# songhayeong/aes-fhe

Hardware: AMD Instinct MI355X
Metric: AES-128 blocks/sec (homomorphic full round) at N=2^16, L=30; 1/2/4/8 MI355X (higher is better)
Workload: dtype u64

## Files before the change

### aes-fhe_amd/csrc/bconv_cols.h

```cpp
#pragma once
#include "bconv_mfma.h"
#include "ntt256f.h"

namespace aesfhe {

__device__ __forceinline__ void cols256_stages_store(double (&x)[16], double q, double qi, bool big, const double* tg,
                                                     const double* cw, const double* twq, double* s, u64* out, int b,
                                                     int cl, int c) {
#pragma unroll
    for (int st = 0; st < 4; st++) {
        const int m = 1 << st, hh = 8 >> st;
        if (big && st == 2) {
#pragma unroll
            for (int a = 0; a < 16; a++) x[a] = fred(x[a], q, qi);
        }
#pragma unroll
        for (int a = 0; a < 16; a++) {
            if (a & hh) continue;
            const int ti = m + (a >> (4 - st));
            ct_fw(x[a], x[a + hh], cw[ti], tg[ti], q);
        }
    }
#pragma unroll
    for (int a = 0; a < 16; a++) s[(a * 16 + b) * kPadF + cl] = x[a];
    __syncthreads();
    const int ap = b;
#pragma unroll
    for (int bb = 0; bb < 16; bb++) x[bb] = s[(ap * 16 + bb) * kPadF + cl];
#pragma unroll
    for (int st = 4; st < 8; st++) {
        const int m = 1 << st, hh = 128 >> st;
        if (big && (st & 1) == 0) {
#pragma unroll
            for (int bb = 0; bb < 16; bb++) x[bb] = fred(x[bb], q, qi);
        }
#pragma unroll
        for (int bb = 0; bb < 16; bb++) {
            if (bb & hh) continue;
            ct_f(x[bb], x[bb + hh], twq[m + ap * (m >> 4) + (bb >> (8 - st))], q);
        }
    }
#pragma unroll
    for (int bb = 0; bb < 16; bb++) st_d(&out[(ap * 16 + bb) * 256 + c], x[bb]);
}

template <int NSTEP, bool YIN, bool VC = false, int PF = 1, int TT = 4, int LT = 2, int MODE = 0>
__global__ __launch_bounds__(256, TT == 4 ? 2 : 3) void k_bconv_cols(BconvArgs a, Tabs T, int ntile) {
    static_assert(TT == 4 || TT == 2, "4 or 2 targets per workgroup");
    static_assert(LT == 1 || LT == 2, "1 or 2 LDS tiles");
    __shared__ double s[LT][256 * kPadF];
    __shared__ double twq[TT][256];
    const int tid = threadIdx.x, lane = tid & 63, w = tid >> 6, c = lane & 31, h = lane >> 5;
    const int cl = tid & 15, b = tid >> 4;
    const int id = blockIdx.x, x8 = id & 7, j = id >> 3;
    const int tile = j % ntile, u = (j / ntile) * 8 + x8;
    const int bx = u & 15, z = u >> 4, zb = z / a.nc, zc = z - zb * a.nc;
    const int logN = T.logN;
    const u64* src = a.src + (long)zb * a.sbs + (long)zc * a.scs;
    u64* dst = a.dst + (long)zb * a.dbs + (long)zc * a.dcs;
    auto limb_of = [&](int tau) { return tau < a.skip0 ? tau : tau + a.skipn; };
    auto pid_of = [&](int tl) { return tl <= a.tl_l ? tl : a.Lp1 + tl - a.tl_l - 1; };
    const int tau0 = TT * tile;
    const int nlive = min(TT, a.nt - tau0);
#pragma unroll
    for (int m = 0; m < TT; m++)
        if (m < nlive) twq[m][tid] = T.psif[((long)pid_of(limb_of(tau0 + m)) << logN) + tid];
    bc_v4i af[NSTEP];
    {
        const int row = lane & 31, ta = row >> 3, pb = (row & 3) + 4 * ((row >> 2) & 1);
        const int tau = tau0 + ta;
        const bc_v4i* ap =
            (const bc_v4i*)(a.tab + ((long)(ta < TT && tau < a.nt ? pid_of(limb_of(tau)) : 0) * 8 + pb) * kBconvKT + 16 * h);
#pragma unroll
        for (int st = 0; st < NSTEP; st++) af[st] = ap[2 * st];
    }
    const u64* sp[NSTEP][2];
    double sq[NSTEP][2], sf[NSTEP][2];
#pragma unroll
    for (int st = 0; st < NSTEP; st++)
#pragma unroll
        for (int uu = 0; uu < 2; uu++) {
            const int sl = 4 * st + 2 * h + uu;
            const int i = sl < a.ns ? sl : 0;
            sp[st][uu] = src + ((long)i << logN) + bx * 16 + (c & 15);
            if (!YIN) {
                const int pid = i < a.s_nq ? a.s_q0 + i : a.s_p0 + i - a.s_nq;
                sq[st][uu] = (double)a.qall[pid];
                sf[st][uu] = a.sinvf[i];
            }
        }
    double xv[TT][16];
    double eq[TT], eqi[TT], ew32[TT], ef32[TT], ecr[TT];
#pragma unroll
    for (int m = 0; m < TT; m++) {
        const int pid = tau0 + m < a.nt ? pid_of(limb_of(tau0 + m)) : 0;
        const double* pc = a.pc + 4 * pid;
        eq[m] = pc[0], eqi[m] = pc[1], ew32[m] = pc[2], ef32[m] = pc[3], ecr[m] = a.corr[pid];
    }
    double ev[VC ? 4 * NSTEP : 1];
#pragma unroll
    for (int sl = 0; sl < (VC ? 4 * NSTEP : 0); sl++) ev[sl] = a.einv[sl];
    u64 raw[PF + 1][NSTEP][2][2];
    auto load = [&](u64 (&r)[NSTEP][2][2], int ar) {
#pragma unroll
        for (int st = 0; st < NSTEP; st++)
#pragma unroll
            for (int uu = 0; uu < 2; uu++)
#pragma unroll
                for (int g = 0; g < 2; g++) r[st][uu][g] = sp[st][uu][(16 * ar + 4 * w + 2 * g + (c >> 4)) * 256];
    };
#pragma unroll
    for (int p = 0; p < PF; p++) load(raw[p], p);
#pragma unroll
    for (int ar = 0; ar < 16; ar++) {
        if (ar + PF < 16) load(raw[(ar + PF) % (PF + 1)], ar + PF);
        bc_v4i bf[2][NSTEP];
        double ys[2][NSTEP][2];
#pragma unroll
        for (int st = 0; st < NSTEP; st++)
#pragma unroll
            for (int uu = 0; uu < 2; uu++)
#pragma unroll
                for (int g = 0; g < 2; g++) {
                    u64 yb = PF ? raw[ar % (PF + 1)][st][uu][g] : sp[st][uu][(16 * ar + 4 * w + 2 * g + (c >> 4)) * 256];
                    if (!YIN) {
                        const double q = sq[st][uu], f = sf[st][uu];
                        double y = fmul_rem(u2d(yb), tw_w(f, q), f, q);
                        y = y < 0.0 ? y + q : y;
                        yb = (u64)__double_as_longlong(y + 4503599627370496.0) & 0xFFFFFFFFFFFFFULL;
                    }
                    if (VC) ys[g][st][uu] = u2d(yb);
                    bf[g][st][2 * uu] = (int)(unsigned)yb ^ (int)0x80808080;
                    bf[g][st][2 * uu + 1] = (int)(unsigned)(yb >> 32) ^ (int)0x80808080;
                }
        if constexpr (VC) {
            double yl[NSTEP][2][2];
#pragma unroll
            for (int st = 0; st < NSTEP; st++)
#pragma unroll
                for (int uu = 0; uu < 2; uu++) swap_halves(ys[0][st][uu], ys[1][st][uu], yl[st][uu][0], yl[st][uu][1]);
            double sum = 0.0;
#pragma unroll
            for (int st = 0; st < NSTEP; st++)
#pragma unroll
                for (int hh = 0; hh < 2; hh++)
#pragma unroll
                    for (int uu = 0; uu < 2; uu++) {
                        const int sl = 4 * st + 2 * hh + uu;
                        sum = sum + yl[st][uu][hh] * ev[sl];
                    }
            const int vown = (int)__builtin_rint(sum);
            const auto pr = __builtin_amdgcn_permlane32_swap((unsigned)vown, (unsigned)vown, false, false);
            const int voth = (int)(h ? pr[0] : pr[1]);
#pragma unroll
            for (int st = 0; st < NSTEP; st++)
#pragma unroll
                for (int uu = 0; uu < 2; uu++)
                    if (4 * st + 2 * h + uu == a.ns) {
#pragma unroll
                        for (int g = 0; g < 2; g++) {
                            bf[g][st][2 * uu] = ((g == h ? vown : voth) & 0xff) ^ (int)0x80808080;
                            bf[g][st][2 * uu + 1] = (int)0x80808080;
                        }
                    }
        }
        if constexpr (MODE == 2) {
#pragma unroll
            for (int m = 0; m < TT; m++) xv[m][ar] = (double)(bf[0][0][0] & 0xffffff) + (double)(bf[1][NSTEP - 1][3] & 0xff);
            continue;
        }
        bc_v16i acc[2];
#pragma unroll
        for (int g = 0; g < 2; g++) {
            acc[g] = bc_v16i{};
#pragma unroll
            for (int st = 0; st < NSTEP; st++) acc[g] = __builtin_amdgcn_mfma_i32_32x32x32_i8(af[st], bf[g][st], acc[g], 0, 0, 0);
        }
#pragma unroll
        for (int m = 0; m < TT; m++) {
            if (m >= nlive) break;
            double part[2];
#pragma unroll
            for (int g = 0; g < 2; g++) {
                const int p01 = acc[g][4 * m] + acc[g][4 * m + 1] * 256, p23 = acc[g][4 * m + 2] + acc[g][4 * m + 3] * 256;
                part[g] = __builtin_fma((double)p23, 65536.0, (double)p01);
            }
            double lo, hi;
            swap_halves(part[0], part[1], lo, hi);
            xv[m][ar] = fred(lo + fmul_rem(hi, ew32[m], ef32[m], eq[m]) + ecr[m], eq[m], eqi[m]);
        }
    }
    __syncthreads();
    if constexpr (MODE == 1) {
#pragma unroll
        for (int m = 0; m < TT; m++) {
            if (m >= nlive) break;
            u64* o = dst + ((long)limb_of(tau0 + m) << logN);
#pragma unroll
            for (int ar = 0; ar < 16; ar++) st_d(&o[(ar * 16 + b) * 256 + bx * 16 + cl], xv[m][ar]);
        }
        return;
    }
#pragma unroll
    for (int m = 0; m < TT; m++) {
        if (m >= nlive) break;
        if (LT == 1 && m > 0) __syncthreads();
        const int tl = limb_of(tau0 + m), pid = pid_of(tl);
        const double q = (double)T.q[pid], qi = T.qinv[pid];
        cols256_stages_store(xv[m], q, qi, q >= kBigPrime, T.psif + ((long)pid << logN), T.cw + (long)pid * kColW,
                             twq[m], s[m % LT], dst + ((long)tl << logN), b, cl, bx * 16 + cl);
    }
}

}
```

### aes-fhe_amd/csrc/engine.hip

```cpp
#include <hip/hip_runtime.h>

#include <algorithm>
#include <atomic>
#include <cstdarg>
#include <cstdlib>
#include <cstdio>
#include <cstring>
#include <map>
#include <unordered_map>
#include <memory>
#include <mutex>
#include <string>
#include <vector>

#include "../../include/aesfhe.h"
#include "kernels_ops.h"
#include "ntt256f.h"
#include "ks_fused.h"
#include "bconv_mfma.h"
#include "bconv_cols.h"
#include "basis_tables.h"
#include "bsgs_plan.h"
#include "operands.h"
#include "arena.h"
// ... 241 lines not shown
    }
    ~ProfScope() {
        if (!on) return;
        hipEventRecord(b, s);
        e->recs.push_back({fam, a, b, bytes, label, disp});
    }
};

static void prof_flush(aesfhe_engine* e) {
    if (e->recs.empty()) return;
    hipStreamSynchronize(e->stream);
    for (auto& r : e->recs) {
        float ms = 0;
        hipEventElapsedTime(&ms, r.a, r.b);
        e->prof_ms[r.fam] += ms;
        e->prof_bytes[r.fam] += r.bytes;
        e->prof_n[r.fam] += 1;
        if (r.label) {
            KernStat& k = e->prof_k[r.label];
            k.n++;
            k.d += r.disp;
            k.ms += ms;
            k.bytes += r.bytes;
        }
        e->spare.push_back(r.a);
        e->spare.push_back(r.b);
    }
    e->recs.clear();
}

template <typename T>
static T* upload_small(aesfhe_engine* e, const T* src, size_t count) {
    size_t bytes = (count * sizeof(T) + 255) & ~(size_t)255;
    if (bytes > e->ring_size) throw_err(AESFHE_EARG, "argument upload too large");
    if (e->ring_off + bytes > e->ring_size) {
        HIPC(hipStreamSynchronize(e->stream));
        e->ring_off = 0;
    }
    memcpy(e->ring_h + e->ring_off, src, count * sizeof(T));
    T* dst = (T*)(e->ring_d + e->ring_off);
    HIPC(hipMemcpyAsync(dst, e->ring_h + e->ring_off, count * sizeof(T), hipMemcpyHostToDevice, e->stream));
    e->ring_off += bytes;
    return dst;
}

struct DevOperands {
    const u64* const* ptr = nullptr;
    const long *bs = nullptr, *ps = nullptr;
    const int* np = nullptr;
};
enum { OP_PTR = 1, OP_BS = 2, OP_PS = 4, OP_NP = 8 };
static std::vector<DevOperands> upload(aesfhe_engine* e, std::initializer_list<const OperandTable*> tabs, int fields) {
    std::vector<DevOperands> d(tabs.size());
    auto array = [&](int bit, auto OperandTable::*src, auto DevOperands::*dst) {
        if (!(fields & bit)) return;
        size_t i = 0;
        for (const OperandTable* t : tabs) {
            if (!(t->*src).empty()) d[i].*dst = upload_small(e, (t->*src).data(), (t->*src).size());
            i++;
        }
    };
    array(OP_PTR, &OperandTable::ptr, &DevOperands::ptr);
    array(OP_BS, &OperandTable::bs, &DevOperands::bs);
    array(OP_PS, &OperandTable::ps, &DevOperands::ps);
    array(OP_NP, &OperandTable::np, &DevOperands::np);
    return d;
}

static void* pool_get(aesfhe_engine* e, size_t bytes, bool tmp = false) {
    static const bool poison = getenv("AESFHE_POOL_POISON") && atoi(getenv("AESFHE_POOL_POISON"));
    (void)tmp;
    void* p = e->pool.get(bytes);
    e->peak_total = std::max(e->peak_total, e->pool.live + e->tpool.live);
    if (poison && p) HIPC(hipMemsetAsync(p, 0xA5, bytes, e->stream));
    return p;
}
static u64* dalloc(aesfhe_engine* e, size_t words) { return (u64*)pool_get(e, words * 8, true); }
static void dfree(aesfhe_engine* e, u64* p, size_t words) { e->pool.put(p, words * 8); }

struct Tmp {
    aesfhe_engine* e = nullptr;
    u64* p = nullptr;
    size_t w = 0;
    Tmp() = default;
    Tmp(aesfhe_engine* e_, size_t words) : e(e_), p(dalloc(e_, words)), w(words) {}
    Tmp(Tmp&& o) noexcept : e(o.e), p(o.p), w(o.w) { o.p = nullptr; }
    Tmp& operator=(Tmp&& o) noexcept {
        std::swap(e, o.e), std::swap(p, o.p), std::swap(w, o.w);
        o.reset();
        return *this;
    }
    ~Tmp() { reset(); }
    void reset() {
        if (p) dfree(e, p, w);
        p = nullptr;
    }
    explicit operator bool() const { return p != nullptr; }
};

struct CtFree {
    void operator()(aesfhe_ct* c) const { aesfhe_ct_free(c); }
};
using CtPtr = std::unique_ptr<aesfhe_ct, CtFree>;

static void release_all(std::vector<CtPtr>& v, aesfhe_ct** outs) {
    for (size_t i = 0; i < v.size(); i++) outs[i] = v[i].release();
}

static CtPtr ct_new(aesfhe_engine* e, int B, int np, int level) {
    auto* c = new aesfhe_ct{e, B, np, level, 0, nullptr, 0};
    e->refs++;
    CtPtr h(c);
    c->bytes = (size_t)B * np * (level + 1) * e->N * 8;
    c->d = (u64*)pool_get(e, c->bytes);
    return h;
}

static std::vector<CtPtr> ct_split_batch(aesfhe_engine* e, CtPtr r, int m) {
    const int B = r->B / m;
    const size_t part = (size_t)B * r->np * (r->level + 1) * e->N * 8;
    std::vector<CtPtr> out(m);
    for (int t = 0; t < m; t++) {
        out[t].reset(new aesfhe_ct{e, B, r->np, r->level, 0, nullptr, 0});
        e->refs++;
    }
    e->pool.split(r->d, m, part);
    for (int t = 0; t < m; t++) {
        out[t]->bytes = part;
        out[t]->d = (u64*)((char*)r->d + (size_t)t * part);
    }
    r->d = nullptr;
    aesfhe_ct_free(r.release());
    return out;
}

static CtPtr ct_zero_new(aesfhe_engine* e, int B, int np, int level) {
    CtPtr c = ct_new(e, B, np, level);
    HIPC(hipMemsetAsync(c->d, 0, c->bytes, e->stream));
    c->is_zero = 1;
    return c;
}

using View = Operand;

static View view_of(const aesfhe_ct* c) {
    View v;
    v.d = c->d;
    v.B = c->B;
    v.np = c->np;
    v.level = c->level;
    v.ps = (long)(c->level + 1) * c->eng->N;
    v.bs = (long)c->np * v.ps;
    v.zero = c->is_zero;
    return v;
}

static Opnd opnd(const View& v, int outB) {
    Opnd o;
    o.ptr = v.zero ? nullptr : v.d;
    o.bs = bcast_stride(v.B, v.bs, outB);
    o.ps = v.ps;
    o.np = v.np;
    o.bmask = (v.B > 1 && v.B < outB) ? v.B - 1 : -1;
    return o;
}

static Out out_of(aesfhe_ct* c) {
    Out o;
    o.ptr = c->d;
    o.ps = (long)(c->level + 1) * c->eng->N;
    o.bs = (long)c->np * o.ps;
    return o;
}

static View view_of(const CtPtr& c) { return view_of(c.get()); }
static Out out_of(const CtPtr& c) { return out_of(c.get()); }

static dim3 ew_grid(aesfhe_engine* e, int y, int z) { return dim3(e->N / 256, y, z); }

template <int R1>
static void ntt_fwd_t(aesfhe_engine* e, Span src, Span dst, int total) {
    constexpr int CW = (kTile / R1) < kC2 ? (kTile / R1) : kC2;
    constexpr int RW = (kTile / kC2) < R1 ? (kTile / kC2) : R1;
    Tabs T = e->tabs();
    const double by = 8.0 * e->N * (double)total;
    {
        ProfScope ps(e, FAM_NTT, by, "ntt_generic");
        hipLaunchKernelGGL(k_ntt_fwd_cols<R1>, dim3(kC2 / CW, total), dim3(256), 0, e->stream, src, dst, T);
    }
    {
        ProfScope ps(e, FAM_NTT, by, "ntt_generic");
        hipLaunchKernelGGL(k_ntt_fwd_rows<R1>, dim3(R1 / RW, total), dim3(256), 0, e->stream, dst, T);
    }
}
template <int R1>
static void ntt_inv_t(aesfhe_engine* e, Span src, Span dst, int total) {
    constexpr int CW = (kTile / R1) < kC2 ? (kTile / R1) : kC2;
    constexpr int RW = (kTile / kC2) < R1 ? (kTile / kC2) : R1;
    Tabs T = e->tabs();
    const double by = 8.0 * e->N * (double)total;
    {
        ProfScope ps(e, FAM_NTT, by, "ntt_generic");
        hipLaunchKernelGGL(k_ntt_inv_rows<R1>, dim3(R1 / RW, total), dim3(256), 0, e->stream, src, dst, T);
    }
    {
        ProfScope ps(e, FAM_NTT, by, "ntt_generic");
        hipLaunchKernelGGL(k_ntt_inv_cols<R1>, dim3(kC2 / CW, total), dim3(256), 0, e->stream, dst, T);
    }
}

template <int R>
static void ntt256(aesfhe_engine* e, Span src, Span dst, int total, bool inverse, const double* lf = nullptr) {
    Tabs T = e->tabs();
    const double by = 8.0 * e->N * (double)total;
    {
        ProfScope ps(e, FAM_NTT, by, inverse ? "ntt_inv_rows" : "ntt_fwd_cols");
        if (!inverse) hipLaunchKernelGGL(k_nttf_fwd_cols<R>, dim3(16, total), dim3(256), 0, e->stream, src, dst, T);
        else hipLaunchKernelGGL((k_nttf_inv_rows<R, false>), dim3(R / 16, total), dim3(256), 0, e->stream, src, dst, T, Span{}, (const u64*)nullptr);
    }
    ProfScope ps(e, FAM_NTT, by, inverse ? "ntt_inv_cols" : "ntt_fwd_rows");
    if (!inverse) hipLaunchKernelGGL((k_nttf_fwd_rows_t<false, R>), dim3(R / 16, total), dim3(256), 0, e->stream, dst, T, RowFin{});
    else if (lf) hipLaunchKernelGGL((k_nttf_inv_cols<R, true>), dim3(16, total), dim3(256), 0, e->stream, dst, T, lf);
    else hipLaunchKernelGGL((k_nttf_inv_cols<R, false>), dim3(16, total), dim3(256), 0, e->stream, dst, T, (const double*)nullptr);
}

static bool fused_ntt(const aesfhe_engine* e) { return e->logN == 16 || e->logN == 17; }

static void intt_prod(aesfhe_engine* e, Span a, Span b, Span dst, int total, const u64* fac, const double* lf = nullptr) {
    if (total <= 0) return;
    Tabs T = e->tabs();
    const double by = 8.0 * e->N * (double)total;
    {
        ProfScope ps(e, FAM_NTT, 2.0 * by, "ntt_inv_rows_prod");
        if (e->logN == 16) {
            if (fac) hipLaunchKernelGGL((k_nttf_inv_rows<256, true, true>), dim3(16, total), dim3(256), 0, e->stream, a, dst, T, b, fac);
            else hipLaunchKernelGGL((k_nttf_inv_rows<256, true, false>), dim3(16, total), dim3(256), 0, e->stream, a, dst, T, b, fac);
        } else {
            if (fac) hipLaunchKernelGGL((k_nttf_inv_rows<512, true, true>), dim3(32, total), dim3(256), 0, e->stream, a, dst, T, b, fac);
            else hipLaunchKernelGGL((k_nttf_inv_rows<512, true, false>), dim3(32, total), dim3(256), 0, e->stream, a, dst, T, b, fac);
        }
    }
    ProfScope ps(e, FAM_NTT, by, "ntt_inv_cols");
    if (e->logN == 16) {
        if (lf) hipLaunchKernelGGL((k_nttf_inv_cols<256, true>), dim3(16, total), dim3(256), 0, e->stream, dst, T, lf);
        else hipLaunchKernelGGL((k_nttf_inv_cols<256, false>), dim3(16, total), dim3(256), 0, e->stream, dst, T, lf);
    } else {
        if (lf) throw_err(AESFHE_EUNSUPPORTED, "per-limb INTT factors at N = 2^17");
        hipLaunchKernelGGL((k_nttf_inv_cols<512, false>), dim3(16, total), dim3(256), 0, e->stream, dst, T, lf);
    }
    HIPC(hipGetLastError());
}

static void ntt_fwd_cols(aesfhe_engine* e, Span src, Span dst, int total) {
    if (e->logN == 16) hipLaunchKernelGGL(k_nttf_fwd_cols<256>, dim3(16, total), dim3(256), 0, e->stream, src, dst, e->tabs());
    else hipLaunchKernelGGL(k_nttf_fwd_cols<512>, dim3(16, total), dim3(256), 0, e->stream, src, dst, e->tabs());
}
static void ntt_fwd_cols(aesfhe_engine* e, Span sp, int total) { ntt_fwd_cols(e, sp, sp, total); }

static void ntt(aesfhe_engine* e, Span src, Span dst, int total, bool inverse) {
    if (total <= 0) return;
    if (e->logN == 16 || e->logN == 17) {
        if (e->logN == 16) ntt256<256>(e, src, dst, total, inverse);
        else ntt256<512>(e, src, dst, total, inverse);
        HIPC(hipGetLastError());
        return;
    }
    switch (e->logN) {
#define CASE(LG, R)                                                        \
    case LG:                                                               \
        if (inverse) ntt_inv_t<R>(e, src, dst, total);                     \
        else ntt_fwd_t<R>(e, src, dst, total);                             \
        break;
        CASE(10, 4)
        CASE(11, 8)
        CASE(12, 16)
        CASE(13, 32)
        CASE(14, 64)
        CASE(15, 128)
        CASE(16, 256)
        CASE(17, 512)
#undef CASE
        default:
            throw_err(AESFHE_EUNSUPPORTED, "log_n %d not supported by the HIP NTT", e->logN);
    }
    HIPC(hipGetLastError());
}

static Span span_s(u64* base, long pstride, int nl, int nq, int qpid0, int spid0) {
    Span s;
    s.base = base;
    s.pstride = pstride;
    s.nl = nl;
    s.nq = nq;
    s.qpid0 = qpid0;
    s.spid0 = spid0;
    return s;
}


static void build_tables(aesfhe_engine* e) {
    const int N = e->N, np = e->np, L = e->L, K = e->K, Lp1 = e->Lp1;
    const auto& Q = e->chain.q;
    std::vector<u64> hq(Q), hpsi((size_t)np * N), hipsi((size_t)np * N), hninv(np);
    std::vector<double> hqinv(np), hpsif((size_t)np * N), hipsif((size_t)np * N), hninvf(np);
    e->h_iroot.resize(np);
    for (int p = 0; p < np; p++) {
        u64 qq = Q[p];
        hqinv[p] = 1.0 / (double)qq;
        u64 psi = min_primitive_root(qq, N), ip = h_invmod(psi, qq);
        std::vector<u64> pw(N), ipw(N);
        pw[0] = ipw[0] = 1;
        for (int k = 1; k < N; k++) {
            pw[k] = h_mulmod(pw[k - 1], psi, qq);
            ipw[k] = h_mulmod(ipw[k - 1], ip, qq);
        }
        for (int k = 0; k < N; k++) {
            unsigned r = bit_reverse((unsigned)k, e->logN);
            hpsi[(size_t)p * N + k] = pw[r];
            hipsi[(size_t)p * N + k] = ipw[r];
            hpsif[(size_t)p * N + k] = (double)pw[r] / (double)qq;
            hipsif[(size_t)p * N + k] = (double)ipw[r] / (double)qq;
        }
        e->h_iroot[p] = pw[N / 2];
        hninv[p] = h_invmod((u64)N, qq);
        hninvf[p] = (double)hninv[p] / (double)qq;
    }
    DevBlocks& dev = e->dev;
    Tabs& t = e->tab;
    t.q = e->q = dev.up(hq);
    t.qinv = e->qinv = dev.up(hqinv);
    t.psi = dev.up(hpsi);
    t.psif = dev.up(hpsif);
    t.ipsi = dev.up(hipsi);
    t.ipsif = dev.up(hipsif);
    t.ninv = dev.up(hninv);
    t.ninvf = dev.up(hninvf);
    if (fused_ntt(e)) {
        const int R = N / 256;
        std::vector<double> hr((size_t)np * R * 8), hir((size_t)np * R * 8);
        for (int p = 0; p < np; p++)
            for (int row = 0; row < R; row++)
                for (int sh = 0; sh < 8; sh++) {
                    hr[((size_t)p * R + row) * 8 + sh] = hpsif[(size_t)p * N + (row << sh)];
                    hir[((size_t)p * R + row) * 8 + sh] = hipsif[(size_t)p * N + (row << sh)];
                }
        t.rtwf = dev.up(hr);
        t.irtwf = dev.up(hir);
    }
    {
        std::vector<Tw> htw((size_t)np * N), hitw((size_t)np * N);
        for (size_t i = 0; i < htw.size(); i++) {
            htw[i] = Tw{hpsi[i], hpsif[i]};
            hitw[i] = Tw{hipsi[i], hipsif[i]};
        }
        t.tw = dev.up(htw);
        t.itw = dev.up(hitw);
    }
    {
        std::vector<double> hcw((size_t)np * kColW), hicw((size_t)np * kColW);
        for (int p = 0; p < np; p++)
            for (int k = 0; k < kColW; k++) {
                hcw[(size_t)p * kColW + k] = (double)hpsi[(size_t)p * N + (k < N ? k : 0)];
                hicw[(size_t)p * kColW + k] = (double)hipsi[(size_t)p * N + (k < N ? k : 0)];
            }
        t.cw = dev.up(hcw);
        t.icw = dev.up(hicw);
    }
    t.logN = e->logN;
    t.Lp1 = Lp1;

    static_assert(sizeof(WQ) == sizeof(TwD), "ModDown's hatf rows are the kernels' TwD");
    ModUpTables mu;
    ModDownTables md;
    if (!build_modup_tables(Q, Lp1, e->A, hninv, mu) || !build_moddown_tables(Q, Lp1, e->K, hninv, md))
        throw_err(AESFHE_EUNSUPPORTED, "base-conversion constant beyond 7 bytes");
    e->mu_hatinvf = dev.up(mu.hatinvf);
    e->mu_nhatf = dev.up(mu.nhatf);
    e->bc_mu_tab = dev.up(mu.tab);
    e->bc_mu_corr = dev.up(mu.corr);
    e->bc_pc = dev.up(mu.pc);
    e->md = MdTabs{dev.up(md.invf), dev.up(md.ninvf), dev.up(md.einv), dev.up(md.tab), dev.up(md.corr),
                   dev.up(md.dinv), dev.up(md.dinvf), (TwD*)dev.up(md.hatf), dev.up(md.dmodf)};
    e->pmod = dev.up(md.pmod);
    e->pmodf = e->md.dmodf;
    const RescaleTables rs = build_rescale_tables(Q, Lp1);
    e->rs_inv = dev.up(rs.inv);
    e->rs_invf = dev.up(rs.invf);
    e->rs_mod = dev.up(rs.mod);
}

extern "C" int aesfhe_engine_create(const aesfhe_params* pp, aesfhe_engine** out) {
    API_BEGIN
    if (!pp || !out) throw_err(AESFHE_EARG, "null argument");
    if (pp->log_n < 10 || pp->log_n > 17) throw_err(AESFHE_EARG, "log_n must be in [10, 17]");
    if (pp->max_level < 1 || pp->special_primes < 1 || pp->special_primes > 16 ||
        pp->max_level + 1 + pp->special_primes > kMaxPrimes)
        throw_err(AESFHE_EARG, "bad level / special prime count");
    if (pp->scale_bits < 20 || pp->scale_bits > 50 || pp->base_bits > 50 || pp->special_bits > 50)
        throw_err(AESFHE_EARG, "bit sizes must keep every prime below 2^50");
    std::unique_ptr<aesfhe_engine> e(new aesfhe_engine());
    e->logN = pp->log_n;
    e->N = 1 << pp->log_n;
    e->L = pp->max_level;
    e->K = pp->special_primes;
    e->Lp1 = e->L + 1;
    e->np = e->L + 1 + e->K;
    e->A = pp->digit_primes > 0 ? pp->digit_primes : e->K;
    if (e->A > 16) throw_err(AESFHE_EARG, "key-switch digit width %d outside 1..16", e->A);
    e->dnum = (e->L + 1 + e->A - 1) / e->A;
    e->device = pp->device;
    e->seed = pp->seed;
    e->ck = chacha_key(pp->seed, pp->seed_ext);
    if (pp->primes) {
        e->chain.q.assign(pp->primes, pp->primes + e->np);
        e->chain.scale = scales_from_primes(e->chain.q, e->L, pp->scale_bits);
    } else {
        e->chain = make_chain(e->logN, e->L, e->K, pp->base_bits, pp->special_bits, pp->scale_bits);
    }
    for (u64 x : e->chain.q)
        if (x >> 50) throw_err(AESFHE_EARG, "prime %llu exceeds 2^50", (unsigned long long)x);
    if (e->A > e->K && !digits_below_p(e->chain.q, e->Lp1, e->K, e->A))
        throw_err(AESFHE_EARG, "a key-switch digit of %d primes exceeds P (%d special primes)", e->A, e->K);
    HIPC(hipSetDevice(e->device));
    HIPC(hipStreamCreateWithFlags(&e->stream, hipStreamNonBlocking));
    build_tables(e.get());
    e->pool.chunk_bytes = std::max((size_t)1 << 28, ((size_t)16384 * 8) << e->logN);
    if (e->logN == 16) {
        e->pool.chunk_bytes = (size_t)8192 * 8 << e->logN;
        e->pool.first_fit = true;
        e->pool.grow_cap = 1.2;
    }
    if (const char* cm = getenv("AESFHE_ARENA_CHUNK_MB")) {
        const long mb = atol(cm);
        if (mb > 0) e->pool.chunk_bytes = (size_t)mb << 20;
    }
    e->tpool.chunk_bytes = e->pool.chunk_bytes;
    e->tpool.tag = 't';
    if (const char* tp = getenv("AESFHE_ARENA_TRACE")) {
        static std::atomic<int> engines{0};
        const std::string path = std::string(tp) + "." + std::to_string(engines++);
        e->pool.trace = e->tpool.trace = fopen(path.c_str(), "w");
    }
    HIPC(hipMalloc(&e->ring_d, e->ring_size));
    HIPC(hipHostMalloc((void**)&e->ring_h, e->ring_size, hipHostMallocDefault));
    *out = e.release();
    API_END
}

extern "C" int aesfhe_chain(const aesfhe_params* pp, uint64_t* primes, double* scales) {
    API_BEGIN
    Chain c = make_chain(pp->log_n, pp->max_level, pp->special_primes, pp->base_bits, pp->special_bits, pp->scale_bits);
    std::copy(c.q.begin(), c.q.end(), primes);
    std::copy(c.scale.begin(), c.scale.end(), scales);
    API_END
}

static void engine_unref(aesfhe_engine* e) {
    if (--e->refs == 0) delete e;
}
extern "C" void aesfhe_engine_destroy(aesfhe_engine* e) {
    if (e) engine_unref(e);
}

extern "C" int aesfhe_engine_dims(const aesfhe_engine* e, int32_t d[4]) {
    d[0] = e->logN;
    d[1] = e->L;
    d[2] = e->K;
    d[3] = e->dnum;
    return 0;
}
extern "C" int aesfhe_engine_primes(const aesfhe_engine* e, uint64_t* o) {
    std::copy(e->chain.q.begin(), e->chain.q.end(), o);
    return 0;
}
extern "C" int aesfhe_engine_scales(const aesfhe_engine* e, double* o) {
    std::copy(e->chain.scale.begin(), e->chain.scale.end(), o);
    return 0;
}
extern "C" double aesfhe_engine_mul_scale(const aesfhe_engine* e, int32_t l) {
    if (l < 1 || l > e->L) return 0.0;
    return e->chain.scale[l - 1] * (double)e->chain.q[l] / e->chain.scale[l];
}
extern "C" int aesfhe_engine_sync(aesfhe_engine* e) {
    API_BEGIN
    HIPC(hipStreamSynchronize(e->stream));
    API_END
}
extern "C" int aesfhe_engine_profile(aesfhe_engine* e, int32_t en) {
    API_BEGIN
    prof_flush(e);
    e->prof = en == -1 ? 7 : (en & 7);
    if (e->prof) {
        for (int i = 0; i < 4; i++) e->prof_ms[i] = e->prof_bytes[i] = 0, e->prof_n[i] = 0;
        e->prof_k.clear();
        while (e->spare.size() < 65536) {
            hipEvent_t x;
            HIPC(hipEventCreate(&x));
            e->spare.push_back(x);
        }
    }
    API_END
}
extern "C" int aesfhe_engine_profile_read(aesfhe_engine* e, const char* fam, int64_t* n,
                                          double* ms, double* bytes) {
    API_BEGIN
    prof_flush(e);
    int f = !strcmp(fam, "ntt") ? FAM_NTT : !strcmp(fam, "keyswitch") ? FAM_KS : !strcmp(fam, "elementwise") ? FAM_EW : 3;
    if (f == 3) {
        *n = e->prof_n[0] + e->prof_n[1] + e->prof_n[2];
        *ms = e->prof_ms[0] + e->prof_ms[1] + e->prof_ms[2];
        if (bytes) *bytes = e->prof_bytes[0] + e->prof_bytes[1] + e->prof_bytes[2];
    } else {
        *n = e->prof_n[f];
        *ms = e->prof_ms[f];
        if (bytes) *bytes = e->prof_bytes[f];
    }
    API_END
}
extern "C" int aesfhe_engine_profile_kernels(aesfhe_engine* e, char* buf, int64_t cap, int64_t* need) {
    API_BEGIN
    prof_flush(e);
    std::string js = "{";
    char tmp[256];
    for (auto& kv : e->prof_k) {
        snprintf(tmp, sizeof tmp, "%s\"%s\": [%lld, %.6f, %.1f, %lld]", js.size() > 1 ? ", " : "", kv.first.c_str(),
                 (long long)kv.second.n, kv.second.ms, kv.second.bytes, (long long)kv.second.d);
        js += tmp;
    }
    js += "}";
    if (need) *need = (int64_t)js.size() + 1;
    if (buf && cap > 0) {
        const size_t m = std::min((size_t)cap - 1, js.size());
        memcpy(buf, js.data(), m);
        buf[m] = 0;
    }
    API_END
}
extern "C" int64_t aesfhe_engine_device_bytes(const aesfhe_engine* e) { return (int64_t)(e->pool.held + e->tpool.held); }
extern "C" int aesfhe_engine_pool_trim(aesfhe_engine* e) {
    API_BEGIN
    HIPC(hipSetDevice(e->device));
    HIPC(hipStreamSynchronize(e->stream));
    e->pool.trim();
    e->tpool.trim();
    API_END
}
extern "C" int aesfhe_engine_pool_stats(const aesfhe_engine* e, int64_t* out) {
    if (!e || !out) return set_err(AESFHE_EARG, "null argument");
    out[0] = (int64_t)(e->pool.held + e->tpool.held);
    out[1] = (int64_t)(e->pool.live + e->tpool.live);
    out[2] = e->pool.mallocs + e->tpool.mallocs;
    out[3] = e->pool.trims + e->tpool.trims;
    out[4] = e->pool.reuse_larger + e->tpool.reuse_larger;
    out[5] = (int64_t)e->peak_total;
    out[6] = (int64_t)(e->pool.fragmentation() + e->tpool.fragmentation());
    return AESFHE_OK;
}

extern "C" int aesfhe_encode(int32_t logN, const double* re, const double* im, int64_t n_slots,
                             double scale, int64_t* co) {
    API_BEGIN
    if (logN < 2 || logN > 17) throw_err(AESFHE_EARG, "log_n out of range");
    Codec c(logN);
    if (n_slots < 0 || n_slots > c.n) throw_err(AESFHE_EARG, "too many slots: %lld > %d", (long long)n_slots, c.n);
    std::vector<double> vr(c.n, 0.0), vi(c.n, 0.0);
    for (int64_t i = 0; i < n_slots; i++) {
        vr[i] = re ? re[i] : 0.0;
        vi[i] = im ? im[i] : 0.0;
    }
    c.special_inv(vr.data(), vi.data());
    for (int i = 0; i < c.n; i++) {
        double a = vr[i] * scale, b = vi[i] * scale;
        if (!(std::fabs(a) < 9.0e18) || !(std::fabs(b) < 9.0e18))
            throw_err(AESFHE_EARG, "encoded coefficient overflows int64 (scale too large?)");
        co[i] = llround(a);
        co[i + c.n] = llround(b);
    }
    API_END
}

extern "C" int aesfhe_decode(int32_t logN, const int64_t* co, double scale, double* re, double* im) {
    API_BEGIN
    if (logN < 2 || logN > 17) throw_err(AESFHE_EARG, "log_n out of range");
    Codec c(logN);
    for (int i = 0; i < c.n; i++) {
        re[i] = (double)co[i] / scale;
        im[i] = (double)co[i + c.n] / scale;
    }
    c.special(re, im);
    API_END
}

extern "C" void aesfhe_key_free(aesfhe_key* k) {
    if (!k) return;
    aesfhe_engine* e = k->eng;
    e->pool.put(k->d, k->bytes);
    delete k;
    engine_unref(e);
}
extern "C" int aesfhe_key_info(const aesfhe_key* k, int32_t* kind, uint64_t* g) {
    *kind = k->kind;
    *g = k->galois;
    return 0;
}
extern "C" uint64_t aesfhe_galois_elt(int32_t logN, int64_t rot, int32_t conj) {
    u64 M = 2ULL << logN, n = 1ULL << (logN - 1);
    if (conj) return M - 1;
    int64_t r = rot % (int64_t)n;
    if (r < 0) r += (int64_t)n;
    u64 ex = (n - (u64)r) % n;
    return h_powmod(5, ex, M);
}

static aesfhe_key* key_new(aesfhe_engine* e, int kind, size_t words) {
    auto* k = new aesfhe_key;
    k->eng = e;
    e->refs++;
    k->kind = kind;
    k->galois = 0;
    k->keyseed = 0;
    k->bytes = words * 8;
    k->d = (u64*)pool_get(e, k->bytes);
    return k;
}

static void sample_small_ntt(aesfhe_engine* e, u64* dst, int nprimes, u64 key, int kind) {
    Span s = span_s(dst, 0, nprimes, std::min(nprimes, e->Lp1), 0, e->Lp1);
    s.pstride = (long)nprimes * e->N;
    hipLaunchKernelGGL(k_sample_small, dim3((e->N / 8 + 255) / 256), dim3(256), 0, e->stream, s, e->ck, key, kind, e->q, e->logN, e->Lp1, nprimes);
    ntt(e, s, s, nprimes, false);
}

extern "C" int aesfhe_key_secret(aesfhe_engine* e, uint64_t seed, aesfhe_key** out) {
    API_BEGIN
    aesfhe_key* k = key_new(e, 0, (size_t)e->np * e->N);
    k->keyseed = derive(e->seed, seed);
    sample_small_ntt(e, k->d, e->np, derive(k->keyseed, 1), 0);
    *out = k;
    API_END
}

extern "C" int aesfhe_key_public(aesfhe_engine* e, const aesfhe_key* sk, aesfhe_key** out) {
    API_BEGIN
    if (!sk || sk->kind != 0) throw_err(AESFHE_EARG, "public key needs a secret key");
    const int N = e->N, nq = e->Lp1;
    aesfhe_key* k = key_new(e, 1, (size_t)2 * nq * N);
    k->keyseed = sk->keyseed;
    u64* b = k->d;
    u64* a = k->d + (size_t)nq * N;
    Span sa = span_s(a, 0, nq, nq, 0, e->Lp1);
    hipLaunchKernelGGL(k_sample_uniform, dim3((N / 8 + 255) / 256, nq), dim3(256), 0, e->stream, sa, e->ck, derive(sk->keyseed, 2), e->q, e->logN, e->Lp1);
    Tmp et(e, (size_t)nq * N);
    sample_small_ntt(e, et.p, nq, derive(sk->keyseed, 3), 1);
    hipLaunchKernelGGL(k_key_combine, dim3(N / 256, nq), dim3(256), 0, e->stream, a, sk->d, et.p, (const u64*)nullptr, (const u64*)nullptr, 0, 0, b, e->q, e->qinv, e->logN);
    HIPC(hipGetLastError());
    *out = k;
    API_END
}

static aesfhe_key* make_ksk_t(aesfhe_engine* e, const u64* starget, u64 keyseed, const u64* sprime, int kind,
                              u64 g, u64 salt) {
    const int N = e->N, np = e->np;
    aesfhe_key* k = key_new(e, kind, (size_t)e->dnum * 2 * np * N);
    k->galois = g;
    k->keyseed = keyseed;
    k->ndig = e->dnum;
    u64 base = derive(derive(keyseed, 4 + (u64)kind), g);
    if (salt) base = derive(base, salt);
    Tmp et(e, (size_t)np * N);
// ... 2252 lines not shown
```

### aes-fhe_amd/csrc/kernels.h

```cpp
#pragma once
#include <hip/hip_runtime.h>

#include <cstdint>

#define AESFHE_HD __host__ __device__
#include "ckks_host.h"

namespace aesfhe {

constexpr int kMaxPrimes = 96;
constexpr double kBigPrime = 4398046511104.0;

__device__ __forceinline__ u64 add_m(u64 a, u64 b, u64 q) {
    u64 s = a + b;
    return s >= q ? s - q : s;
}
__device__ __forceinline__ u64 sub_m(u64 a, u64 b, u64 q) { return a >= b ? a - b : a + q - b; }

__device__ __forceinline__ u64 fix_m(u64 r, u64 q) {
    int64_t s = (int64_t)r;
    s = s < 0 ? s + (int64_t)q : s;
    s = s >= (int64_t)q ? s - (int64_t)q : s;
    return (u64)s;
}

__device__ __forceinline__ double u2d(u64 a) {
    return __longlong_as_double((long long)(a | 0x4330000000000000ULL)) - 4503599627370496.0;
}
__device__ __forceinline__ u64 rint_u(double x_times, double scale) {
    return (u64)__double_as_longlong(__builtin_fma(x_times, scale, 4503599627370496.0)) & 0xFFFFFFFFFFFFFULL;
}

__device__ __forceinline__ u64 mul_m(u64 a, u64 b, u64 q, double qinv) {
    const u64 qh = rint_u(u2d(a) * u2d(b), qinv);
    return fix_m(a * b - qh * q, q);
}
__device__ __forceinline__ u64 mul_w(u64 a, u64 w, double wq, u64 q) {
    const u64 qh = rint_u(u2d(a), wq);
    int64_t r = (int64_t)(a * w - qh * q);
    r += (r >> 63) & (int64_t)q;
    return (u64)r;
}

constexpr double kMagic52 = 6755399441055744.0;
__device__ __forceinline__ double fmul_rem(double a, double w, double wq, double q) {
    const double p = a * w;
    const double pl = __builtin_fma(a, w, -p);
    const double qh = __builtin_rint(a * wq);
    const double u = __builtin_fma(-qh, q, p);
    return u + pl;
}
__device__ __forceinline__ double fmul_rem_r(double a, double w, double wq, double q) {
    return fmul_rem(a, w, wq, q);
}
__device__ __forceinline__ double fred(double x, double q, double qinv) {
    const double qh = __builtin_rint(x * qinv);
    return __builtin_fma(-qh, q, x);
}
__device__ __forceinline__ u64 fcanon(double x, double q, double qinv) {
    double r = fred(x, q, qinv);
    r = r < 0.0 ? r + q : r;
    return (u64)__double_as_longlong(r + 4503599627370496.0) & 0xFFFFFFFFFFFFFULL;
}
__device__ __forceinline__ double tw_w(double wq, double q) {
    return __builtin_rint(wq * q);
}
struct Opnd2 {
    const u64* ptr;
    long bs, ps;
    int np;
};
struct alignas(16) TwD {
    double w;
    double wq;
};

struct Span {
    u64* base;
    long pstride;
    int nl;
    int nq;
    int qpid0;
    int spid0;
    int pmask = -1;
};

__device__ __forceinline__ u64* span_ptr(const Span& s, int y, int logN, int Lp1, int& pid) {
    (void)Lp1;
    int p = y / s.nl, l = y - p * s.nl;
    pid = l < s.nq ? s.qpid0 + l : s.spid0 + (l - s.nq);
    return s.base + (long)(p & s.pmask) * s.pstride + ((long)l << logN);
}

constexpr int kColW = 64;

struct Tabs {
    const u64* q;
    const double* qinv;
    const u64* psi;
    const double* psif;
    const u64* ipsi;
    const double* ipsif;
    const double* rtwf;
    const double* irtwf;
    const u64* ninv;
    const double* ninvf;
    const struct Tw* tw;
    const struct Tw* itw;
    const double* cw;
    const double* icw;
    int logN;
    int Lp1;
};

struct alignas(16) Tw {
    u64 w;
    double wq;
};

constexpr int kTile = 4096;
constexpr int kC2 = 256;

template <int R1>
__global__ __launch_bounds__(256) void k_ntt_fwd_cols(Span src, Span dst, Tabs T) {
    constexpr int CW = (kTile / R1) < kC2 ? (kTile / R1) : kC2;
    __shared__ u64 s[R1 * CW];
    int pid;
    const u64* in = span_ptr(src, blockIdx.y, T.logN, T.Lp1, pid);
    u64* out = span_ptr(dst, blockIdx.y, T.logN, T.Lp1, pid);
    const int c0 = blockIdx.x * CW;
    const u64 q = T.q[pid];
    const u64* W = T.psi + ((long)pid << T.logN);
    const double* Wf = T.psif + ((long)pid << T.logN);
    for (int e = threadIdx.x; e < R1 * CW; e += 256) {
        int r = e / CW, c = e - r * CW;
        s[e] = in[r * kC2 + c0 + c];
    }
    __syncthreads();
    for (int m = 1, t = R1 / 2; m < R1; m <<= 1, t >>= 1) {
        for (int bf = threadIdx.x; bf < (R1 / 2) * CW; bf += 256) {
            int c = bf % CW, g = bf / CW;
            int i = g / t, r1 = i * 2 * t + (g - i * t), r2 = r1 + t;
            u64 w = W[m + i];
            double wf = Wf[m + i];
            u64 U = s[r1 * CW + c];
            u64 V = mul_w(s[r2 * CW + c], w, wf, q);
            s[r1 * CW + c] = add_m(U, V, q);
            s[r2 * CW + c] = sub_m(U, V, q);
        }
        __syncthreads();
    }
    for (int e = threadIdx.x; e < R1 * CW; e += 256) {
        int r = e / CW, c = e - r * CW;
        out[r * kC2 + c0 + c] = s[e];
    }
}

template <int R1>
__global__ __launch_bounds__(256) void k_ntt_fwd_rows(Span dst, Tabs T) {
    constexpr int RW = (kTile / kC2) < R1 ? (kTile / kC2) : R1;
    __shared__ u64 s[RW * kC2];
    int pid;
    u64* io = span_ptr(dst, blockIdx.y, T.logN, T.Lp1, pid);
    const int row0 = blockIdx.x * RW;
    const u64 q = T.q[pid];
    const u64* W = T.psi + ((long)pid << T.logN);
    const double* Wf = T.psif + ((long)pid << T.logN);
    u64* base = io + (long)row0 * kC2;
    for (int e = threadIdx.x; e < RW * kC2; e += 256) s[e] = base[e];
    __syncthreads();
    for (int ml = 1, t = kC2 / 2; ml < kC2; ml <<= 1, t >>= 1) {
        for (int bf = threadIdx.x; bf < RW * (kC2 / 2); bf += 256) {
            int rl = bf / (kC2 / 2), g = bf - rl * (kC2 / 2);
            int i = g / t, c1 = i * 2 * t + (g - i * t), c2 = c1 + t;
            int widx = R1 * ml + (row0 + rl) * ml + i;
            u64 w = W[widx];
            double wf = Wf[widx];
            u64* rowp = s + rl * kC2;
            u64 U = rowp[c1];
            u64 V = mul_w(rowp[c2], w, wf, q);
            rowp[c1] = add_m(U, V, q);
            rowp[c2] = sub_m(U, V, q);
        }
        __syncthreads();
    }
    for (int e = threadIdx.x; e < RW * kC2; e += 256) base[e] = s[e];
}

template <int R1>
__global__ __launch_bounds__(256) void k_ntt_inv_rows(Span src, Span dst, Tabs T) {
    constexpr int RW = (kTile / kC2) < R1 ? (kTile / kC2) : R1;
    __shared__ u64 s[RW * kC2];
    int pid;
    const u64* in = span_ptr(src, blockIdx.y, T.logN, T.Lp1, pid);
    u64* out = span_ptr(dst, blockIdx.y, T.logN, T.Lp1, pid);
    const int row0 = blockIdx.x * RW;
    const u64 q = T.q[pid];
    const u64* W = T.ipsi + ((long)pid << T.logN);
    const double* Wf = T.ipsif + ((long)pid << T.logN);
    const int N = 1 << T.logN;
    for (int e = threadIdx.x; e < RW * kC2; e += 256) s[e] = in[(long)row0 * kC2 + e];
    __syncthreads();
    for (int t = 1; t < kC2; t <<= 1) {
        int hg = N / (2 * t);
        for (int bf = threadIdx.x; bf < RW * (kC2 / 2); bf += 256) {
            int rl = bf / (kC2 / 2), g = bf - rl * (kC2 / 2);
            int i = g / t, c1 = i * 2 * t + (g - i * t), c2 = c1 + t;
            int widx = hg + (row0 + rl) * (kC2 / (2 * t)) + i;
            u64* rowp = s + rl * kC2;
            u64 U = rowp[c1], V = rowp[c2];
            rowp[c1] = add_m(U, V, q);
            rowp[c2] = mul_w(sub_m(U, V, q), W[widx], Wf[widx], q);
        }
        __syncthreads();
    }
    for (int e = threadIdx.x; e < RW * kC2; e += 256) out[(long)row0 * kC2 + e] = s[e];
}

template <int R1>
__global__ __launch_bounds__(256) void k_ntt_inv_cols(Span dst, Tabs T) {
    constexpr int CW = (kTile / R1) < kC2 ? (kTile / R1) : kC2;
    __shared__ u64 s[R1 * CW];
    int pid;
    u64* io = span_ptr(dst, blockIdx.y, T.logN, T.Lp1, pid);
    const int c0 = blockIdx.x * CW;
    const u64 q = T.q[pid];
    const u64* W = T.ipsi + ((long)pid << T.logN);
    const double* Wf = T.ipsif + ((long)pid << T.logN);
    for (int e = threadIdx.x; e < R1 * CW; e += 256) {
        int r = e / CW, c = e - r * CW;
        s[e] = io[r * kC2 + c0 + c];
    }
    __syncthreads();
    for (int tr = 1; tr < R1; tr <<= 1) {
        int hg = R1 / (2 * tr);
        for (int bf = threadIdx.x; bf < (R1 / 2) * CW; bf += 256) {
            int c = bf % CW, g = bf / CW;
            int i = g / tr, r1 = i * 2 * tr + (g - i * tr), r2 = r1 + tr;
            u64 U = s[r1 * CW + c], V = s[r2 * CW + c];
            s[r1 * CW + c] = add_m(U, V, q);
            s[r2 * CW + c] = mul_w(sub_m(U, V, q), W[hg + i], Wf[hg + i], q);
        }
        __syncthreads();
    }
    const u64 ni = T.ninv[pid];
    const double nif = T.ninvf[pid];
    for (int e = threadIdx.x; e < R1 * CW; e += 256) {
        int r = e / CW, c = e - r * CW;
        io[r * kC2 + c0 + c] = mul_w(s[e], ni, nif, q);
    }
}

}
```

### aes-fhe_amd/csrc/kernels_ops.h

```cpp
#pragma once
#include "kernels.h"

namespace aesfhe {

__device__ __forceinline__ u64 red_m(u64 x, u64 q, double qinv) {
    u64 qh = (u64)((double)x * qinv);
    return fix_m(x - qh * q, q);
}

struct Opnd {
    const u64* ptr;
    long bs;
    long ps;
    int np;
    int bmask = -1;
};

__device__ const u64 kZeroWord = 0;
__device__ __forceinline__ u64 opnd_get(const Opnd& o, int b, int p, int l, int k, int logN) {
    const bool has = o.ptr && p < o.np;
    return *(has ? o.ptr + (long)(b & o.bmask) * o.bs + (long)p * o.ps + ((long)l << logN) + k : &kZeroWord);
}

struct Out {
    u64* ptr;
    long bs;
    long ps;
};

__global__ void k_addsub(Opnd a, Opnd b, Out o, int np, const u64* __restrict__ qs, int sub,
                         int logN) {
    const int k = blockIdx.x * blockDim.x + threadIdx.x;
    const int l = blockIdx.y, bb = blockIdx.z / np, p = blockIdx.z - bb * np;
    const u64 q = qs[l];
    u64 va = opnd_get(a, bb, p, l, k, logN), vb = opnd_get(b, bb, p, l, k, logN);
    o.ptr[(long)bb * o.bs + (long)p * o.ps + ((long)l << logN) + k] = sub ? sub_m(va, vb, q) : add_m(va, vb, q);
}

__global__ void k_gather_batch(const u64* __restrict__ src, u64* __restrict__ dst,
                               const int* __restrict__ idx, long per) {
    const int b = blockIdx.y;
    const ulonglong2* s = (const ulonglong2*)(src + (long)idx[b] * per);
    ulonglong2* o = (ulonglong2*)(dst + (long)b * per);
    const long nv = per >> 1;
    for (long i = (long)blockIdx.x * blockDim.x + threadIdx.x; i < nv; i += (long)gridDim.x * blockDim.x)
        o[i] = s[i];
}

__global__ void k_mul_const(Opnd in, Out o, int np, const u64* __restrict__ f,
                            const double* __restrict__ ff, const u64* __restrict__ qs, int acc,
                            int logN) {
    const int k = blockIdx.x * blockDim.x + threadIdx.x;
    const int l = blockIdx.y, bb = blockIdx.z / np, p = blockIdx.z - bb * np;
    const u64 q = qs[l];
    const int h = k >> (logN - 1);
    u64 v = mul_w(opnd_get(in, bb, p, l, k, logN), f[2 * l + h], ff[2 * l + h], q);
    u64* dst = o.ptr + (long)bb * o.bs + (long)p * o.ps + ((long)l << logN) + k;
    *dst = acc ? add_m(*dst, v, q) : v;
}

__global__ void k_mul_pt(Opnd in, const u64* __restrict__ pt, Out o, int np,
                         const u64* __restrict__ qs, const double* __restrict__ qinv, int logN) {
    const int k = blockIdx.x * blockDim.x + threadIdx.x;
    const int l = blockIdx.y, bb = blockIdx.z / np, p = blockIdx.z - bb * np;
    u64 v = mul_m(opnd_get(in, bb, p, l, k, logN), pt[((long)l << logN) + k], qs[l], qinv[l]);
    o.ptr[(long)bb * o.bs + (long)p * o.ps + ((long)l << logN) + k] = v;
}

__global__ void k_add_pt(Opnd in, const u64* __restrict__ pt, Out o, int np,
                         const u64* __restrict__ qs, int logN) {
    const int k = blockIdx.x * blockDim.x + threadIdx.x;
    const int l = blockIdx.y, bb = blockIdx.z / np, p = blockIdx.z - bb * np;
    u64 v = opnd_get(in, bb, p, l, k, logN);
    if (p == 0) v = add_m(v, pt[((long)l << logN) + k], qs[l]);
    o.ptr[(long)bb * o.bs + (long)p * o.ps + ((long)l << logN) + k] = v;
}

__global__ void k_add_const(Opnd in, Out o, int np, const u64* __restrict__ f,
                            const u64* __restrict__ qs, int logN) {
    const int k = blockIdx.x * blockDim.x + threadIdx.x;
    const int l = blockIdx.y, bb = blockIdx.z / np, p = blockIdx.z - bb * np;
    u64 v = opnd_get(in, bb, p, l, k, logN);
    if (p == 0) v = add_m(v, f[2 * l + (k >> (logN - 1))], qs[l]);
    o.ptr[(long)bb * o.bs + (long)p * o.ps + ((long)l << logN) + k] = v;
}

__global__ void k_tensor(Opnd a, Opnd b, Out o, const u64* __restrict__ qs,
                         const double* __restrict__ qinv, int acc, int logN) {
    const int k = blockIdx.x * blockDim.x + threadIdx.x;
    const int l = blockIdx.y, bb = blockIdx.z;
    const u64 q = qs[l];
    const double qi = qinv[l];
    u64 a0 = opnd_get(a, bb, 0, l, k, logN), a1 = opnd_get(a, bb, 1, l, k, logN);
    u64 b0 = opnd_get(b, bb, 0, l, k, logN), b1 = opnd_get(b, bb, 1, l, k, logN);
    u64 d0 = mul_m(a0, b0, q, qi);
    u64 d1 = add_m(mul_m(a0, b1, q, qi), mul_m(a1, b0, q, qi), q);
    u64 d2 = mul_m(a1, b1, q, qi);
    u64* base = o.ptr + (long)bb * o.bs + ((long)l << logN) + k;
    if (acc) {
        base[0] = add_m(base[0], d0, q);
        base[o.ps] = add_m(base[o.ps], d1, q);
        base[2 * o.ps] = add_m(base[2 * o.ps], d2, q);
    } else {
        __builtin_nontemporal_store(d0, &base[0]);
        __builtin_nontemporal_store(d1, &base[o.ps]);
        __builtin_nontemporal_store(d2, &base[2 * o.ps]);
    }
}

__global__ void k_tensor_fma(Opnd a, Opnd b, Opnd c, Out o, const u64* __restrict__ fac,
                             const u64* __restrict__ qs, const double* __restrict__ qinv, int logN) {
    const int k = blockIdx.x * blockDim.x + threadIdx.x;
    const int l = blockIdx.y, bb = blockIdx.z;
    const u64 q = qs[l];
    const double qi = qinv[l];
    const u64 am = fac[3 * l], cm = fac[3 * l + 1], km = fac[3 * l + 2];
    const u64 a0 = opnd_get(a, bb, 0, l, k, logN), a1 = opnd_get(a, bb, 1, l, k, logN);
    const u64 b0 = opnd_get(b, bb, 0, l, k, logN), b1 = opnd_get(b, bb, 1, l, k, logN);
    u64 d0 = mul_m(mul_m(a0, b0, q, qi), am, q, qi);
    u64 d1 = mul_m(add_m(mul_m(a0, b1, q, qi), mul_m(a1, b0, q, qi), q), am, q, qi);
    const u64 d2 = mul_m(mul_m(a1, b1, q, qi), am, q, qi);
    d0 = add_m(d0, mul_m(opnd_get(c, bb, 0, l, k, logN), cm, q, qi), q);
    d1 = add_m(d1, mul_m(opnd_get(c, bb, 1, l, k, logN), cm, q, qi), q);
    d0 = add_m(d0, km, q);
    u64* base = o.ptr + (long)bb * o.bs + ((long)l << logN) + k;
    base[0] = d0;
    base[o.ps] = d1;
    base[2 * o.ps] = d2;
}

__global__ void k_lincomb(const u64* const* __restrict__ ptrs, const long* __restrict__ bstr,
                          const int* __restrict__ npi, int n, const long* __restrict__ pss,
                          const u64* __restrict__ f,
                          const double* __restrict__ ff, Out o, int np, int nl,
                          const u64* __restrict__ qs, const double* __restrict__ qinv, int logN) {
    const int k = blockIdx.x * blockDim.x + threadIdx.x;
    const int l = blockIdx.y, bb = blockIdx.z / np, p = blockIdx.z - bb * np;
    const u64 q = qs[l];
    const int h = k >> (logN - 1);
    const long off = ((long)l << logN) + k;
    u64 acc = 0;
    for (int i0 = 0; i0 < n; i0 += 8) {
        u64 v[8];
#pragma unroll
        for (int c = 0; c < 8; c++) {
            const int i = i0 + c;
            v[c] = (i < n && p < npi[i]) ? ptrs[i][(long)bb * bstr[i] + (long)p * pss[i] + off] : 0;
        }
#pragma unroll
        for (int c = 0; c < 8; c++) {
            const int i = i0 + c;
            if (i < n) {
                const int fi = (i * nl + l) * 2 + h;
                acc += mul_w(v[c], f[fi], ff[fi], q);
            }
        }
    }
    o.ptr[(long)bb * o.bs + (long)p * o.ps + ((long)l << logN) + k] = red_m(acc, q, qinv[l]);
}

constexpr int kManyMax = 16;
__global__ void k_lincomb_many(const u64* const* __restrict__ ptrs, const long* __restrict__ bstr,
                               const int* __restrict__ npi, int n, const long* __restrict__ pss,
                               const u64* __restrict__ F, const double* __restrict__ FF, int m,
                               u64* __restrict__ out, long orow, long obs, int np, int nl,
                               const u64* __restrict__ qs, const double* __restrict__ qinv,
                               int logN) {
    const int k = blockIdx.x * blockDim.x + threadIdx.x;
    const int l = blockIdx.y, bb = blockIdx.z / np, p = blockIdx.z - bb * np;
    const u64 q = qs[l];
    const int h = k >> (logN - 1);
    const long off = ((long)l << logN) + k;
    u64 v[kManyMax];
#pragma unroll
    for (int j = 0; j < kManyMax; j++)
        v[j] = (j < n && p < npi[j]) ? ptrs[j][(long)bb * bstr[j] + (long)p * pss[j] + off] : 0;
    u64* o = out + (long)bb * obs + ((long)p * nl << logN) + off;
    for (int i = 0; i < m; i++) {
        u64 acc = 0;
#pragma unroll
        for (int j = 0; j < kManyMax; j++) {
            if (j < n) {
                const int fi = ((i * n + j) * nl + l) * 2 + h;
                acc += mul_w(v[j], F[fi], FF[fi], q);
            }
        }
        o[(long)i * orow] = red_m(acc, q, qinv[l]);
    }
}

__global__ void k_dot(const u64* const* __restrict__ ap, const long* __restrict__ abs_,
                      const u64* const* __restrict__ bp, const long* __restrict__ bbs, int n,
                      long ps, Out o, const u64* __restrict__ qs, const double* __restrict__ qinv,
                      int logN) {
    const int k = blockIdx.x * blockDim.x + threadIdx.x;
    const int l = blockIdx.y, bb = blockIdx.z;
    const u64 q = qs[l];
    const double qi = qinv[l];
    const long off = ((long)l << logN) + k;
    u64 d0 = 0, d1 = 0, d2 = 0;
    for (int i = 0; i < n; i++) {
        const u64* a = ap[i] + (long)bb * abs_[i] + off;
        const u64* b = bp[i] + (long)bb * bbs[i] + off;
        const u64 a0 = a[0], a1 = a[ps], b0 = b[0], b1 = b[ps];
        d0 += mul_m(a0, b0, q, qi);
        d1 += mul_m(a0, b1, q, qi) + mul_m(a1, b0, q, qi);
        d2 += mul_m(a1, b1, q, qi);
        if ((i & 15) == 15) {
            d0 = red_m(d0, q, qi);
            d1 = red_m(d1, q, qi);
            d2 = red_m(d2, q, qi);
        }
    }
    u64* base = o.ptr + (long)bb * o.bs + off;
    base[0] = red_m(d0, q, qi);
    base[o.ps] = red_m(d1, q, qi);
    base[2 * o.ps] = red_m(d2, q, qi);
}

__global__ void k_dot_fma(const u64* const* __restrict__ ap, const long* __restrict__ abs_,
                          const u64* const* __restrict__ bp, const long* __restrict__ bbs, int n,
                          long ps, const u64* const* __restrict__ cp, const long* __restrict__ cbs,
                          const long* __restrict__ cps, int nc, const u64* __restrict__ cf,
                          const u64* __restrict__ km, int nl, Out o, const u64* __restrict__ qs,
                          const double* __restrict__ qinv, int logN) {
    const int k = blockIdx.x * blockDim.x + threadIdx.x;
    const int l = blockIdx.y, bb = blockIdx.z;
    const u64 q = qs[l];
    const double qi = qinv[l];
    const long off = ((long)l << logN) + k;
    u64 d0 = 0, d1 = 0, d2 = 0;
    for (int i = 0; i < n; i++) {
        const u64* a = ap[i] + (long)bb * abs_[i] + off;
        const u64* b = bp[i] + (long)bb * bbs[i] + off;
        const u64 a0 = a[0], a1 = a[ps], b0 = b[0], b1 = b[ps];
        d0 += mul_m(a0, b0, q, qi);
        d1 += mul_m(a0, b1, q, qi) + mul_m(a1, b0, q, qi);
        d2 += mul_m(a1, b1, q, qi);
        if ((i & 15) == 15) {
            d0 = red_m(d0, q, qi);
            d1 = red_m(d1, q, qi);
            d2 = red_m(d2, q, qi);
        }
    }
    d0 = red_m(d0, q, qi);
    d1 = red_m(d1, q, qi);
    for (int j = 0; j < nc; j++) {
        const u64* c = cp[j] + (long)bb * cbs[j] + off;
        const u64 f = cf[(long)j * nl + l];
        d0 = add_m(d0, mul_m(c[0], f, q, qi), q);
        d1 = add_m(d1, mul_m(c[cps[j]], f, q, qi), q);
    }
    u64* base = o.ptr + (long)bb * o.bs + off;
    base[0] = add_m(d0, km[l], q);
    base[o.ps] = d1;
    base[2 * o.ps] = red_m(d2, q, qi);
}

template <bool SC = false>
__global__ void k_rescale_spread(const u64* __restrict__ x, u64* __restrict__ t, u64 ql,
                                 const u64* __restrict__ qs, const double* __restrict__ qinv,
                                 const u64* __restrict__ qlmod, int l, int logN, u64 sc, double scf) {
    const int k = blockIdx.x * blockDim.x + threadIdx.x;
    const int i = blockIdx.y, P = blockIdx.z;
    const u64 q = qs[i];
    u64 v = x[((long)P << logN) + k];
    if (SC) v = mul_w(v, sc, scf, ql);
    u64 r = red_m(v, q, qinv[i]);
    if (v > (ql >> 1)) r = sub_m(r, qlmod[i], q);
    t[(((long)P * l + i) << logN) + k] = r;
}

template <bool SC = false>
__global__ void k_rescale_finish(Opnd c, const u64* __restrict__ t, Out o, int np, int l,
                                 const u64* __restrict__ qs, const u64* __restrict__ inv,
                                 const double* __restrict__ invf, int logN, const u64* __restrict__ f,
                                 const double* __restrict__ ff) {
    const int k = blockIdx.x * blockDim.x + threadIdx.x;
    const int i = blockIdx.y, P = blockIdx.z, bb = P / np, p = P - bb * np;
    const u64 q = qs[i];
    u64 cv = opnd_get(c, bb, p, i, k, logN);
    if (SC) cv = mul_w(cv, f[2 * i], ff[2 * i], q);
    u64 tv = t[(((long)P * l + i) << logN) + k];
    o.ptr[(long)bb * o.bs + (long)p * o.ps + ((long)i << logN) + k] = mul_w(sub_m(cv, tv, q), inv[i], invf[i], q);
}

__global__ void k_rescale_finish_g(const u64* __restrict__ c, long cps, const u64* __restrict__ t,
                                   u64* const* __restrict__ outs, long ops, int np, int Bg, int l,
                                   const u64* __restrict__ qs, const u64* __restrict__ inv,
                                   const double* __restrict__ invf, int logN) {
    const int k = blockIdx.x * blockDim.x + threadIdx.x;
    const int i = blockIdx.y, P = blockIdx.z;
    const int g = P / (Bg * np), rem = P - g * Bg * np;
    const u64 q = qs[i];
    u64 cv = c[(long)P * cps + ((long)i << logN) + k];
    u64 tv = t[(((long)P * l + i) << logN) + k];
    outs[g][(long)rem * ops + ((long)i << logN) + k] = mul_w(sub_m(cv, tv, q), inv[i], invf[i], q);
}

template <int BM>
__global__ void k_ks_inner_all(const u64* __restrict__ d, long dbs, const u64* __restrict__ ext,
                               long exs, long exj, const u64* __restrict__ key, long kdig,
                               long kcomp, u64* __restrict__ acc, long abs_, long acs, int B,
                               int beta, int K, int l, const u64* __restrict__ qall,
                               const double* __restrict__ qinvall, int Lp1, Opnd addend,
                               const double* __restrict__ pmodf, int logN, int accum) {
    const int k = blockIdx.x * blockDim.x + threadIdx.x;
    const int t = blockIdx.y;
    const int pid = t <= l ? t : Lp1 + (t - l - 1);
    const double q = (double)qall[pid];
    const double qi = qinvall[pid];
    const int own = t <= l ? t / K : -1;
    double kb[BM], ka[BM], kbq[BM], kaq[BM];
#pragma unroll
    for (int j = 0; j < BM; j++) {
        kb[j] = ka[j] = kbq[j] = kaq[j] = 0.0;
        if (j < beta) {
            const long ko = (long)j * kdig + ((long)pid << logN) + k;
            kb[j] = u2d(key[ko]);
            ka[j] = u2d(key[ko + kcomp]);
            kbq[j] = kb[j] * qi;
            kaq[j] = ka[j] * qi;
        }
    }
#pragma unroll 4
    for (int bb = 0; bb < B; bb++) {
        double s0 = 0.0, s1 = 0.0;
#pragma unroll
        for (int j = 0; j < BM; j++) {
            if (j < beta) {
                const double e = u2d((j == own) ? d[(long)bb * dbs + ((long)t << logN) + k]
                                                : ext[(long)j * exj + (long)bb * exs + ((long)t << logN) + k]);
                s0 += fmul_rem(e, kb[j], kbq[j], q);
                s1 += fmul_rem(e, ka[j], kaq[j], q);
                if ((j & 3) == 3) {
                    s0 = fred(s0, q, qi);
                    s1 = fred(s1, q, qi);
                }
            }
        }
        if (pmodf && t <= l) {
            const double f = pmodf[t], w = tw_w(f, q);
            s0 = fred(s0, q, qi) + fmul_rem(u2d(opnd_get(addend, bb, 0, t, k, logN)), w, f, q);
            s1 = fred(s1, q, qi) + fmul_rem(u2d(opnd_get(addend, bb, 1, t, k, logN)), w, f, q);
        }
        u64* a0 = acc + (long)bb * abs_ + ((long)t << logN) + k;
        if (accum) {
            s0 += u2d(a0[0]);
            s1 += u2d(a0[acs]);
        }
        a0[0] = fcanon(s0, q, qi);
        a0[acs] = fcanon(s1, q, qi);
    }
}

template <int BM, int KC>
__global__ void k_ks_inner_multi(const u64* __restrict__ d, long dbs, const u64* __restrict__ ext,
                                 long exs, long exj, const u64* const* __restrict__ keys, int nk, long kdig,
                                 long kcomp, u64* const* __restrict__ accs, long abs_, long acs, int B,
                                 int beta, int K, int l, const u64* __restrict__ qall,
                                 const double* __restrict__ qinvall, int Lp1, Opnd addend,
                                 const double* __restrict__ pmodf, int logN) {
    const int k = blockIdx.x * blockDim.x + threadIdx.x;
    const int t = blockIdx.y;
    const int pid = t <= l ? t : Lp1 + (t - l - 1);
    const double q = (double)qall[pid];
    const double qi = qinvall[pid];
    const int own = t <= l ? t / K : -1;
    const bool pm = pmodf && t <= l;
    const double f = pm ? pmodf[t] : 0.0, fw = pm ? tw_w(f, q) : 0.0;
    for (int i0 = 0; i0 < nk; i0 += KC) {
        double kb[KC][BM], ka[KC][BM];
#pragma unroll
        for (int ii = 0; ii < KC; ii++) {
#pragma unroll
            for (int j = 0; j < BM; j++) {
                const bool ok = i0 + ii < nk && j < beta;
                const u64* kp = keys[ok ? i0 + ii : 0] + (long)j * kdig + ((long)pid << logN) + k;
                kb[ii][j] = u2d(*(ok ? kp : &kZeroWord));
                ka[ii][j] = u2d(*(ok ? kp + kcomp : &kZeroWord));
            }
        }
#pragma unroll 1
        for (int bb = 0; bb < B; bb++) {
            double e[BM];
#pragma unroll
            for (int j = 0; j < BM; j++)
                e[j] = u2d(*(j >= beta ? &kZeroWord
                             : (j == own) ? d + (long)bb * dbs + ((long)t << logN) + k
                                          : ext + (long)j * exj + (long)bb * exs + ((long)t << logN) + k));
            double ad0 = 0.0, ad1 = 0.0;
            if (pm) {
                ad0 = fmul_rem(u2d(opnd_get(addend, bb, 0, t, k, logN)), fw, f, q);
                ad1 = fmul_rem(u2d(opnd_get(addend, bb, 1, t, k, logN)), fw, f, q);
            }
#pragma unroll
            for (int ii = 0; ii < KC; ii++) {
                if (i0 + ii >= nk) break;
                double s0 = 0.0, s1 = 0.0;
#pragma unroll
                for (int j = 0; j < BM; j++) {
                    if (j < beta) {
                        s0 += fmul_rem(e[j], kb[ii][j], kb[ii][j] * qi, q);
                        s1 += fmul_rem(e[j], ka[ii][j], ka[ii][j] * qi, q);
                        if ((j & 3) == 3) {
                            s0 = fred(s0, q, qi);
                            s1 = fred(s1, q, qi);
                        }
                    }
                }
                if (pm) {
                    s0 = fred(s0, q, qi) + ad0;
                    s1 = fred(s1, q, qi) + ad1;
                }
                u64* a0 = accs[i0 + ii] + (long)bb * abs_ + ((long)t << logN) + k;
                a0[0] = fcanon(s0, q, qi);
                a0[acs] = fcanon(s1, q, qi);
            }
        }
    }
}

template <int NE>
__global__ void k_moddown(const u64* __restrict__ acc, long abs_, long acs, int l, int r,
                          u64* __restrict__ conv, long cbs, long ccs,
                          const double* __restrict__ invf, const TwD* __restrict__ hat,
                          const double* __restrict__ einv, const double* __restrict__ dmodf,
                          int Lp1, const u64* __restrict__ qall, const double* __restrict__ qinvall,
                          int logN, int hs) {
    const int k = blockIdx.x * 512 + threadIdx.x;
    const int bb = blockIdx.z >> 1, c = blockIdx.z & 1;
    const u64* src = acc + (long)bb * abs_ + (long)c * acs;
    const int t0 = l - r + 1;
    double y[NE], z[NE];
#pragma unroll
    for (int j = 0; j < NE; j++) {
        const int pid = j < r ? t0 + j : Lp1 + (j - r);
        const double pp = (double)qall[pid];
        const double f = invf[j], w = tw_w(f, pp);
        const u64* sp = src + ((long)(t0 + j) << logN) + k;
        const double v = fmul_rem(u2d(sp[0]), w, f, pp), v2 = fmul_rem(u2d(sp[256]), w, f, pp);
        y[j] = v < 0.0 ? v + pp : v;
        z[j] = v2 < 0.0 ? v2 + pp : v2;
    }
    double v = 0.0, v2 = 0.0;
    {
        double u = 0.0, u2 = 0.0;
#pragma unroll
        for (int j = 0; j < NE; j++) {
            u = u + y[j] * einv[j];
            u2 = u2 + z[j] * einv[j];
        }
        v = __builtin_rint(u);
        v2 = __builtin_rint(u2);
    }
    const int ig = (l - r + 1 + gridDim.y - 1) / gridDim.y, i0 = blockIdx.y * ig;
    for (int i = i0; i < i0 + ig && i <= l - r; i++) {
        const double q = (double)qall[i], qi = qinvall[i];
        const double fd = dmodf[i], wd = tw_w(fd, q);
        TwD f[NE];
#pragma unroll
        for (int j = 0; j < NE; j++) f[j] = hat[i * hs + j];
        double sum = fmul_rem(-v, wd, fd, q), sum2 = fmul_rem(-v2, wd, fd, q);
        const bool fold = q >= kBigPrime;
#pragma unroll
        for (int j = 0; j < NE; j++) {
            sum += fmul_rem_r(y[j], f[j].w, f[j].wq, q);
            sum2 += fmul_rem_r(z[j], f[j].w, f[j].wq, q);
            if (fold && (j & 3) == 3) {
                sum = fred(sum, q, qi);
                sum2 = fred(sum2, q, qi);
            }
        }
        u64* o = conv + (long)bb * cbs + (long)c * ccs + ((long)i << logN) + k;
        __builtin_nontemporal_store(fcanon(sum, q, qi), &o[0]);
        __builtin_nontemporal_store(fcanon(sum2, q, qi), &o[256]);
    }
}

#define AESFHE_DISPATCH16(n, F, ...)                                                     \
    switch (n) {                                                                         \
        case 1: F<1>(__VA_ARGS__); break;   case 2: F<2>(__VA_ARGS__); break;             \
        case 3: F<3>(__VA_ARGS__); break;   case 4: F<4>(__VA_ARGS__); break;             \
        case 5: F<5>(__VA_ARGS__); break;   case 6: F<6>(__VA_ARGS__); break;             \
        case 7: F<7>(__VA_ARGS__); break;   case 8: F<8>(__VA_ARGS__); break;             \
        case 9: F<9>(__VA_ARGS__); break;   case 10: F<10>(__VA_ARGS__); break;           \
        case 11: F<11>(__VA_ARGS__); break; case 12: F<12>(__VA_ARGS__); break;           \
        case 13: F<13>(__VA_ARGS__); break; case 14: F<14>(__VA_ARGS__); break;           \
        case 15: F<15>(__VA_ARGS__); break; case 16: F<16>(__VA_ARGS__); break;           \
        default: break;                                                                  \
    }

__global__ void k_moddown_finish(const u64* __restrict__ acc, long abs_, long acs,
                                 const u64* __restrict__ conv, long cbs, long ccs, Opnd addend,
                                 Out o, const u64* __restrict__ qs, const u64* __restrict__ pinv,
                                 const double* __restrict__ pinvf, int logN) {
    const int k = blockIdx.x * blockDim.x + threadIdx.x;
    const int i = blockIdx.y, bb = blockIdx.z >> 1, c = blockIdx.z & 1;
    const u64 q = qs[i];
    u64 a = acc[(long)bb * abs_ + (long)c * acs + ((long)i << logN) + k];
    u64 v = conv[(long)bb * cbs + (long)c * ccs + ((long)i << logN) + k];
    u64 r = mul_w(sub_m(a, v, q), pinv[i], pinvf[i], q);
    r = add_m(r, opnd_get(addend, bb, c, i, k, logN), q);
    o.ptr[(long)bb * o.bs + (long)c * o.ps + ((long)i << logN) + k] = r;
}

__global__ void k_galois(Span src, Span dst, u64 g, int logN, int Lp1) {
    const int k = blockIdx.x * blockDim.x + threadIdx.x;
    int pid;
    const u64* in = span_ptr(src, blockIdx.y, logN, Lp1, pid);
    u64* out = span_ptr(dst, blockIdx.y, logN, Lp1, pid);
    const u64 M = 2ULL << logN;
    const unsigned rk = __brev((unsigned)k) >> (32 - logN);
    const u64 e = 2 * (u64)rk + 1;
    const u64 t = (g * e) & (M - 1);
    const unsigned idx = __brev((unsigned)((t - 1) >> 1)) >> (32 - logN);
    out[k] = in[idx];
}

__global__ void k_sample_uniform(Span dst, ChaKey K, u64 key, const u64* __restrict__ qall, int logN,
                                 int Lp1) {
    const int k0 = (blockIdx.x * blockDim.x + threadIdx.x) * 8;
    if (k0 >= (1 << logN)) return;
    int pid;
    u64* out = span_ptr(dst, blockIdx.y, logN, Lp1, pid);
    uint32_t o[16];
    chacha20_block(K, key, (((u64)pid << logN) + k0) >> 3, o);
    const u64 q = qall[pid];
#pragma unroll
    for (int e = 0; e < 8; e += 2) {
        ulonglong2 v;
        v.x = __umul64hi((u64)o[2 * e] | ((u64)o[2 * e + 1] << 32), q);
        v.y = __umul64hi((u64)o[2 * e + 2] | ((u64)o[2 * e + 3] << 32), q);
        *(ulonglong2*)&out[k0 + e] = v;
    }
}

__global__ void k_sample_small(Span dst, ChaKey K, u64 key, int kind, const u64* __restrict__ qall,
                               int logN, int Lp1, int nlim) {
    const int k0 = (blockIdx.x * blockDim.x + threadIdx.x) * 8;
    if (k0 >= (1 << logN)) return;
    uint32_t o[16];
    chacha20_block(K, key, (u64)k0 >> 3, o);
    i64 v[8];
#pragma unroll
    for (int e = 0; e < 8; e++) {
        const u64 r = (u64)o[2 * e] | ((u64)o[2 * e + 1] << 32);
        v[e] = kind == 0 ? ternary(r) : cbd21(r);
    }
    for (int y = 0; y < nlim; y++) {
        int pid;
        u64* out = span_ptr(dst, y, logN, Lp1, pid);
        const u64 q = qall[pid];
#pragma unroll
        for (int e = 0; e < 8; e += 2) {
            ulonglong2 w;
            w.x = v[e] >= 0 ? (u64)v[e] : q - (u64)(-v[e]);
            w.y = v[e + 1] >= 0 ? (u64)v[e + 1] : q - (u64)(-v[e + 1]);
            *(ulonglong2*)&out[k0 + e] = w;
        }
    }
}

__global__ void k_coeffs_res(const i64* __restrict__ co, u64* __restrict__ out, int nl,
                             const u64* __restrict__ qs, int logN) {
    const int k = blockIdx.x * blockDim.x + threadIdx.x;
    const int l = blockIdx.y, bb = blockIdx.z;
    const i64 v = co[((long)bb << logN) + k];
    const u64 q = qs[l];
    u64 r;
    if (v >= 0) r = (u64)v % q;
    else r = q - 1 - ((u64)(-(v + 1)) % q);
    out[(((long)bb * nl + l) << logN) + k] = r;
}

__global__ void k_key_combine(const u64* __restrict__ a, const u64* __restrict__ s,
                              const u64* __restrict__ e, const u64* __restrict__ sp,
                              const u64* __restrict__ pmod, int lo, int hi, u64* __restrict__ out,
                              const u64* __restrict__ qall, const double* __restrict__ qinvall,
                              int logN) {
    const int k = blockIdx.x * blockDim.x + threadIdx.x;
    const int pid = blockIdx.y;
    const long off = ((long)pid << logN) + k;
    const u64 q = qall[pid];
    const double qi = qinvall[pid];
    u64 v = add_m(sub_m(0, mul_m(a[off], s[off], q, qi), q), e[off], q);
    if (sp && pid >= lo && pid < hi) v = add_m(v, mul_m(pmod[pid], sp[off], q, qi), q);
    out[off] = v;
}

__global__ void k_enc_pk(const u64* __restrict__ vem, const u64* __restrict__ pk0,
                         const u64* __restrict__ pk1, u64* __restrict__ ct, int nl,
                         const u64* __restrict__ qs, const double* __restrict__ qinv, int logN) {
    const int k = blockIdx.x * blockDim.x + threadIdx.x;
    const int l = blockIdx.y, bb = blockIdx.z;
    const u64 q = qs[l];
    const double qi = qinv[l];
    const long lo = ((long)l << logN) + k;
    const long step = (long)nl << logN;
    const u64* base = vem + (long)bb * 4 * step + lo;
    u64 v = base[0], e0 = base[step], e1 = base[2 * step], m = base[3 * step];
    u64* c = ct + (long)bb * 2 * step + lo;
    c[0] = add_m(add_m(mul_m(v, pk0[lo], q, qi), e0, q), m, q);
    c[step] = add_m(mul_m(v, pk1[lo], q, qi), e1, q);
}

__global__ void k_enc_sk(const u64* __restrict__ vem, const u64* __restrict__ s,
                         u64* __restrict__ ct, int nl, const u64* __restrict__ qs,
                         const double* __restrict__ qinv, ChaKey K, const u64* __restrict__ keys, int logN) {
    const int k0 = (blockIdx.x * blockDim.x + threadIdx.x) * 8;
    if (k0 >= (1 << logN)) return;
    const int l = blockIdx.y, bb = blockIdx.z;
    const u64 q = qs[l];
    const double qi = qinv[l];
    const long step = (long)nl << logN;
    uint32_t o[16];
    chacha20_block(K, keys[bb], (((u64)l << logN) + k0) >> 3, o);
#pragma unroll
    for (int e = 0; e < 8; e++) {
        const long lo = ((long)l << logN) + k0 + e;
        const u64* base = vem + (long)bb * 4 * step + lo;
        const u64 e0 = base[step], m = base[3 * step];
        const u64 a = __umul64hi((u64)o[2 * e] | ((u64)o[2 * e + 1] << 32), q);
        u64* c = ct + (long)bb * 2 * step + lo;
        c[step] = a;
        c[0] = add_m(add_m(sub_m(0, mul_m(a, s[lo], q, qi), q), e0, q), m, q);
    }
}

__global__ void k_dec_limb0(const u64* __restrict__ ct, long bs, long ps, int np,
                            const u64* __restrict__ s, u64* __restrict__ t, u64 q, double qinv,
                            int logN) {
    const int k = blockIdx.x * blockDim.x + threadIdx.x;
    const int bb = blockIdx.z;
    const u64* c = ct + (long)bb * bs + k;
    u64 sv = s[k];
    u64 v = c[0];
    if (np >= 2) v = add_m(v, mul_m(c[ps], sv, q, qinv), q);
    if (np == 3) v = add_m(v, mul_m(c[2 * ps], mul_m(sv, sv, q, qinv), q, qinv), q);
    t[((long)bb << logN) + k] = v;
}

__global__ void k_square(const u64* __restrict__ s, u64* __restrict__ o,
                         const u64* __restrict__ qall, const double* __restrict__ qinvall,
                         int logN) {
    const int k = blockIdx.x * blockDim.x + threadIdx.x;
    const long off = ((long)blockIdx.y << logN) + k;
    o[off] = mul_m(s[off], s[off], qall[blockIdx.y], qinvall[blockIdx.y]);
}

constexpr int kPoly2Max = 16, kPoly2Out = 4, kPoly2OutMax = 8;
__global__ void __launch_bounds__(256) k_poly2(const u64* const* __restrict__ xp, const long* __restrict__ xbs,
                        const long* __restrict__ xps, int nx, const u64* const* __restrict__ yp,
                        const long* __restrict__ ybs, const long* __restrict__ yps, int ny,
                        const TwD* __restrict__ F, int mtot, int t0, int mc,
                        u64* __restrict__ out, long oos, long obs, const u64* __restrict__ qs,
                        const double* __restrict__ qinv, int logN) {
    const int k = blockIdx.x * blockDim.x + threadIdx.x;
    const int l = blockIdx.y, bb = blockIdx.z, nl = gridDim.y;
    const int h = (int)((blockIdx.x * blockDim.x) >> (logN - 1));
    const double q = (double)qs[l];
    const double qi = qinv[l];
    const long off = ((long)l << logN) + k;
    double y0[kPoly2Max - 1], y1[kPoly2Max - 1];
#pragma unroll
    for (int j = 0; j < kPoly2Max - 1; j++) {
        y0[j] = y1[j] = 0.0;
        if (j < ny - 1) {
            const u64* p = yp[j] + (long)bb * ybs[j] + off;
            y0[j] = u2d(p[0]);
            y1[j] = u2d(p[yps[j]]);
        }
    }
    double d0[kPoly2Out], d1[kPoly2Out], d2[kPoly2Out];
#pragma unroll
    for (int t = 0; t < kPoly2Out; t++) d0[t] = d1[t] = d2[t] = 0.0;
    const TwD* Fl = F + ((size_t)(l * 2 + h) * mtot + t0) * nx * ny;
#pragma unroll 1
    for (int i = 0; i < nx; i++) {
        double xa = 0.0, xb = 0.0;
        if (i > 0) {
            const u64* p = xp[i - 1] + (long)bb * xbs[i - 1] + off;
            xa = u2d(p[0]);
            xb = u2d(p[xps[i - 1]]);
        }
#pragma unroll
        for (int t = 0; t < kPoly2Out; t++) {
            if (t < mc) {
                const TwD* Fi = Fl + ((size_t)t * nx + i) * ny;
                double a0 = Fi[0].w, a1 = 0.0;
#pragma unroll
                for (int j = 1; j < kPoly2Max; j++) {
                    if (j < ny) {
                        const TwD f = Fi[j];
                        a0 += fmul_rem_r(y0[j - 1], f.w, f.wq, q);
                        a1 += fmul_rem_r(y1[j - 1], f.w, f.wq, q);
                        if ((j & 3) == 0) {
                            a0 = fred(a0, q, qi);
                            a1 = fred(a1, q, qi);
                        }
                    }
                }
                a0 = fred(a0, q, qi);
                a1 = fred(a1, q, qi);
                if (i == 0) {
                    d0[t] += a0;
                    d1[t] += a1;
// ... 48 lines not shown
        double y0[kPoly2Max - 1], y1[kPoly2Max - 1];
#pragma unroll
        for (int j = 0; j < kPoly2Max - 1; j++) {
            y0[j] = y1[j] = 0.0;
            if (j < nyv - 1) {
                const u64* p = yp[j] + (long)bb * ybs[j] + off;
                const TwD r = Rc[ycls[j + 1]];
                y0[j] = fred(fmul_rem_r(u2d(p[0]), r.w, r.wq, q), q, qi);
                y1[j] = fred(fmul_rem_r(u2d(p[yps[j]]), r.w, r.wq, q), q, qi);
            }
        }
        const double c0 = C0[(size_t)l * cxn + c];
#pragma unroll 1
    for (int i = xstart[c]; i < xstart[c + 1]; i++) {
        double xa = 0.0, xb = 0.0;
        if (i > 0) {
            const u64* p = xp[i - 1] + (long)bb * xbs[i - 1] + off;
            xa = u2d(p[0]);
            xb = u2d(p[xps[i - 1]]);
        }
#pragma unroll
        for (int t = 0; t < MO; t++) {
            if (t < mc) {
                const double* w = Wt + ((size_t)(t0 + t) * nx + i) * ny;
                double a0, a1;
                if constexpr (!big) {
                    a0 = w[0] * c0;
                    a1 = 0.0;
#pragma unroll
                    for (int j = 1; j < kPoly2Max; j++) {
                        if (j < nyv) {
                            a0 = __builtin_fma(w[j], y0[j - 1], a0);
                            a1 = __builtin_fma(w[j], y1[j - 1], a1);
                        }
                    }
                } else {
                    const double w0 = w[0];
                    a0 = fmul_rem(c0, w0, w0 * qi, q);
                    a1 = 0.0;
#pragma unroll
                    for (int j = 1; j < kPoly2Max; j++) {
                        if (j < nyv) {
                            const double wj = w[j], wjq = wj * qi;
                            a0 = fred(a0 + fmul_rem(y0[j - 1], wj, wjq, q), q, qi);
                            a1 = fred(a1 + fmul_rem(y1[j - 1], wj, wjq, q), q, qi);
                        }
                    }
                }
                if (i == 0) {
                    d0[t] += a0;
                    d1[t] += a1;
                } else {
                    const double a0q = a0 * qi, a1q = a1 * qi;
                    d0[t] += fmul_rem(xa, a0, a0q, q);
                    d1[t] += fmul_rem(xa, a1, a1q, q) + fmul_rem(xb, a0, a0q, q);
                    d2[t] += fmul_rem(xb, a1, a1q, q);
                }
                if constexpr (big) {
                    d0[t] = fred(d0[t], q, qi);
                    d1[t] = fred(d1[t], q, qi);
                    d2[t] = fred(d2[t], q, qi);
                }
            }
        }
    }
    }
    const int ob = (bb & ~3) | ((bb - orot) & 3);
    u64* o = out + (long)ob * obs + off;
    const long pstr = (long)nl << logN;
#pragma unroll
    for (int t = 0; t < MO; t++) {
        if (t < mc) {
            u64* ot = o + (long)(t0 + t) * oos;
            ot[0] = fcanon(d0[t], q, qi);
            ot[pstr] = fcanon(d1[t], q, qi);
            ot[2 * pstr] = fcanon(d2[t], q, qi);
        }
    }
}

template <int NY, bool BIG>
__device__ __forceinline__ void inner_sums(const double* __restrict__ w, double c0, const double (&y0)[NY - 1],
                                           const double (&y1)[NY - 1], double q, double qi, double& a0, double& a1) {
    if constexpr (!BIG) {
        a0 = w[0] * c0;
        a1 = 0.0;
#pragma unroll
        for (int j = 1; j < NY; j++) {
            a0 = __builtin_fma(w[j], y0[j - 1], a0);
            a1 = __builtin_fma(w[j], y1[j - 1], a1);
        }
    } else {
        const double w0 = w[0];
        a0 = fmul_rem(c0, w0, w0 * qi, q);
        a1 = 0.0;
#pragma unroll
        for (int j = 1; j < NY; j++) {
            const double wj = w[j], wjq = wj * qi;
            a0 = fred(a0 + fmul_rem(y0[j - 1], wj, wjq, q), q, qi);
            a1 = fred(a1 + fmul_rem(y1[j - 1], wj, wjq, q), q, qi);
        }
    }
}

template <int MO, bool LAZY, bool BIG = false>
__global__ void __launch_bounds__(256, 3) k_poly2_int_s(const u64* const* __restrict__ xp, const long* __restrict__ xbs,
                        const long* __restrict__ xps, int nx, const u64* const* __restrict__ yp,
                        const long* __restrict__ ybs, const long* __restrict__ yps,
                        const int* __restrict__ xstart, const int* __restrict__ ycls, int cxn,
                        int cyn, const double* __restrict__ Wt, const TwD* __restrict__ Rt,
                        const double* __restrict__ C0, int t0, u64* __restrict__ out, long oos, long obs,
                        const u64* __restrict__ qs, const double* __restrict__ qinv, int l0, int nl,
                        int logN, int orot) {
    constexpr int NY = kPoly2Max;
    static_assert(!(BIG && LAZY), "the folding path needs reduced y'");
    const int bx = blockIdx.x, half = (bx >> 3) & 1;
    const int k = (((bx >> 4) << 3) | (bx & 7)) * blockDim.x + threadIdx.x;
    const int l = l0 + blockIdx.y, bb = blockIdx.z;
    t0 += half * MO;
    const double q = (double)qs[l];
    const double qi = qinv[l];
    const long off = ((long)l << logN) + k;
    const TwD* Rl = Rt + (size_t)l * cxn * cyn;
    double y0[NY - 1], y1[NY - 1];
    auto load_y = [&](int c) {
        const TwD* Rc = Rl + c * cyn;
#pragma unroll
        for (int j = 0; j < NY - 1; j++) {
            const u64* p = yp[j] + (long)bb * ybs[j] + off;
            const TwD r = Rc[ycls[j + 1]];
            const double v0 = fmul_rem_r(u2d(p[0]), r.w, r.wq, q), v1 = fmul_rem_r(u2d(p[yps[j]]), r.w, r.wq, q);
            y0[j] = LAZY ? v0 : fred(v0, q, qi);
            y1[j] = LAZY ? v1 : fred(v1, q, qi);
        }
    };
    double d0[MO], d1[MO], d2[MO];
    load_y(0);
    {
        const double c0 = C0[(size_t)l * cxn];
#pragma unroll
        for (int t = 0; t < MO; t++) {
            const double* w = Wt + (size_t)(t0 + t) * nx * NY;
            double a0, a1;
            inner_sums<NY, BIG>(w, c0, y0, y1, q, qi, a0, a1);
            d0[t] = a0;
            d1[t] = a1;
            d2[t] = 0.0;
        }
    }
#pragma unroll 1
    for (int c = 1; c < cxn; c++) {
        load_y(c);
        const double c0 = C0[(size_t)l * cxn + c];
#pragma unroll 1
        for (int i = xstart[c]; i < xstart[c + 1]; i++) {
            const u64* p = xp[i - 1] + (long)bb * xbs[i - 1] + off;
            const double xa = u2d(p[0]), xb = u2d(p[xps[i - 1]]);
#pragma unroll
            for (int t = 0; t < MO; t++) {
                const double* w = Wt + ((size_t)(t0 + t) * nx + i) * NY;
                double a0, a1;
                inner_sums<NY, BIG>(w, c0, y0, y1, q, qi, a0, a1);
                const double a0q = a0 * qi, a1q = a1 * qi;
                d0[t] += fmul_rem(xa, a0, a0q, q);
                d1[t] += fmul_rem(xa, a1, a1q, q) + fmul_rem(xb, a0, a0q, q);
                d2[t] += fmul_rem(xb, a1, a1q, q);
                if constexpr (BIG) {
                    d0[t] = fred(d0[t], q, qi);
                    d1[t] = fred(d1[t], q, qi);
                    d2[t] = fred(d2[t], q, qi);
                }
            }
        }
    }
    const int ob = (bb & ~3) | ((bb - orot) & 3);
    u64* o = out + (long)ob * obs + off;
    const long pstr = (long)nl << logN;
#pragma unroll
    for (int t = 0; t < MO; t++) {
        u64* ot = o + (long)(t0 + t) * oos;
        ot[0] = fcanon(d0[t], q, qi);
        ot[pstr] = fcanon(d1[t], q, qi);
        ot[2 * pstr] = fcanon(d2[t], q, qi);
    }
}

template <int MO>
__global__ void __launch_bounds__(256, 3) k_poly2_int_split(const u64* const* __restrict__ xp, const long* __restrict__ xbs,
                        const long* __restrict__ xps, int nx, const u64* const* __restrict__ yp,
                        const long* __restrict__ ybs, const long* __restrict__ yps,
                        const int* __restrict__ xstart, const int* __restrict__ ycls, int cxn,
                        int cyn, const double* __restrict__ Wt, const TwD* __restrict__ Rt,
                        const double* __restrict__ C0, int t0, u64* __restrict__ out, long oos, long obs,
                        const u64* __restrict__ qs, const double* __restrict__ qinv, int l0, int nl,
                        int logN, int orot) {
    constexpr int NY = kPoly2Max;
    constexpr double S = 16777216.0, Si = 1.0 / 16777216.0;
    const int bx = blockIdx.x, half = (bx >> 3) & 1;
    const int k = (((bx >> 4) << 3) | (bx & 7)) * blockDim.x + threadIdx.x;
    const int l = l0 + blockIdx.y, bb = blockIdx.z;
    t0 += half * MO;
    const double q = (double)qs[l], qi = qinv[l], sq = S * qi;
    const long off = ((long)l << logN) + k;
    const TwD* Rl = Rt + (size_t)l * cxn * cyn;
    double d0[MO], d1[MO], d2[MO];
#pragma unroll
    for (int t = 0; t < MO; t++) d0[t] = d1[t] = d2[t] = 0.0;
#pragma unroll 1
    for (int p = 0; p < 2; p++) {
        double yh[NY - 1], yl[NY - 1];
#pragma unroll 1
        for (int c = 0; c < cxn; c++) {
            const TwD* Rc = Rl + c * cyn;
#pragma unroll
            for (int j = 0; j < NY - 1; j++) {
                const u64* yq = yp[j] + (long)bb * ybs[j] + off + (p ? yps[j] : 0);
                const TwD r = Rc[ycls[j + 1]];
                const double v = fred(fmul_rem_r(u2d(*yq), r.w, r.wq, q), q, qi);
                yh[j] = __builtin_rint(v * Si);
                yl[j] = __builtin_fma(-yh[j], S, v);
            }
            const double c0 = p ? 0.0 : C0[(size_t)l * cxn + c];
            const double c0h = __builtin_rint(c0 * Si), c0l = __builtin_fma(-c0h, S, c0);
#pragma unroll 1
            for (int i = xstart[c]; i < xstart[c + 1]; i++) {
                double xa = 1.0, xb = 0.0;
                if (i > 0) {
                    const u64* xq = xp[i - 1] + (long)bb * xbs[i - 1] + off;
                    xa = u2d(xq[0]);
                    xb = u2d(xq[xps[i - 1]]);
                }
#pragma unroll
                for (int t = 0; t < MO; t++) {
                    const double* w = Wt + ((size_t)(t0 + t) * nx + i) * NY;
                    double ah = w[0] * c0h, al = w[0] * c0l;
#pragma unroll
                    for (int j = 1; j < NY; j++) {
                        ah = __builtin_fma(w[j], yh[j - 1], ah);
                        al = __builtin_fma(w[j], yl[j - 1], al);
                    }
                    const double a = fmul_rem(ah, S, sq, q) + al, aq = a * qi;
                    if (i == 0) {
                        if (p == 0) d0[t] += a;
                        else d1[t] += a;
                    } else if (p == 0) {
                        d0[t] += fmul_rem(xa, a, aq, q);
                        d1[t] += fmul_rem(xb, a, aq, q);
                    } else {
                        d1[t] += fmul_rem(xa, a, aq, q);
                        d2[t] += fmul_rem(xb, a, aq, q);
                    }
                    d0[t] = fred(d0[t], q, qi);
                    d1[t] = fred(d1[t], q, qi);
                    d2[t] = fred(d2[t], q, qi);
                }
            }
        }
    }
    const int ob = (bb & ~3) | ((bb - orot) & 3);
    u64* o = out + (long)ob * obs + off;
    const long pstr = (long)nl << logN;
#pragma unroll
    for (int t = 0; t < MO; t++) {
        u64* ot = o + (long)(t0 + t) * oos;
        ot[0] = fcanon(d0[t], q, qi);
        ot[pstr] = fcanon(d1[t], q, qi);
        ot[2 * pstr] = fcanon(d2[t], q, qi);
    }
}

__global__ void k_lift0(const u64* __restrict__ x, u64* __restrict__ out, int nl, u64 q0,
                        const u64* __restrict__ qs, int logN) {
    const int k = blockIdx.x * blockDim.x + threadIdx.x;
    const int i = blockIdx.y, p = blockIdx.z;
    const u64 v = x[((long)p << logN) + k], q = qs[i];
    u64 r;
    if (v > (q0 >> 1)) {
        const u64 m = (q0 - v) % q;
        r = m ? q - m : 0;
    } else {
        r = v % q;
    }
    out[(((long)p * nl + i) << logN) + k] = r;
}

__global__ void k_dot_pt(const u64* const* __restrict__ cp, const long* __restrict__ cbs, long cps,
                         const u64* const* __restrict__ pp, int n, Out o, int np,
                         const u64* __restrict__ qs, const double* __restrict__ qinv, int logN) {
    const int k = blockIdx.x * blockDim.x + threadIdx.x;
    const int l = blockIdx.y, bb = blockIdx.z / np, p = blockIdx.z - bb * np;
    const double q = (double)qs[l], qi = qinv[l];
    const long off = ((long)l << logN) + k;
    double acc = 0.0;
    int i = 0;
    for (; i + 8 <= n; i += 8) {
        double cv[8], wv[8];
#pragma unroll
        for (int u = 0; u < 8; u++) {
            cv[u] = u2d(cp[i + u][(long)bb * cbs[i + u] + (long)p * cps + off]);
            wv[u] = u2d(pp[i + u][off]);
        }
#pragma unroll
        for (int u = 0; u < 8; u++) {
            acc += fmul_rem(cv[u], wv[u], wv[u] * qi, q);
            if ((u & 3) == 3) acc = fred(acc, q, qi);
        }
    }
    for (; i < n; i++) {
        const double c = u2d(cp[i][(long)bb * cbs[i] + (long)p * cps + off]);
        const double w = u2d(pp[i][off]);
        acc += fmul_rem(c, w, w * qi, q);
        if ((i & 3) == 3) acc = fred(acc, q, qi);
    }
    o.ptr[(long)bb * o.bs + (long)p * o.ps + off] = fcanon(acc, q, qi);
}

__device__ __forceinline__ int ext_pid(int t, int l, int Lp1) { return t <= l ? t : Lp1 + (t - l - 1); }

__global__ void k_scale_p_ext(Opnd in, u64* __restrict__ out, int l, int ne, const u64* __restrict__ qall,
                              const double* __restrict__ qinvall, const double* __restrict__ pmodf, int Lp1, int logN) {
    const int k = blockIdx.x * blockDim.x + threadIdx.x;
    const int t = blockIdx.y, bb = blockIdx.z >> 1, c = blockIdx.z & 1;
    u64 v = 0;
    if (t <= l) {
        const double q = (double)qall[t], qi = qinvall[t], f = pmodf[t];
        v = fcanon(fmul_rem(u2d(opnd_get(in, bb, c, t, k, logN)), tw_w(f, q), f, q), q, qi);
    }
    out[((((long)bb * 2 + c) * ne + t) << logN) + k] = v;
}

template <int GM, int BCT>
__global__ void k_dot_pt_ext_multi(const u64* const* __restrict__ ep, const u64* __restrict__ gal,
                                   const u64* const* __restrict__ pt, int nb,
                                   int ng, u64* const* __restrict__ outs, int l, int ne,
                                   const u64* __restrict__ qall, const double* __restrict__ qinvall, int Lp1,
                                   int logN, int nbc) {
    const int kbits = logN - 8, ngrp = nbc / BCT;
    const int x8 = blockIdx.x & 7, w = blockIdx.x >> 3;
    const int pair = (w / ngrp) * 8 + x8, bc0 = (w % ngrp) * BCT;
    if (pair >= (ne << kbits)) return;
    const int t = pair >> kbits, k = ((pair & ((1 << kbits) - 1)) << 8) + threadIdx.x;
    const int pid = ext_pid(t, l, Lp1);
    const double q = (double)qall[pid], qi = qinvall[pid];
    const long po = ((long)t << logN) + k;
    long base[BCT];
#pragma unroll
    for (int u = 0; u < BCT; u++) base[u] = ((long)(bc0 + u) * ne + t) << logN;
    const u64 M = 2ULL << logN;
    const u64 ek = 2 * (u64)(__brev((unsigned)k) >> (32 - logN)) + 1;
    double acc[BCT][GM];
#pragma unroll
    for (int u = 0; u < BCT; u++)
#pragma unroll
        for (int j = 0; j < GM; j++) acc[u][j] = 0.0;
    for (int i = 0; i < nb; i++) {
        const u64 g = gal[i];
        long src = k;
        if (g > 1) src = __brev((unsigned)((((g * ek) & (M - 1)) - 1) >> 1)) >> (32 - logN);
        double e[BCT];
#pragma unroll
        for (int u = 0; u < BCT; u++) e[u] = u2d(ep[i][base[u] + src]);
        const u64* pj[GM];
        double wv[GM];
#pragma unroll
        for (int j = 0; j < GM; j++) pj[j] = j < ng ? pt[j * nb + i] : nullptr;
#pragma unroll
        for (int j = 0; j < GM; j++) wv[j] = pj[j] ? u2d(pj[j][po]) : 0.0;
#pragma unroll
        for (int j = 0; j < GM; j++) {
            if (pj[j]) {
                const double wq = wv[j] * qi;
#pragma unroll
                for (int u = 0; u < BCT; u++) acc[u][j] += fmul_rem(e[u], wv[j], wq, q);
            }
        }
        if ((i & 3) == 3) {
#pragma unroll
            for (int u = 0; u < BCT; u++)
#pragma unroll
                for (int j = 0; j < GM; j++) acc[u][j] = fred(acc[u][j], q, qi);
        }
    }
#pragma unroll
    for (int j = 0; j < GM; j++)
        if (j < ng) {
#pragma unroll
            for (int u = 0; u < BCT; u++) outs[j][base[u] + k] = fcanon(acc[u][j], q, qi);
        }
}

template <int GM, int BM, int BB, int PB = 1, int OCC = 1>
__global__ __launch_bounds__(256, OCC) void k_bsgs_terms(const u64* __restrict__ c0p, long c0bs, const u64* __restrict__ c1p, long c1bs,
                             const u64* __restrict__ ext, long exs, long exj,
                             const u64* const* __restrict__ keys, const u64* __restrict__ gal, long kdig, long kcomp,
                             const u64* const* __restrict__ pt, int nb, int ng, u64* const* __restrict__ outs,
                             int l, int ne, int beta, int A, const u64* __restrict__ qall,
                             const double* __restrict__ qinvall, const double* __restrict__ pmodf, int Lp1, int logN,
                             int B, const unsigned short* __restrict__ kord) {
    const int nblk = 1 << (logN - 8), nbb = (B + BB - 1) / BB;
    const int x8 = blockIdx.x & 7, w = blockIdx.x >> 3;
    const int r = w / nbb, b0 = (w % nbb) * BB;
    int t, m;
    if (nblk >= 8) {
        const int seg = nblk >> 3;
        t = r / seg;
        m = x8 * seg + r - t * seg;
    } else {
        const int pos = r * 8 + x8;
        t = pos / nblk;
        m = pos - t * nblk;
    }
    if (t >= ne) return;
    const int k = ((int)kord[m] << 8) + threadIdx.x;
    const int pid = ext_pid(t, l, Lp1);
    const bool isq = t <= l;
    const int own = isq ? t / A : -1;
    const double q = (double)qall[pid], qi = qinvall[pid];
    const double pf = isq ? pmodf[t] : 0.0, pw = isq ? tw_w(pf, q) : 0.0;
    const long po = ((long)t << logN) + k;
    const u64 M = 2ULL << logN;
    const u64 ek = 2 * (u64)(__brev((unsigned)k) >> (32 - logN)) + 1;
    const u64* c0r[BB];
    const u64* c1r[BB];
    const u64* er[BB];
#pragma unroll
    for (int u = 0; u < BB; u++) {
        const int b = min(b0 + u, B - 1);
        c0r[u] = c0p + (long)b * c0bs + ((long)t << logN);
        c1r[u] = c1p + (long)b * c1bs + ((long)t << logN);
        er[u] = ext + (long)b * exs + ((long)t << logN);
    }
    double acc0[BB][GM], acc1[BB][GM];
#pragma unroll
    for (int u = 0; u < BB; u++)
#pragma unroll
        for (int j = 0; j < GM; j++) acc0[u][j] = acc1[u][j] = 0.0;
    auto pt_word = [&](int j, int i) {
        const u64* pp = j < ng ? pt[j * nb + i] : nullptr;
        return u2d(*(pp ? pp + po : &kZeroWord));
    };
    auto add_terms = [&](const double (&e0)[BB], const double (&e1)[BB], const double (&wv)[GM]) {
#pragma unroll
        for (int u = 0; u < BB; u++) {
            const double f0 = fred(e0[u], q, qi), f1 = fred(e1[u], q, qi);
#pragma unroll
            for (int j = 0; j < GM; j++) {
                const double wq = wv[j] * qi;
                acc0[u][j] += fmul_rem(f0, wv[j], wq, q);
                acc1[u][j] += fmul_rem(f1, wv[j], wq, q);
            }
        }
    };
    int i = 0;
    if (!keys[0]) {
        double wv[GM], e0[BB], e1[BB];
#pragma unroll
        for (int j = 0; j < GM; j++) wv[j] = pt_word(j, 0);
#pragma unroll
        for (int u = 0; u < BB; u++) {
            e0[u] = isq ? fmul_rem(u2d(*(isq ? c0r[u] + k : &kZeroWord)), pw, pf, q) : 0.0;
            e1[u] = isq ? fmul_rem(u2d(*(isq ? c1r[u] + k : &kZeroWord)), pw, pf, q) : 0.0;
        }
        add_terms(e0, e1, wv);
        i = 1;
    }
    int nsum = 1;
#pragma unroll 1
    for (; i < nb; i += PB) {
        double kb[PB][BM], ka[PB][BM], x[PB][BB][BM], c0v[PB][BB], wv[PB][GM];
#pragma unroll
        for (int p = 0; p < PB; p++) {
            const int ii = min(i + p, nb - 1);
            const bool live = i + p < nb;
            const u64 g = gal[ii];
            const long src = __brev((unsigned)((((g * ek) & (M - 1)) - 1) >> 1)) >> (32 - logN);
            const u64* kp = keys[ii];
#pragma unroll
            for (int d = 0; d < BM; d++) {
                const u64* kk = kp + (long)min(d, beta - 1) * kdig + ((long)pid << logN) + src;
                kb[p][d] = u2d(kk[0]);
                ka[p][d] = u2d(kk[kcomp]);
            }
#pragma unroll
            for (int j = 0; j < GM; j++) wv[p][j] = live ? pt_word(j, ii) : 0.0;
#pragma unroll
            for (int u = 0; u < BB; u++) {
#pragma unroll
                for (int d = 0; d < BM; d++)
                    x[p][u][d] = u2d(*(d == own ? c1r[u] + src : er[u] + (long)min(d, beta - 1) * exj + src));
                c0v[p][u] = u2d(*(isq ? c0r[u] + src : &kZeroWord));
            }
        }
#pragma unroll
        for (int p = 0; p < PB; p++) {
            double e0[BB], e1[BB];
#pragma unroll
            for (int u = 0; u < BB; u++) {
                double a0 = isq ? fmul_rem(c0v[p][u], pw, pf, q) : 0.0, a1 = 0.0;
#pragma unroll
                for (int d = 0; d < BM; d++) {
                    if (d < beta) {
                        a0 += fmul_rem(x[p][u][d], kb[p][d], kb[p][d] * qi, q);
                        a1 += fmul_rem(x[p][u][d], ka[p][d], ka[p][d] * qi, q);
                        if ((d & 3) == 3) {
                            a0 = fred(a0, q, qi);
                            a1 = fred(a1, q, qi);
                        }
                    }
                }
                e0[u] = a0;
                e1[u] = a1;
            }
            add_terms(e0, e1, wv[p]);
        }
        nsum += PB;
        if (nsum >= 4) {
            nsum = 0;
#pragma unroll
            for (int u = 0; u < BB; u++)
#pragma unroll
                for (int j = 0; j < GM; j++) {
                    acc0[u][j] = fred(acc0[u][j], q, qi);
                    acc1[u][j] = fred(acc1[u][j], q, qi);
                }
        }
    }
#pragma unroll
    for (int u = 0; u < BB; u++) {
        if (b0 + u >= B) break;
#pragma unroll
        for (int j = 0; j < GM; j++)
            if (j < ng) {
                u64* o = outs[j] + (((long)(2 * (b0 + u)) * ne + t) << logN) + k;
                o[0] = fcanon(acc0[u][j], q, qi);
                o[(long)ne << logN] = fcanon(acc1[u][j], q, qi);
            }
    }
}

}
```

### aes-fhe_amd/csrc/ks_fused.h

```cpp
#pragma once
#include "kernels_ops.h"
#include "ntt256f.h"

namespace aesfhe {

__device__ __forceinline__ int r8p(int e) { return e + (e >> 3); }

__device__ __forceinline__ void wave_lds_sync() {
    __builtin_amdgcn_fence(__ATOMIC_RELEASE, "wavefront");
    __builtin_amdgcn_wave_barrier();
    __builtin_amdgcn_fence(__ATOMIC_ACQUIRE, "wavefront");
}

__device__ __forceinline__ void row_ntt8_stages(double (&x)[8], double* sr, int L, int rt, const double* W, double q,
                                                double qi, bool big);
__device__ __forceinline__ void row_ntt8_fwd(double (&x)[8], const u64* rp, double* sr, int L, int rt,
                                             const double* W, double q, double qi, bool big) {
#pragma unroll
    for (int r = 0; r < 8; r++) x[r] = ld_d(&rp[L + 32 * r]);
    row_ntt8_stages(x, sr, L, rt, W, q, qi, big);
}
__device__ __forceinline__ void row_ntt8_stages(double (&x)[8], double* sr, int L, int rt, const double* W, double q,
                                                double qi, bool big) {
#pragma unroll
    for (int st = 0; st < 3; st++) {
        const int ml = 1 << st, h = 4 >> st;
        if (big && (st & 1) == 0) {
#pragma unroll
            for (int r = 0; r < 8; r++) x[r] = fred(x[r], q, qi);
        }
        const int base = ml * rt;
#pragma unroll
        for (int j = 0; j < ml; j++) {
            const double wq = W[base + j];
#pragma unroll
            for (int k = 0; k < h; k++) ct_f(x[j * 2 * h + k], x[j * 2 * h + k + h], wq, q);
        }
    }
#pragma unroll
    for (int r = 0; r < 8; r++) sr[r8p(L + 32 * r)] = x[r];
    wave_lds_sync();
    const int eb = 32 * (L >> 2) + (L & 3);
#pragma unroll
    for (int r = 0; r < 8; r++) x[r] = sr[r8p(eb + 4 * r)];
#pragma unroll
    for (int st = 3; st < 6; st++) {
        const int ml = 1 << st, h = 4 >> (st - 3), nj = ml >> 3;
        if (big && (st & 1) == 0) {
#pragma unroll
            for (int r = 0; r < 8; r++) x[r] = fred(x[r], q, qi);
        }
        const int base = ml * rt + (L >> 2) * nj;
#pragma unroll
        for (int j = 0; j < nj; j++) {
            const double wq = W[base + j];
#pragma unroll
            for (int k = 0; k < h; k++) ct_f(x[j * 2 * h + k], x[j * 2 * h + k + h], wq, q);
        }
    }
    wave_lds_sync();
#pragma unroll
    for (int r = 0; r < 8; r++) sr[r8p(eb + 4 * r)] = x[r];
    wave_lds_sync();
#pragma unroll
    for (int r = 0; r < 8; r++) x[r] = sr[r8p(8 * L + r)];
    if (big) {
#pragma unroll
        for (int r = 0; r < 8; r++) x[r] = fred(x[r], q, qi);
    }
    {
        const int base = 64 * rt + 2 * L;
        const double w0 = W[base], w1 = W[base + 1];
        ct_f(x[0], x[2], w0, q);
        ct_f(x[1], x[3], w0, q);
        ct_f(x[4], x[6], w1, q);
        ct_f(x[5], x[7], w1, q);
    }
    {
        const int base = 128 * rt + 4 * L;
#pragma unroll
        for (int j = 0; j < 4; j++) ct_f(x[2 * j], x[2 * j + 1], W[base + j], q);
    }
    wave_lds_sync();
#pragma unroll
    for (int r = 0; r < 8; r++) sr[r8p(8 * L + r)] = big ? fred(x[r], q, qi) : x[r];
    wave_lds_sync();
#pragma unroll
    for (int r = 0; r < 8; r++) x[r] = sr[r8p(L + 32 * r)];
    wave_lds_sync();
}

__device__ __forceinline__ void row_intt8(double (&x)[8], double* sr, int L, const double* W, double q, double qi,
                                          bool big) {
    auto gs = [&](double& a, double& b, double wq) {
        if (big) gs_f<true>(a, b, wq, q, qi);
        else gs_f<false>(a, b, wq, q, qi);
    };
#pragma unroll
    for (int r = 0; r < 8; r++) sr[r8p(L + 32 * r)] = x[r];
    wave_lds_sync();
#pragma unroll
    for (int r = 0; r < 8; r++) x[r] = sr[r8p(8 * L + r)];
#pragma unroll
    for (int j = 0; j < 4; j++) gs(x[2 * j], x[2 * j + 1], W[128 + 4 * L + j]);
    {
        const double w0 = W[64 + 2 * L], w1 = W[64 + 2 * L + 1];
        gs(x[0], x[2], w0);
        gs(x[1], x[3], w0);
        gs(x[4], x[6], w1);
        gs(x[5], x[7], w1);
    }
    wave_lds_sync();
#pragma unroll
    for (int r = 0; r < 8; r++) sr[r8p(8 * L + r)] = x[r];
    wave_lds_sync();
    const int eb = 32 * (L >> 2) + (L & 3);
#pragma unroll
    for (int r = 0; r < 8; r++) x[r] = sr[r8p(eb + 4 * r)];
#pragma unroll
    for (int st = 5; st >= 3; st--) {
        const int ml = 1 << st, h = 4 >> (st - 3), nj = ml >> 3;
        const int base = ml + (L >> 2) * nj;
#pragma unroll
        for (int j = 0; j < nj; j++) {
            const double wq = W[base + j];
#pragma unroll
            for (int k = 0; k < h; k++) gs(x[j * 2 * h + k], x[j * 2 * h + k + h], wq);
        }
    }
    wave_lds_sync();
#pragma unroll
    for (int r = 0; r < 8; r++) sr[r8p(eb + 4 * r)] = x[r];
    wave_lds_sync();
#pragma unroll
    for (int r = 0; r < 8; r++) x[r] = sr[r8p(L + 32 * r)];
#pragma unroll
    for (int st = 2; st >= 0; st--) {
        const int ml = 1 << st, h = 4 >> st;
#pragma unroll
        for (int j = 0; j < ml; j++) {
            const double wq = W[ml + j];
#pragma unroll
            for (int k = 0; k < h; k++) gs(x[j * 2 * h + k], x[j * 2 * h + k + h], wq);
        }
    }
    wave_lds_sync();
}

template <bool FMA>
__device__ __forceinline__ void ks_prod_prologue(double (&a0)[8], double (&a1)[8], const u64* kp, long kcomp,
                                                 const u64* xa, long aps, const u64* xb, long bps, const u64* xc,
                                                 long cps, bool has_c, double wv, double f, double fal, double fC,
                                                 double fK, double q, double qi, bool big) {
    double x0[8], x1[8], y0[8], y1[8], kb[8], ka[8];
#pragma unroll
    for (int r = 0; r < 8; r++) {
        x0[r] = u2d(xa[32 * r]);
        x1[r] = u2d(xa[aps + 32 * r]);
        y0[r] = u2d(xb[32 * r]);
        y1[r] = u2d(xb[bps + 32 * r]);
        kb[r] = u2d(kp[32 * r]);
        ka[r] = u2d(kp[32 * r + kcomp]);
    }
#pragma unroll
    for (int r = 0; r < 8; r++) {
        const double y0q = y0[r] * qi, y1q = y1[r] * qi;
        double p0 = fmul_rem(x0[r], y0[r], y0q, q);
        double p1 = fmul_rem(x0[r], y1[r], y1q, q) + fmul_rem(x1[r], y0[r], y0q, q);
        double p2 = fmul_rem(x1[r], y1[r], y1q, q);
        if constexpr (FMA) {
            p0 = fmul_rem(p0, fal, fal * qi, q) + fK;
            p1 = fmul_rem(p1, fal, fal * qi, q);
            p2 = fmul_rem(p2, fal, fal * qi, q);
            if (has_c) {
                p0 += fmul_rem(u2d(xc[32 * r]), fC, fC * qi, q);
                p1 += fmul_rem(u2d(xc[cps + 32 * r]), fC, fC * qi, q);
            }
        }
        a0[r] = fmul_rem(p0, wv, f, q) + fmul_rem(p2, kb[r], kb[r] * qi, q);
        a1[r] = fmul_rem(p1, wv, f, q) + fmul_rem(p2, ka[r], ka[r] * qi, q);
        if (big) {
            a0[r] = fred(a0[r], q, qi);
            a1[r] = fred(a1[r], q, qi);
        }
    }
}

struct KsFin {
    const u64* conv;
    long cbs, cps;
    u64* out;
    long obs, ops;
    const double* dinvf;
    Opnd2 add;
};
template <int G, int R = 256, bool PROD = false, int EPI = 0>
__global__ __launch_bounds__(256, 4) void k_nttf_rows_ks(const u64* __restrict__ d, long dbs,
                                                      const u64* __restrict__ ext, long exs, long exj,
                                                      const u64* __restrict__ key, long kdig, long kcomp,
                                                      u64* __restrict__ acc, long abs_, long acs, int B,
                                                      int beta, int K, int l, int ne, Tabs T, Opnd addend,
                                                      const double* __restrict__ pmodf, int accum, Opnd pb,
                                                      const u64* __restrict__ fac, Opnd pc, int t0, int nt,
                                                      KsFin fin) {
    static_assert(G == 1 && !PROD && EPI == 0, "the accumulating giants' kernel: the other forms are k_nttf_rows_ks_p's");
    __shared__ double s[8 * 288 + 8 * 256];
    const int nbg = (B + G - 1) / G;
    const int id = blockIdx.x, x8 = id & 7, rest = id >> 3;
    const int b0 = (rest % nbg) * G, pair = (rest / nbg) * 8 + x8;
    constexpr int RB = R / 8;
    constexpr int LOGN = R == 256 ? 16 : 17;
    const int tq = pair / RB, rb = pair - tq * RB;
    if (tq >= nt) return;
    const int t = t0 + tq;
    const int pid = t <= l ? t : T.Lp1 + (t - l - 1);
    const int own = t <= l ? t / K : -1;
    const int tid = threadIdx.x, L = tid & 31, rl = tid >> 5;
    const int row = rb * 8 + rl;
    const double q = (double)T.q[pid], qi = T.qinv[pid];
    const bool big = q >= kBigPrime;
    const double* W = T.psif + ((long)pid << LOGN);
    double* sr = s + rl * 288;
    double* tw = s + 8 * 288 + rl * 256;
#pragma unroll
    for (int m = 0; m < 8; m++) {
        const int e = L + 32 * m;
        if (e > 0) {
            const int ml = 1 << (31 - __clz(e));
            tw[e] = W[(long)ml * (R + row) + (e - ml)];
        }
    }
    wave_lds_sync();
    const long roff = ((long)t << LOGN) + (long)row * 256 + L;
    double a0[G][8], a1[G][8];
#pragma unroll
    for (int g = 0; g < G; g++) {
        const int bb = b0 + g;
#pragma unroll
        for (int r = 0; r < 8; r++) a0[g][r] = a1[g][r] = 0.0;
        if (bb >= B) continue;
        if (pmodf && t <= l && addend.ptr) {
            const double f = pmodf[t], w = tw_w(f, q);
            const u64* xa = addend.ptr + (long)bb * addend.bs + roff;
            if (addend.np > 0) {
#pragma unroll
                for (int r = 0; r < 8; r++) a0[g][r] = fmul_rem(u2d(xa[32 * r]), w, f, q);
            }
            if (addend.np > 1) {
#pragma unroll
                for (int r = 0; r < 8; r++) a1[g][r] = fmul_rem(u2d(xa[addend.ps + 32 * r]), w, f, q);
            }
        }
        if (accum) {
            const u64* o0 = acc + (long)bb * abs_ + roff;
#pragma unroll
            for (int r = 0; r < 8; r++) {
                a0[g][r] = fred(a0[g][r] + u2d(o0[32 * r]), q, qi);
                a1[g][r] = fred(a1[g][r] + u2d(o0[acs + 32 * r]), q, qi);
            }
        }
    }
    int nsum = 0;
#pragma unroll 1
    for (int j = 0; j < beta; j++) {
        const u64* kp = key + (long)j * kdig + ((long)pid << LOGN) + (long)row * 256 + L;
        u64 kbw[8], kaw[8];
#pragma unroll
        for (int r = 0; r < 8; r++) {
            kbw[r] = kp[32 * r];
            kaw[r] = kp[32 * r + kcomp];
        }
#pragma unroll
        for (int g = 0; g < G; g++) {
            const int bb = b0 + g;
            if (bb >= B) break;
            double v[8];
            if (j == own) {
                const u64* dp = d + (long)bb * dbs + roff;
#pragma unroll
                for (int r = 0; r < 8; r++) v[r] = u2d(dp[32 * r]);
            } else {
                row_ntt8_fwd(v, ext + (long)j * exj + (long)bb * exs + ((long)t << LOGN) + (long)row * 256, sr, L, 1,
                             tw, q, qi, big);
            }
#pragma unroll
            for (int r = 0; r < 8; r++) {
                const double kb = u2d(kbw[r]), ka = u2d(kaw[r]);
                a0[g][r] += fmul_rem(v[r], kb, kb * qi, q);
                a1[g][r] += fmul_rem(v[r], ka, ka * qi, q);
            }
        }
        if (big && (++nsum & 3) == 0) {
#pragma unroll
            for (int g = 0; g < G; g++)
#pragma unroll
                for (int r = 0; r < 8; r++) {
                    a0[g][r] = fred(a0[g][r], q, qi);
                    a1[g][r] = fred(a1[g][r], q, qi);
                }
        }
    }
#pragma unroll
    for (int g = 0; g < G; g++) {
        const int bb = b0 + g;
        if (bb >= B) break;
        u64* o0 = acc + (long)bb * abs_ + roff;
#pragma unroll
        for (int r = 0; r < 8; r++) {
            __builtin_nontemporal_store(fcanon(a0[g][r], q, qi), &o0[32 * r]);
            __builtin_nontemporal_store(fcanon(a1[g][r], q, qi), &o0[acs + 32 * r]);
        }
    }
}

typedef __attribute__((address_space(3))) void ks_lds_void;
__device__ __forceinline__ void ks_dma_rows(const u64* g, double* lds_wave, int lane) {
#pragma unroll
    for (int k = 0; k < 4; k++)
        __builtin_amdgcn_global_load_lds((const void*)(g + 128 * k + 2 * lane), (ks_lds_void*)(lds_wave + 128 * k), 16, 0, 0);
}
__device__ __forceinline__ void ks_dma_wait() {
    asm volatile("s_waitcnt vmcnt(0)" ::: "memory");
    __builtin_amdgcn_wave_barrier();
}
__device__ __forceinline__ void ks_lds_reads_done() {
    asm volatile("s_waitcnt lgkmcnt(0)" ::: "memory");
    __builtin_amdgcn_wave_barrier();
}

template <int R = 256, bool PROD = false, int EPI = 0>
__global__ __launch_bounds__(256, 3) void k_nttf_rows_ks_p(const u64* __restrict__ d, long dbs,
                                                      const u64* __restrict__ ext, long exs, long exj,
                                                      const u64* __restrict__ key, long kdig, long kcomp,
                                                      u64* __restrict__ acc, long abs_, long acs, int B,
                                                      int beta, int K, int l, int ne, Tabs T, Opnd addend,
                                                      const double* __restrict__ pmodf, int accum, Opnd pb,
                                                      const u64* __restrict__ fac, Opnd pc, int t0, int nt,
                                                      KsFin fin) {
    static_assert(EPI == 1 || EPI == 2, "FIN or INV: the canonical accumulators are k_nttf_rows_ks's");
    constexpr bool FIN = EPI == 1;
    __shared__ double s[8 * 288 + 8 * 256 + 8 * 256];
    const int id = blockIdx.x, x8 = id & 7, rest = id >> 3;
    const int bb = rest % B, pair = (rest / B) * 8 + x8;
    constexpr int RB = R / 8;
    constexpr int LOGN = R == 256 ? 16 : 17;
    const int tq = pair / RB, rb = pair - tq * RB;
    if (tq >= nt) return;
    const int t = t0 + tq;
    const int pid = t <= l ? t : T.Lp1 + (t - l - 1);
    const int own = t <= l ? t / K : -1;
    const int tid = threadIdx.x, L = tid & 31, rl = tid >> 5, lane = tid & 63, w = tid >> 6;
    const int row = rb * 8 + rl;
    const double q = (double)T.q[pid], qi = T.qinv[pid];
    const bool big = q >= kBigPrime;
    const double* W = T.psif + ((long)pid << LOGN);
    double* sr = s + rl * 288;
    double* tw = s + 8 * 288 + rl * 256;
    double* ebw = s + 8 * 288 + 8 * 256 + w * 512;
    const double* er = ebw + (rl & 1) * 256;
    const long woff = ((long)t << LOGN) + (long)(rb * 8 + 2 * w) * 256;
    auto next_digit = [&](int j) {
        for (j++; j < beta && j == own; j++) {
        }
        return j;
    };
    int jn = next_digit(-1);
    if (jn < beta) ks_dma_rows(ext + (long)jn * exj + (long)bb * exs + woff, ebw, lane);
#pragma unroll
    for (int m = 0; m < 8; m++) {
        const int e = L + 32 * m;
        if (e > 0) {
            const int ml = 1 << (31 - __clz(e));
            tw[e] = W[(long)ml * (R + row) + (e - ml)];
        }
    }
    const long roff = ((long)t << LOGN) + (long)row * 256 + L;
    double a0[8], a1[8];
#pragma unroll
    for (int r = 0; r < 8; r++) a0[r] = a1[r] = 0.0;
    if (PROD && t <= l) {
        const double f = pmodf[t], wv = tw_w(f, q);
        const u64* kp = key + (long)own * kdig + ((long)pid << LOGN) + (long)row * 256 + L;
        const u64* xa = addend.ptr + (long)(bb & addend.bmask) * addend.bs + roff;
        const u64* xb = pb.ptr + (long)(bb & pb.bmask) * pb.bs + roff;
        const u64* xc = pc.ptr ? pc.ptr + (long)(bb & pc.bmask) * pc.bs + roff : xb;
        if (fac)
            ks_prod_prologue<true>(a0, a1, kp, kcomp, xa, addend.ps, xb, pb.ps, xc, pc.ps, pc.ptr != nullptr, wv, f,
                                   (double)fac[3 * t], (double)fac[3 * t + 1], (double)fac[3 * t + 2], q, qi, big);
        else
            ks_prod_prologue<false>(a0, a1, kp, kcomp, xa, addend.ps, xb, pb.ps, xc, pc.ps, false, wv, f, 0.0, 0.0, 0.0,
                                    q, qi, big);
    } else if (!PROD) {
        if (pmodf && t <= l && addend.ptr) {
            const double f = pmodf[t], wv = tw_w(f, q);
            const u64* xa = addend.ptr + (long)bb * addend.bs + roff;
            if (addend.np > 0) {
#pragma unroll
                for (int r = 0; r < 8; r++) a0[r] = fmul_rem(u2d(xa[32 * r]), wv, f, q);
            }
            if (addend.np > 1) {
#pragma unroll
                for (int r = 0; r < 8; r++) a1[r] = fmul_rem(u2d(xa[addend.ps + 32 * r]), wv, f, q);
            }
        }
        if (own >= 0 && own < beta) {
            const u64* kp = key + (long)own * kdig + ((long)pid << LOGN) + (long)row * 256 + L;
            const u64* dp = d + (long)bb * dbs + roff;
#pragma unroll
            for (int r = 0; r < 8; r++) {
                const double v = u2d(dp[32 * r]), kb = u2d(kp[32 * r]), ka = u2d(kp[32 * r + kcomp]);
                a0[r] += fmul_rem(v, kb, kb * qi, q);
                a1[r] += fmul_rem(v, ka, ka * qi, q);
            }
        }
    }
    if (accum) {
        const u64* o0 = acc + (long)bb * abs_ + roff;
#pragma unroll
        for (int r = 0; r < 8; r++) {
            a0[r] = fred(a0[r] + u2d(o0[32 * r]), q, qi);
            a1[r] = fred(a1[r] + u2d(o0[acs + 32 * r]), q, qi);
        }
    } else if (big) {
#pragma unroll
        for (int r = 0; r < 8; r++) {
            a0[r] = fred(a0[r], q, qi);
            a1[r] = fred(a1[r], q, qi);
        }
    }
    wave_lds_sync();
    int nsum = 0;
    const long coff = ((long)t << LOGN) + (long)(rb * 8 + 2 * w) * 256;
#pragma unroll 1
    while (jn < beta) {
        const int j = jn;
        ks_dma_wait();
        double v[8];
#pragma unroll
        for (int r = 0; r < 8; r++) v[r] = er[L + 32 * r];
        ks_lds_reads_done();
        jn = next_digit(j);
        if (jn < beta) ks_dma_rows(ext + (long)jn * exj + (long)bb * exs + woff, ebw, lane);
        else if (FIN) ks_dma_rows(fin.conv + (long)bb * fin.cbs + coff, ebw, lane);
        const u64* kp = key + (long)j * kdig + ((long)pid << LOGN) + (long)row * 256 + L;
        u64 kbw[8], kaw[8];
#pragma unroll
        for (int r = 0; r < 8; r++) {
            kbw[r] = kp[32 * r];
            kaw[r] = kp[32 * r + kcomp];
        }
        row_ntt8_stages(v, sr, L, 1, tw, q, qi, big);
#pragma unroll
        for (int r = 0; r < 8; r++) {
            const double kb = u2d(kbw[r]), ka = u2d(kaw[r]);
            a0[r] += fmul_rem(v[r], kb, kb * qi, q);
            a1[r] += fmul_rem(v[r], ka, ka * qi, q);
        }
        if (big && (++nsum & 3) == 0) {
#pragma unroll
            for (int r = 0; r < 8; r++) {
                a0[r] = fred(a0[r], q, qi);
                a1[r] = fred(a1[r], q, qi);
            }
        }
    }
    if constexpr (FIN) {
        const double f = fin.dinvf[t], wv = tw_w(f, q);
        if (beta == 0 || next_digit(-1) >= beta)
            ks_dma_rows(fin.conv + (long)bb * fin.cbs + coff, ebw, lane);
#pragma unroll 1
        for (int c = 0; c < 2; c++) {
            ks_dma_wait();
            double cv[8];
#pragma unroll
            for (int r = 0; r < 8; r++) cv[r] = er[L + 32 * r];
            ks_lds_reads_done();
            if (c == 0) ks_dma_rows(fin.conv + (long)bb * fin.cbs + fin.cps + coff, ebw, lane);
            row_ntt8_stages(cv, sr, L, 1, tw, q, qi, big);
            const u64* ap = fin.add.ptr && c < fin.add.np ? fin.add.ptr + (long)bb * fin.add.bs + (long)c * fin.add.ps + roff
                                                          : nullptr;
            u64* op = fin.out + (long)bb * fin.obs + (long)c * fin.ops + roff;
#pragma unroll
            for (int r = 0; r < 8; r++) {
                double a = c ? a1[r] : a0[r];
                if (big) a = fred(a, q, qi);
                double v = fmul_rem(a - cv[r], wv, f, q);
                if (ap) v += u2d(ap[32 * r]);
                __builtin_nontemporal_store(fcanon(v, q, qi), &op[32 * r]);
            }
        }
        return;
    }
    const double* IW = T.ipsif + ((long)pid << LOGN);
#pragma unroll
    for (int m = 0; m < 8; m++) {
        const int e = L + 32 * m;
        if (e > 0) {
            const int ml = 1 << (31 - __clz(e));
            tw[e] = IW[(long)ml * (R + row) + (e - ml)];
        }
    }
    wave_lds_sync();
    u64* o0 = acc + (long)bb * abs_ + roff;
#pragma unroll
    for (int c = 0; c < 2; c++) {
        double x[8];
#pragma unroll
        for (int r = 0; r < 8; r++) x[r] = fred(c ? a1[r] : a0[r], q, qi);
        row_intt8(x, sr, L, tw, q, qi, big);
#pragma unroll
        for (int r = 0; r < 8; r++) st_d(&o0[(long)c * acs + 32 * r], x[r]);
    }
}

}
```

### aes-fhe_amd/csrc/ntt256f.h

```cpp
#pragma once
#include <type_traits>

#include "kernels.h"

namespace aesfhe {


__device__ __forceinline__ void ct_f(double& x, double& y, double wq, double q) {
    const double v = fmul_rem(y, tw_w(wq, q), wq, q);
    const double t = x;
    x = t + v;
    y = t - v;
}
template <bool FOLD>
__device__ __forceinline__ void gs_f(double& x, double& y, double wq, double q, double qi) {
    const double s = x + y, d = x - y;
    x = FOLD ? fred(s, q, qi) : s;
    y = fmul_rem(d, tw_w(wq, q), wq, q);
}
__device__ __forceinline__ void ct_fw(double& x, double& y, double w, double wq, double q) {
    const double v = fmul_rem(y, w, wq, q);
    const double t = x;
    x = t + v;
    y = t - v;
}
template <bool FOLD>
__device__ __forceinline__ void gs_fw(double& x, double& y, double w, double wq, double q, double qi) {
    const double s = x + y, d = x - y;
    x = FOLD ? fred(s, q, qi) : s;
    y = fmul_rem(d, w, wq, q);
}
__device__ __forceinline__ void tw_row(const double* W, int idx, double rq, double q, double qi,
                                       double& w, double& wq) {
    w = fmul_rem(tw_w(W[idx], q), tw_w(rq, q), rq, q);
    wq = w * qi;
}
__device__ __forceinline__ double ld_d(const u64* p) { return __longlong_as_double((long long)*p); }
__device__ __forceinline__ void st_d(u64* p, double v) { __builtin_nontemporal_store((u64)__double_as_longlong(v), p); }

constexpr int kPadF = 17;

__device__ __forceinline__ void wave_sync_lds() {
    __builtin_amdgcn_fence(__ATOMIC_RELEASE, "wavefront");
    __builtin_amdgcn_wave_barrier();
    __builtin_amdgcn_fence(__ATOMIC_ACQUIRE, "wavefront");
}

struct SpreadSrc {
    const u64* x;
    long xs;
    u64 ql, sc;
    double scf;
};
template <int R, int SPREAD = 0>
__device__ __forceinline__ void nttf_fwd_cols_body(const Span& src, const Span& dst, const Tabs& T, int bx, int by,
                                                   double* s, double* twq, const SpreadSrc& ss = SpreadSrc{}) {
    static_assert(R == 256 || R == 512, "rows of 256: N = 2^16 or 2^17");
    constexpr int H = R / 256;
    int pid;
    const u64* in = SPREAD ? ss.x + (long)(by / dst.nl) * ss.xs : span_ptr(src, by, T.logN, T.Lp1, pid);
    u64* out = span_ptr(dst, by, T.logN, T.Lp1, pid);
    const int tid = threadIdx.x, cl = tid & 15, b = tid >> 4;
    const int c = bx * 16 + cl;
    const double q = (double)T.q[pid], qi = T.qinv[pid];
    const bool big = q >= kBigPrime;
    const double* tg = T.psif + ((long)pid << T.logN);
    const double* cw = T.cw + (long)pid * kColW;
#pragma unroll
    for (int h = 0; h < H; h++) twq[tid + 256 * h] = tg[tid + 256 * h];
    double x[16 * H];
#pragma unroll
    for (int h = 0; h < H; h++)
#pragma unroll
        for (int a = 0; a < 16; a++) {
            const u64 v = in[(h * 256 + a * 16 + b) * 256 + c];
            if constexpr (SPREAD == 0) {
                x[16 * h + a] = u2d(v);
            } else {
                const u64 w = SPREAD == 2 ? mul_w(v, ss.sc, ss.scf, ss.ql) : v;
                double d = u2d(w) - (SPREAD != 3 && w > (ss.ql >> 1) ? (double)ss.ql : 0.0);
                d = fred(d, q, qi);
                x[16 * h + a] = d < 0.0 ? d + q : d;
            }
        }
    __syncthreads();
    if (H == 2) {
        const double w = cw[1], wq = tg[1];
#pragma unroll
        for (int a = 0; a < 16; a++) ct_fw(x[a], x[16 + a], w, wq, q);
    }
#pragma unroll
    for (int h = 0; h < H; h++) {
        double* xh = x + 16 * h;
        const int mul = H == 1 ? 1 : 2 + h;
#pragma unroll
        for (int st = 0; st < 4; st++) {
            const int m = 1 << st, hh = 8 >> st;
            if (big && (H == 1 ? st == 2 : (st & 1) == 0)) {
#pragma unroll
                for (int a = 0; a < 16; a++) xh[a] = fred(xh[a], q, qi);
            }
#pragma unroll
            for (int a = 0; a < 16; a++) {
                if (a & hh) continue;
                const int ti = m * mul + (a >> (4 - st));
                ct_fw(xh[a], xh[a + hh], cw[ti], tg[ti], q);
            }
        }
        if (h > 0) __syncthreads();
#pragma unroll
        for (int a = 0; a < 16; a++) s[(a * 16 + b) * kPadF + cl] = xh[a];
        __syncthreads();
        const int ap = b;
#pragma unroll
        for (int bb = 0; bb < 16; bb++) xh[bb] = s[(ap * 16 + bb) * kPadF + cl];
#pragma unroll
        for (int st = 4; st < 8; st++) {
            const int m = 1 << st, hh = 128 >> st;
            if (big && (st & 1) == 0) {
#pragma unroll
                for (int bb = 0; bb < 16; bb++) xh[bb] = fred(xh[bb], q, qi);
            }
#pragma unroll
            for (int bb = 0; bb < 16; bb++) {
                if (bb & hh) continue;
                ct_f(xh[bb], xh[bb + hh], twq[m * mul + ap * (m >> 4) + (bb >> (8 - st))], q);
            }
        }
#pragma unroll
        for (int bb = 0; bb < 16; bb++) st_d(&out[(h * 256 + ap * 16 + bb) * 256 + c], xh[bb]);
    }
}
template <int R = 256>
__global__ __launch_bounds__(256) void k_nttf_fwd_cols(Span src, Span dst, Tabs T) {
    __shared__ double s[256 * kPadF];
    __shared__ double twq[R];
    nttf_fwd_cols_body<R>(src, dst, T, blockIdx.x, blockIdx.y, s, twq);
}
template <int R, int SPREAD>
__global__ __launch_bounds__(256) void k_nttf_fwd_cols_spread(SpreadSrc ss, Span dst, Tabs T) {
    __shared__ double s[256 * kPadF];
    __shared__ double twq[R];
    nttf_fwd_cols_body<R, SPREAD>(dst, dst, T, blockIdx.x, blockIdx.y, s, twq, ss);
}

struct RowFin {
    const u64* acc;
    long abs_, acs;
    Opnd2 addend;
    u64* out;
    long obs, ops;
    const double* dinvf;
    int nl;
    const double* cf;
};

__device__ __forceinline__ void row_ntt_load(double (&x)[16], const u64* rp, int b) {
#pragma unroll
    for (int a = 0; a < 16; a++) x[a] = ld_d(&rp[a * 16 + b]);
}
template <int RR>
__device__ __forceinline__ void row_ntt_fwd_stages(double (&x)[16], double* sr, int b, int row,
                                                   const double* W, const double* R, double q, double qi,
                                                   bool big) {
#pragma unroll
    for (int st = 0; st < 4; st++) {
        const int ml = 1 << st, h = 8 >> st;
        if (big && (st & 1) == 0) {
#pragma unroll
            for (int a = 0; a < 16; a++) x[a] = fred(x[a], q, qi);
        }
        const double rq = R[st];
#pragma unroll
        for (int j = 0; j < ml; j++) {
            double w, wq;
            tw_row(W, RR * ml + j, rq, q, qi, w, wq);
#pragma unroll
            for (int k = 0; k < h; k++) ct_fw(x[j * 2 * h + k], x[j * 2 * h + k + h], w, wq, q);
        }
    }
#pragma unroll
    for (int a = 0; a < 16; a++) sr[a * kPadF + b] = x[a];
    wave_sync_lds();
    const int ap = b;
#pragma unroll
    for (int bb = 0; bb < 16; bb++) x[bb] = sr[ap * kPadF + bb];
#pragma unroll
    for (int st = 4; st < 8; st++) {
        const int ml = 1 << st, h = 128 >> st, nj = ml >> 4;
        if (big && (st & 1) == 0) {
#pragma unroll
            for (int bb = 0; bb < 16; bb++) x[bb] = fred(x[bb], q, qi);
        }
        const double rq = R[st];
#pragma unroll
        for (int j = 0; j < nj; j++) {
            double w, wq;
            tw_row(W, RR * ml + ap * nj + j, rq, q, qi, w, wq);
#pragma unroll
            for (int k = 0; k < h; k++) ct_fw(x[j * 2 * h + k], x[j * 2 * h + k + h], w, wq, q);
        }
    }
}
template <int RR>
__device__ __forceinline__ void row_ntt_fwd(double (&x)[16], const u64* rp, double* sr, int b, int row,
                                            const double* W, const double* R, double q, double qi,
                                            bool big) {
    row_ntt_load(x, rp, b);
    row_ntt_fwd_stages<RR>(x, sr, b, row, W, R, q, qi, big);
}
__device__ __forceinline__ int row_tile_idx(int e) {
    const int r = e >> 8, cc = e & 255;
    return r * 16 * kPadF + (cc >> 4) * kPadF + (cc & 15);
}

template <bool FIN, int R>
__device__ __forceinline__ void nttf_fwd_rows_body(const Span& dst, const Tabs& T, const RowFin& fin, int bx, int by,
                                                   double* s) {
    int pid;
    u64* io = span_ptr(dst, by, T.logN, T.Lp1, pid);
    const int tid = threadIdx.x, b = tid & 15, rl = tid >> 4;
    const int row = bx * 16 + rl;
    const double q = (double)T.q[pid], qi = T.qinv[pid];
    const bool big = q >= kBigPrime;
    const double* W = T.psif + ((long)pid << T.logN);
    const double* Rf = T.rtwf + (long)pid * R * 8 + row * 8;
    double x[16];
    double* sr = s + rl * 16 * kPadF;
    const int ap = b;
    const int e0 = (tid >> 6) * 1024 + (tid & 63);
    row_ntt_load(x, io + (long)row * 256, b);
    u64 accw[FIN ? 16 : 1];
    if (FIN) {
        const int p = by / fin.nl, i = by - p * fin.nl;
        const u64* apf = fin.acc + (long)(p >> 1) * fin.abs_ + (long)(p & 1) * fin.acs + ((long)i << T.logN) +
                         (long)bx * 16 * 256;
#pragma unroll
        for (int k = 0; k < (FIN ? 16 : 1); k++) accw[k] = apf[e0 + 64 * k];
    }
    row_ntt_fwd_stages<R>(x, sr, b, row, W, Rf, q, qi, big);
#pragma unroll
    for (int bb = 0; bb < 16; bb++) sr[ap * kPadF + bb] = __longlong_as_double((long long)fcanon(x[bb], q, qi));
    wave_sync_lds();
    if (!FIN) {
        u64* base = io + (long)bx * 16 * 256;
#pragma unroll
        for (int k = 0; k < 16; k++) {
            const int e = e0 + 64 * k;
            __builtin_nontemporal_store((u64)__double_as_longlong(s[row_tile_idx(e)]), &base[e]);
        }
    } else {
        const int y = by, p = y / fin.nl, i = y - p * fin.nl, bb = p >> 1, c = p & 1;
        const long off = ((long)i << T.logN) + (long)bx * 16 * 256;
        const u64* dp = fin.addend.ptr && c < fin.addend.np ? fin.addend.ptr + (long)bb * fin.addend.bs + (long)c * fin.addend.ps + off : nullptr;
        u64* op = fin.out + (long)bb * fin.obs + (long)c * fin.ops + off;
        const double f = fin.dinvf[i], w = tw_w(f, q);
        const double cf = fin.cf ? fin.cf[i] : 0.0, cw = fin.cf ? tw_w(cf, q) : 0.0;
#pragma unroll
        for (int k = 0; k < 16; k++) {
            const int e = e0 + 64 * k;
            const double conv = u2d((u64)__double_as_longlong(s[row_tile_idx(e)]));
            double a = u2d(accw[FIN ? k : 0]);
            if (fin.cf) a = fmul_rem(a, cw, cf, q);
            double v = fmul_rem(a - conv, w, f, q);
            if (dp) v += u2d(dp[e]);
            __builtin_nontemporal_store(fcanon(v, q, qi), &op[e]);
        }
    }
}
template <bool FIN, int R = 256>
__global__ __launch_bounds__(256) void k_nttf_fwd_rows_t(Span dst, Tabs T, RowFin fin) {
    __shared__ double s[16 * 16 * kPadF];
    nttf_fwd_rows_body<FIN, R>(dst, T, fin, blockIdx.x, blockIdx.y, s);
}

template <int RR = 256, bool PROD = false, bool FMA = false>
__global__ __launch_bounds__(256, 4) void k_nttf_inv_rows(Span src, Span dst, Tabs T, Span src2,
                                                          const u64* __restrict__ fac) {
    __shared__ double s[16 * 16 * kPadF];
    int pid;
    const u64* in = span_ptr(src, blockIdx.y, T.logN, T.Lp1, pid);
    u64* out = span_ptr(dst, blockIdx.y, T.logN, T.Lp1, pid);
    const int tid = threadIdx.x, b = tid & 15, rl = tid >> 4;
    const int row = blockIdx.x * 16 + rl;
    const double q = (double)T.q[pid], qi = T.qinv[pid];
    const bool big = q >= kBigPrime;
    const double* W = T.ipsif + ((long)pid << T.logN);
    const u64* gb = in + (long)blockIdx.x * 16 * 256;
    {
        const int e0 = (tid >> 6) * 1024 + (tid & 63);
        if (PROD) {
            int pid2;
            const u64* gb2 = span_ptr(src2, blockIdx.y, T.logN, T.Lp1, pid2) + (long)blockIdx.x * 16 * 256;
            const double al = FMA ? (double)fac[3 * pid] : 0.0;
#pragma unroll
            for (int k = 0; k < 16; k++) {
                const int e = e0 + 64 * k;
                const double y = u2d(gb2[e]);
                double v = fmul_rem(u2d(gb[e]), y, y * qi, q);
                if (FMA) v = fmul_rem(v, al, al * qi, q);
                s[row_tile_idx(e)] = u2d(fcanon(v, q, qi));
            }
        } else {
#pragma unroll
            for (int k = 0; k < 16; k++) {
                const int e = e0 + 64 * k;
                s[row_tile_idx(e)] = u2d(gb[e]);
            }
        }
    }
    wave_sync_lds();
    double* sr = s + rl * 16 * kPadF;
    const int ap = b;
    double x[16];
#pragma unroll
    for (int bb = 0; bb < 16; bb++) x[bb] = sr[ap * kPadF + bb];
    const double* R = T.irtwf + (long)pid * RR * 8 + row * 8;
    auto stages_lo = [&](auto fold) {
#pragma unroll
        for (int st = 0; st < 4; st++) {
            const int t = 1 << st, ml = 128 / t, nj = 8 / t;
            const double rq = R[7 - st];
#pragma unroll
            for (int j = 0; j < nj; j++) {
                double w, wq;
                tw_row(W, RR * ml + ap * nj + j, rq, q, qi, w, wq);
#pragma unroll
                for (int k = 0; k < t; k++)
                    gs_fw<decltype(fold)::value>(x[j * 2 * t + k], x[j * 2 * t + k + t], w, wq, q, qi);
            }
        }
    };
    if (big) stages_lo(std::true_type{});
    else stages_lo(std::false_type{});
#pragma unroll
    for (int bb = 0; bb < 16; bb++) sr[ap * kPadF + bb] = x[bb];
    wave_sync_lds();
#pragma unroll
    for (int a = 0; a < 16; a++) x[a] = sr[a * kPadF + b];
    auto stages_hi = [&](auto fold) {
#pragma unroll
        for (int st = 4; st < 8; st++) {
            const int t = 1 << st, ta = t >> 4, ml = 128 / t;
            const double rq = R[7 - st];
#pragma unroll
            for (int j = 0; j < ml; j++) {
                double w, wq;
                tw_row(W, RR * ml + j, rq, q, qi, w, wq);
#pragma unroll
                for (int k = 0; k < ta; k++)
                    gs_fw<decltype(fold)::value>(x[j * 2 * ta + k], x[j * 2 * ta + k + ta], w, wq, q, qi);
            }
        }
    };
    if (big) stages_hi(std::true_type{});
    else stages_hi(std::false_type{});
    u64* op = out + (long)row * 256;
#pragma unroll
    for (int a = 0; a < 16; a++) st_d(&op[a * 16 + b], x[a]);
}

template <int R = 256, bool LF = false>
__global__ __launch_bounds__(256) void k_nttf_inv_cols(Span dst, Tabs T, const double* __restrict__ lf) {
    static_assert(R == 256 || R == 512, "rows of 256: N = 2^16 or 2^17");
    constexpr int H = R / 256;
    __shared__ double s[256 * kPadF];
    __shared__ double twq[R];
    int pid;
    u64* io = span_ptr(dst, blockIdx.y, T.logN, T.Lp1, pid);
    const int tid = threadIdx.x, cl = tid & 15, b = tid >> 4;
    const int c = blockIdx.x * 16 + cl;
    const double q = (double)T.q[pid], qi = T.qinv[pid];
    const bool big = q >= kBigPrime;
    const double* tg = T.ipsif + ((long)pid << T.logN);
    const double* icw = T.icw + (long)pid * kColW;
#pragma unroll
    for (int h = 0; h < H; h++) twq[tid + 256 * h] = tg[tid + 256 * h];
    const int ap = b;
    double x[16 * H];
#pragma unroll
    for (int h = 0; h < H; h++)
#pragma unroll
        for (int bb = 0; bb < 16; bb++) x[16 * h + bb] = fred(ld_d(&io[(h * 256 + ap * 16 + bb) * 256 + c]), q, qi);
    __syncthreads();
#pragma unroll
    for (int h = 0; h < H; h++) {
        double* xh = x + 16 * h;
        const int mul = H == 1 ? 1 : 2 + h;
        auto stages_lo = [&](auto fold) {
#pragma unroll
            for (int st = 0; st < 4; st++) {
                const int tr = 1 << st;
                const int base = (128 / tr) * mul + ap * (8 / tr);
#pragma unroll
                for (int bb = 0; bb < 16; bb++) {
                    if (bb & tr) continue;
                    gs_f<decltype(fold)::value>(xh[bb], xh[bb + tr], twq[base + (bb >> (st + 1))], q, qi);
                }
            }
        };
        if (big) stages_lo(std::true_type{});
        else stages_lo(std::false_type{});
        if (h > 0) __syncthreads();
#pragma unroll
        for (int bb = 0; bb < 16; bb++) s[(ap * 16 + bb) * kPadF + cl] = xh[bb];
        __syncthreads();
#pragma unroll
        for (int a = 0; a < 16; a++) xh[a] = s[(a * 16 + b) * kPadF + cl];
        auto stages_hi = [&](auto fold) {
#pragma unroll
            for (int st = 4; st < 8; st++) {
                const int tr = 1 << st, ta = tr >> 4;
                const int base = (128 / tr) * mul;
#pragma unroll
                for (int a = 0; a < 16; a++) {
                    if (a & ta) continue;
                    const int ti = base + (a >> (st - 3));
                    gs_fw<decltype(fold)::value>(xh[a], xh[a + ta], icw[ti], tg[ti], q, qi);
                }
            }
        };
        if (big) stages_hi(std::true_type{});
        else stages_hi(std::false_type{});
    }
    if (H == 2) {
        const double w = icw[1], wq = tg[1];
#pragma unroll
        for (int a = 0; a < 16; a++) {
            x[a] = fred(x[a], q, qi);
            x[16 + a] = fred(x[16 + a], q, qi);
            gs_fw<false>(x[a], x[16 + a], w, wq, q, qi);
        }
    }
    const double nif = LF ? lf[blockIdx.y % dst.nl] : T.ninvf[pid];
    const double ni = LF ? tw_w(nif, q) : (double)T.ninv[pid];
#pragma unroll
    for (int h = 0; h < H; h++)
#pragma unroll
        for (int a = 0; a < 16; a++) {
            const double r = fred(x[16 * h + a], q, qi);
            __builtin_nontemporal_store(fcanon(fmul_rem(r, ni, nif, q), q, qi), &io[(h * 256 + a * 16 + b) * 256 + c]);
        }
}


}
```

Before: 283,500.

## Store raw twiddles and compute modular-multiply quotient from q inverse

Twiddle tables now hold the raw root values in double instead of precomputed w/q ratios. Butterflies and key/weight multiplies use a new fmul_remq that forms the product a*w first and multiplies it by 1/q to estimate the quotient. This drops the separate cw/icw column twiddle tables and the per-element kbq/kaq precomputation, which cuts table loads, LDS traffic and register pressure. In exchange each multiply has one more dependent operation, and the rounding behaviour of the reduction changes.

```diff
diff --git a/aes-fhe_amd/csrc/bconv_cols.h b/aes-fhe_amd/csrc/bconv_cols.h
--- a/aes-fhe_amd/csrc/bconv_cols.h
+++ b/aes-fhe_amd/csrc/bconv_cols.h
@@ -5,8 +5,7 @@
 namespace aesfhe {
 
 __device__ __forceinline__ void cols256_stages_store(double (&x)[16], double q, double qi, bool big, const double* tg,
-                                                     const double* cw, const double* twq, double* s, u64* out, int b,
-                                                     int cl, int c) {
+                                                     const double* tws, double* s, u64* out, int b, int cl, int c) {
 #pragma unroll
     for (int st = 0; st < 4; st++) {
         const int m = 1 << st, hh = 8 >> st;
@@ -18,7 +17,7 @@
         for (int a = 0; a < 16; a++) {
             if (a & hh) continue;
             const int ti = m + (a >> (4 - st));
-            ct_fw(x[a], x[a + hh], cw[ti], tg[ti], q);
+            ct_f(x[a], x[a + hh], tg[ti], q, qi);
         }
     }
 #pragma unroll
@@ -37,7 +36,7 @@
 #pragma unroll
         for (int bb = 0; bb < 16; bb++) {
             if (bb & hh) continue;
-            ct_f(x[bb], x[bb + hh], twq[m + ap * (m >> 4) + (bb >> (8 - st))], q);
+            ct_f(x[bb], x[bb + hh], tws[m + ap * (m >> 4) + (bb >> (8 - st))], q, qi);
         }
     }
 #pragma unroll
@@ -49,7 +48,7 @@
     static_assert(TT == 4 || TT == 2, "4 or 2 targets per workgroup");
     static_assert(LT == 1 || LT == 2, "1 or 2 LDS tiles");
     __shared__ double s[LT][256 * kPadF];
-    __shared__ double twq[TT][256];
+    __shared__ double tws[TT][256];
     const int tid = threadIdx.x, lane = tid & 63, w = tid >> 6, c = lane & 31, h = lane >> 5;
     const int cl = tid & 15, b = tid >> 4;
     const int id = blockIdx.x, x8 = id & 7, j = id >> 3;
@@ -64,7 +63,7 @@
     const int nlive = min(TT, a.nt - tau0);
 #pragma unroll
     for (int m = 0; m < TT; m++)
-        if (m < nlive) twq[m][tid] = T.psif[((long)pid_of(limb_of(tau0 + m)) << logN) + tid];
+        if (m < nlive) tws[m][tid] = T.psid[((long)pid_of(limb_of(tau0 + m)) << logN) + tid];
     bc_v4i af[NSTEP];
     {
         const int row = lane & 31, ta = row >> 3, pb = (row & 3) + 4 * ((row >> 2) & 1);
@@ -207,8 +206,8 @@
         if (LT == 1 && m > 0) __syncthreads();
         const int tl = limb_of(tau0 + m), pid = pid_of(tl);
         const double q = (double)T.q[pid], qi = T.qinv[pid];
-        cols256_stages_store(xv[m], q, qi, q >= kBigPrime, T.psif + ((long)pid << logN), T.cw + (long)pid * kColW,
-                             twq[m], s[m % LT], dst + ((long)tl << logN), b, cl, bx * 16 + cl);
+        cols256_stages_store(xv[m], q, qi, q >= kBigPrime, T.psid + ((long)pid << logN), tws[m], s[m % LT],
+                             dst + ((long)tl << logN), b, cl, bx * 16 + cl);
     }
 }
 
diff --git a/aes-fhe_amd/csrc/engine.hip b/aes-fhe_amd/csrc/engine.hip
--- a/aes-fhe_amd/csrc/engine.hip
+++ b/aes-fhe_amd/csrc/engine.hip
@@ -567,7 +567,7 @@
     const int N = e->N, np = e->np, L = e->L, K = e->K, Lp1 = e->Lp1;
     const auto& Q = e->chain.q;
     std::vector<u64> hq(Q), hpsi((size_t)np * N), hipsi((size_t)np * N), hninv(np);
-    std::vector<double> hqinv(np), hpsif((size_t)np * N), hipsif((size_t)np * N), hninvf(np);
+    std::vector<double> hqinv(np), hpsid((size_t)np * N), hipsid((size_t)np * N), hninvf(np);
     e->h_iroot.resize(np);
     for (int p = 0; p < np; p++) {
         u64 qq = Q[p];
@@ -583,8 +583,8 @@
             unsigned r = bit_reverse((unsigned)k, e->logN);
             hpsi[(size_t)p * N + k] = pw[r];
             hipsi[(size_t)p * N + k] = ipw[r];
-            hpsif[(size_t)p * N + k] = (double)pw[r] / (double)qq;
-            hipsif[(size_t)p * N + k] = (double)ipw[r] / (double)qq;
+            hpsid[(size_t)p * N + k] = (double)pw[r];
+            hipsid[(size_t)p * N + k] = (double)ipw[r];
         }
         e->h_iroot[p] = pw[N / 2];
         hninv[p] = h_invmod((u64)N, qq);
@@ -595,9 +595,9 @@
     t.q = e->q = dev.up(hq);
     t.qinv = e->qinv = dev.up(hqinv);
     t.psi = dev.up(hpsi);
-    t.psif = dev.up(hpsif);
+    t.psid = dev.up(hpsid);
     t.ipsi = dev.up(hipsi);
-    t.ipsif = dev.up(hipsif);
+    t.ipsid = dev.up(hipsid);
     t.ninv = dev.up(hninv);
     t.ninvf = dev.up(hninvf);
     if (fused_ntt(e)) {
@@ -606,30 +606,21 @@
         for (int p = 0; p < np; p++)
             for (int row = 0; row < R; row++)
                 for (int sh = 0; sh < 8; sh++) {
-                    hr[((size_t)p * R + row) * 8 + sh] = hpsif[(size_t)p * N + (row << sh)];
-                    hir[((size_t)p * R + row) * 8 + sh] = hipsif[(size_t)p * N + (row << sh)];
+                    hr[((size_t)p * R + row) * 8 + sh] = hpsid[(size_t)p * N + (row << sh)];
+                    hir[((size_t)p * R + row) * 8 + sh] = hipsid[(size_t)p * N + (row << sh)];
                 }
-        t.rtwf = dev.up(hr);
-        t.irtwf = dev.up(hir);
+        t.rtwd = dev.up(hr);
+        t.irtwd = dev.up(hir);
     }
     {
         std::vector<Tw> htw((size_t)np * N), hitw((size_t)np * N);
         for (size_t i = 0; i < htw.size(); i++) {
-            htw[i] = Tw{hpsi[i], hpsif[i]};
-            hitw[i] = Tw{hipsi[i], hipsif[i]};
+            const double qq = (double)Q[i / (size_t)N];
+            htw[i] = Tw{hpsi[i], (double)hpsi[i] / qq};
+            hitw[i] = Tw{hipsi[i], (double)hipsi[i] / qq};
         }
         t.tw = dev.up(htw);
         t.itw = dev.up(hitw);
-    }
-    {
-        std::vector<double> hcw((size_t)np * kColW), hicw((size_t)np * kColW);
-        for (int p = 0; p < np; p++)
-            for (int k = 0; k < kColW; k++) {
-                hcw[(size_t)p * kColW + k] = (double)hpsi[(size_t)p * N + (k < N ? k : 0)];
-                hicw[(size_t)p * kColW + k] = (double)hipsi[(size_t)p * N + (k < N ? k : 0)];
-            }
-        t.cw = dev.up(hcw);
-        t.icw = dev.up(hicw);
     }
     t.logN = e->logN;
     t.Lp1 = Lp1;
diff --git a/aes-fhe_amd/csrc/kernels.h b/aes-fhe_amd/csrc/kernels.h
--- a/aes-fhe_amd/csrc/kernels.h
+++ b/aes-fhe_amd/csrc/kernels.h
@@ -52,6 +52,13 @@
 }
 __device__ __forceinline__ double fmul_rem_r(double a, double w, double wq, double q) {
     return fmul_rem(a, w, wq, q);
+}
+__device__ __forceinline__ double fmul_remq(double a, double w, double qi, double q) {
+    const double p = a * w;
+    const double pl = __builtin_fma(a, w, -p);
+    const double qh = __builtin_rint(p * qi);
+    const double u = __builtin_fma(-qh, q, p);
+    return u + pl;
 }
 __device__ __forceinline__ double fred(double x, double q, double qinv) {
     const double qh = __builtin_rint(x * qinv);
@@ -92,23 +99,19 @@
     return s.base + (long)(p & s.pmask) * s.pstride + ((long)l << logN);
 }
 
-constexpr int kColW = 64;
-
 struct Tabs {
     const u64* q;
     const double* qinv;
     const u64* psi;
-    const double* psif;
+    const double* psid;
     const u64* ipsi;
-    const double* ipsif;
-    const double* rtwf;
-    const double* irtwf;
+    const double* ipsid;
+    const double* rtwd;
+    const double* irtwd;
     const u64* ninv;
     const double* ninvf;
     const struct Tw* tw;
     const struct Tw* itw;
-    const double* cw;
-    const double* icw;
     int logN;
     int Lp1;
 };
@@ -130,8 +133,7 @@
     u64* out = span_ptr(dst, blockIdx.y, T.logN, T.Lp1, pid);
     const int c0 = blockIdx.x * CW;
     const u64 q = T.q[pid];
-    const u64* W = T.psi + ((long)pid << T.logN);
-    const double* Wf = T.psif + ((long)pid << T.logN);
+    const Tw* W = T.tw + ((long)pid << T.logN);
     for (int e = threadIdx.x; e < R1 * CW; e += 256) {
         int r = e / CW, c = e - r * CW;
         s[e] = in[r * kC2 + c0 + c];
@@ -141,8 +143,9 @@
         for (int bf = threadIdx.x; bf < (R1 / 2) * CW; bf += 256) {
             int c = bf % CW, g = bf / CW;
             int i = g / t, r1 = i * 2 * t + (g - i * t), r2 = r1 + t;
-            u64 w = W[m + i];
-            double wf = Wf[m + i];
+            const Tw tw = W[m + i];
+            u64 w = tw.w;
+            double wf = tw.wq;
             u64 U = s[r1 * CW + c];
             u64 V = mul_w(s[r2 * CW + c], w, wf, q);
             s[r1 * CW + c] = add_m(U, V, q);
@@ -164,8 +167,7 @@
     u64* io = span_ptr(dst, blockIdx.y, T.logN, T.Lp1, pid);
     const int row0 = blockIdx.x * RW;
     const u64 q = T.q[pid];
-    const u64* W = T.psi + ((long)pid << T.logN);
-    const double* Wf = T.psif + ((long)pid << T.logN);
+    const Tw* W = T.tw + ((long)pid << T.logN);
     u64* base = io + (long)row0 * kC2;
     for (int e = threadIdx.x; e < RW * kC2; e += 256) s[e] = base[e];
     __syncthreads();
@@ -174,8 +176,9 @@
             int rl = bf / (kC2 / 2), g = bf - rl * (kC2 / 2);
             int i = g / t, c1 = i * 2 * t + (g - i * t), c2 = c1 + t;
             int widx = R1 * ml + (row0 + rl) * ml + i;
-            u64 w = W[widx];
-            double wf = Wf[widx];
+            const Tw tw = W[widx];
+            u64 w = tw.w;
+            double wf = tw.wq;
             u64* rowp = s + rl * kC2;
             u64 U = rowp[c1];
             u64 V = mul_w(rowp[c2], w, wf, q);
@@ -196,8 +199,7 @@
     u64* out = span_ptr(dst, blockIdx.y, T.logN, T.Lp1, pid);
     const int row0 = blockIdx.x * RW;
     const u64 q = T.q[pid];
-    const u64* W = T.ipsi + ((long)pid << T.logN);
-    const double* Wf = T.ipsif + ((long)pid << T.logN);
+    const Tw* W = T.itw + ((long)pid << T.logN);
     const int N = 1 << T.logN;
     for (int e = threadIdx.x; e < RW * kC2; e += 256) s[e] = in[(long)row0 * kC2 + e];
     __syncthreads();
@@ -210,7 +212,8 @@
             u64* rowp = s + rl * kC2;
             u64 U = rowp[c1], V = rowp[c2];
             rowp[c1] = add_m(U, V, q);
-            rowp[c2] = mul_w(sub_m(U, V, q), W[widx], Wf[widx], q);
+            const Tw tw = W[widx];
+            rowp[c2] = mul_w(sub_m(U, V, q), tw.w, tw.wq, q);
         }
         __syncthreads();
     }
@@ -225,8 +228,7 @@
     u64* io = span_ptr(dst, blockIdx.y, T.logN, T.Lp1, pid);
     const int c0 = blockIdx.x * CW;
     const u64 q = T.q[pid];
-    const u64* W = T.ipsi + ((long)pid << T.logN);
-    const double* Wf = T.ipsif + ((long)pid << T.logN);
+    const Tw* W = T.itw + ((long)pid << T.logN);
     for (int e = threadIdx.x; e < R1 * CW; e += 256) {
         int r = e / CW, c = e - r * CW;
         s[e] = io[r * kC2 + c0 + c];
@@ -239,7 +241,8 @@
             int i = g / tr, r1 = i * 2 * tr + (g - i * tr), r2 = r1 + tr;
             u64 U = s[r1 * CW + c], V = s[r2 * CW + c];
             s[r1 * CW + c] = add_m(U, V, q);
-            s[r2 * CW + c] = mul_w(sub_m(U, V, q), W[hg + i], Wf[hg + i], q);
+            const Tw tw = W[hg + i];
+            s[r2 * CW + c] = mul_w(sub_m(U, V, q), tw.w, tw.wq, q);
         }
         __syncthreads();
     }
diff --git a/aes-fhe_amd/csrc/kernels_ops.h b/aes-fhe_amd/csrc/kernels_ops.h
--- a/aes-fhe_amd/csrc/kernels_ops.h
+++ b/aes-fhe_amd/csrc/kernels_ops.h
@@ -311,16 +311,14 @@
     const double q = (double)qall[pid];
     const double qi = qinvall[pid];
     const int own = t <= l ? t / K : -1;
-    double kb[BM], ka[BM], kbq[BM], kaq[BM];
+    double kb[BM], ka[BM];
 #pragma unroll
     for (int j = 0; j < BM; j++) {
-        kb[j] = ka[j] = kbq[j] = kaq[j] = 0.0;
+        kb[j] = ka[j] = 0.0;
         if (j < beta) {
             const long ko = (long)j * kdig + ((long)pid << logN) + k;
             kb[j] = u2d(key[ko]);
             ka[j] = u2d(key[ko + kcomp]);
-            kbq[j] = kb[j] * qi;
-            kaq[j] = ka[j] * qi;
         }
     }
 #pragma unroll 4
@@ -331,8 +329,8 @@
             if (j < beta) {
                 const double e = u2d((j == own) ? d[(long)bb * dbs + ((long)t << logN) + k]
                                                 : ext[(long)j * exj + (long)bb * exs + ((long)t << logN) + k]);
-                s0 += fmul_rem(e, kb[j], kbq[j], q);
-                s1 += fmul_rem(e, ka[j], kaq[j], q);
+                s0 += fmul_remq(e, kb[j], qi, q);
+                s1 += fmul_remq(e, ka[j], qi, q);
                 if ((j & 3) == 3) {
                     s0 = fred(s0, q, qi);
                     s1 = fred(s1, q, qi);
@@ -401,8 +399,8 @@
 #pragma unroll
                 for (int j = 0; j < BM; j++) {
                     if (j < beta) {
-                        s0 += fmul_rem(e[j], kb[ii][j], kb[ii][j] * qi, q);
-                        s1 += fmul_rem(e[j], ka[ii][j], ka[ii][j] * qi, q);
+                        s0 += fmul_remq(e[j], kb[ii][j], qi, q);
+                        s1 += fmul_remq(e[j], ka[ii][j], qi, q);
                         if ((j & 3) == 3) {
                             s0 = fred(s0, q, qi);
                             s1 = fred(s1, q, qi);
@@ -1057,14 +1055,14 @@
         }
 #pragma unroll
         for (int u = 0; u < 8; u++) {
-            acc += fmul_rem(cv[u], wv[u], wv[u] * qi, q);
+            acc += fmul_remq(cv[u], wv[u], qi, q);
             if ((u & 3) == 3) acc = fred(acc, q, qi);
         }
     }
     for (; i < n; i++) {
         const double c = u2d(cp[i][(long)bb * cbs[i] + (long)p * cps + off]);
         const double w = u2d(pp[i][off]);
-        acc += fmul_rem(c, w, w * qi, q);
+        acc += fmul_remq(c, w, qi, q);
         if ((i & 3) == 3) acc = fred(acc, q, qi);
     }
     o.ptr[(long)bb * o.bs + (long)p * o.ps + off] = fcanon(acc, q, qi);
@@ -1124,9 +1122,8 @@
 #pragma unroll
         for (int j = 0; j < GM; j++) {
             if (pj[j]) {
-                const double wq = wv[j] * qi;
-#pragma unroll
-                for (int u = 0; u < BCT; u++) acc[u][j] += fmul_rem(e[u], wv[j], wq, q);
+#pragma unroll
+                for (int u = 0; u < BCT; u++) acc[u][j] += fmul_remq(e[u], wv[j], qi, q);
             }
         }
         if ((i & 3) == 3) {
@@ -1200,9 +1197,8 @@
             const double f0 = fred(e0[u], q, qi), f1 = fred(e1[u], q, qi);
 #pragma unroll
             for (int j = 0; j < GM; j++) {
-                const double wq = wv[j] * qi;
-                acc0[u][j] += fmul_rem(f0, wv[j], wq, q);
-                acc1[u][j] += fmul_rem(f1, wv[j], wq, q);
+                acc0[u][j] += fmul_remq(f0, wv[j], qi, q);
+                acc1[u][j] += fmul_remq(f1, wv[j], qi, q);
             }
         }
     };
@@ -1255,8 +1251,8 @@
 #pragma unroll
                 for (int d = 0; d < BM; d++) {
                     if (d < beta) {
-                        a0 += fmul_rem(x[p][u][d], kb[p][d], kb[p][d] * qi, q);
-                        a1 += fmul_rem(x[p][u][d], ka[p][d], ka[p][d] * qi, q);
+                        a0 += fmul_remq(x[p][u][d], kb[p][d], qi, q);
+                        a1 += fmul_remq(x[p][u][d], ka[p][d], qi, q);
                         if ((d & 3) == 3) {
                             a0 = fred(a0, q, qi);
                             a1 = fred(a1, q, qi);
diff --git a/aes-fhe_amd/csrc/ks_fused.h b/aes-fhe_amd/csrc/ks_fused.h
--- a/aes-fhe_amd/csrc/ks_fused.h
+++ b/aes-fhe_amd/csrc/ks_fused.h
@@ -32,9 +32,9 @@
         const int base = ml * rt;
 #pragma unroll
         for (int j = 0; j < ml; j++) {
-            const double wq = W[base + j];
-#pragma unroll
-            for (int k = 0; k < h; k++) ct_f(x[j * 2 * h + k], x[j * 2 * h + k + h], wq, q);
+            const double w = W[base + j];
+#pragma unroll
+            for (int k = 0; k < h; k++) ct_f(x[j * 2 * h + k], x[j * 2 * h + k + h], w, q, qi);
         }
     }
 #pragma unroll
@@ -53,9 +53,9 @@
         const int base = ml * rt + (L >> 2) * nj;
 #pragma unroll
         for (int j = 0; j < nj; j++) {
-            const double wq = W[base + j];
-#pragma unroll
-            for (int k = 0; k < h; k++) ct_f(x[j * 2 * h + k], x[j * 2 * h + k + h], wq, q);
+            const double w = W[base + j];
+#pragma unroll
+            for (int k = 0; k < h; k++) ct_f(x[j * 2 * h + k], x[j * 2 * h + k + h], w, q, qi);
         }
     }
     wave_lds_sync();
@@ -71,15 +71,15 @@
     {
         const int base = 64 * rt + 2 * L;
         const double w0 = W[base], w1 = W[base + 1];
-        ct_f(x[0], x[2], w0, q);
-        ct_f(x[1], x[3], w0, q);
-        ct_f(x[4], x[6], w1, q);
-        ct_f(x[5], x[7], w1, q);
+        ct_f(x[0], x[2], w0, q, qi);
+        ct_f(x[1], x[3], w0, q, qi);
+        ct_f(x[4], x[6], w1, q, qi);
+        ct_f(x[5], x[7], w1, q, qi);
     }
     {
         const int base = 128 * rt + 4 * L;
 #pragma unroll
-        for (int j = 0; j < 4; j++) ct_f(x[2 * j], x[2 * j + 1], W[base + j], q);
+        for (int j = 0; j < 4; j++) ct_f(x[2 * j], x[2 * j + 1], W[base + j], q, qi);
     }
     wave_lds_sync();
 #pragma unroll
@@ -92,9 +92,9 @@
 
 __device__ __forceinline__ void row_intt8(double (&x)[8], double* sr, int L, const double* W, double q, double qi,
                                           bool big) {
-    auto gs = [&](double& a, double& b, double wq) {
-        if (big) gs_f<true>(a, b, wq, q, qi);
-        else gs_f<false>(a, b, wq, q, qi);
+    auto gs = [&](double& a, double& b, double w) {
+        if (big) gs_f<true>(a, b, w, q, qi);
+        else gs_f<false>(a, b, w, q, qi);
     };
 #pragma unroll
     for (int r = 0; r < 8; r++) sr[r8p(L + 32 * r)] = x[r];
@@ -123,9 +123,9 @@
         const int base = ml + (L >> 2) * nj;
 #pragma unroll
         for (int j = 0; j < nj; j++) {
-            const double wq = W[base + j];
-#pragma unroll
-            for (int k = 0; k < h; k++) gs(x[j * 2 * h + k], x[j * 2 * h + k + h], wq);
+            const double w = W[base + j];
+#pragma unroll
+            for (int k = 0; k < h; k++) gs(x[j * 2 * h + k], x[j * 2 * h + k + h], w);
         }
     }
     wave_lds_sync();
@@ -139,9 +139,9 @@
         const int ml = 1 << st, h = 4 >> st;
 #pragma unroll
         for (int j = 0; j < ml; j++) {
-            const double wq = W[ml + j];
-#pragma unroll
-            for (int k = 0; k < h; k++) gs(x[j * 2 * h + k], x[j * 2 * h + k + h], wq);
+            const double w = W[ml + j];
+#pragma unroll
+            for (int k = 0; k < h; k++) gs(x[j * 2 * h + k], x[j * 2 * h + k + h], w);
         }
     }
     wave_lds_sync();
@@ -164,21 +164,20 @@
     }
 #pragma unroll
     for (int r = 0; r < 8; r++) {
-        const double y0q = y0[r] * qi, y1q = y1[r] * qi;
-        double p0 = fmul_rem(x0[r], y0[r], y0q, q);
-        double p1 = fmul_rem(x0[r], y1[r], y1q, q) + fmul_rem(x1[r], y0[r], y0q, q);
-        double p2 = fmul_rem(x1[r], y1[r], y1q, q);
+        double p0 = fmul_remq(x0[r], y0[r], qi, q);
+        double p1 = fmul_remq(x0[r], y1[r], qi, q) + fmul_remq(x1[r], y0[r], qi, q);
+        double p2 = fmul_remq(x1[r], y1[r], qi, q);
         if constexpr (FMA) {
-            p0 = fmul_rem(p0, fal, fal * qi, q) + fK;
-            p1 = fmul_rem(p1, fal, fal * qi, q);
-            p2 = fmul_rem(p2, fal, fal * qi, q);
+            p0 = fmul_remq(p0, fal, qi, q) + fK;
+            p1 = fmul_remq(p1, fal, qi, q);
+            p2 = fmul_remq(p2, fal, qi, q);
             if (has_c) {
-                p0 += fmul_rem(u2d(xc[32 * r]), fC, fC * qi, q);
-                p1 += fmul_rem(u2d(xc[cps + 32 * r]), fC, fC * qi, q);
-            }
-        }
-        a0[r] = fmul_rem(p0, wv, f, q) + fmul_rem(p2, kb[r], kb[r] * qi, q);
-        a1[r] = fmul_rem(p1, wv, f, q) + fmul_rem(p2, ka[r], ka[r] * qi, q);
+                p0 += fmul_remq(u2d(xc[32 * r]), fC, qi, q);
+                p1 += fmul_remq(u2d(xc[cps + 32 * r]), fC, qi, q);
+            }
+        }
+        a0[r] = fmul_rem(p0, wv, f, q) + fmul_remq(p2, kb[r], qi, q);
+        a1[r] = fmul_rem(p1, wv, f, q) + fmul_remq(p2, ka[r], qi, q);
         if (big) {
             a0[r] = fred(a0[r], q, qi);
             a1[r] = fred(a1[r], q, qi);
@@ -219,7 +218,7 @@
     const int row = rb * 8 + rl;
     const double q = (double)T.q[pid], qi = T.qinv[pid];
     const bool big = q >= kBigPrime;
-    const double* W = T.psif + ((long)pid << LOGN);
+    const double* W = T.psid + ((long)pid << LOGN);
     double* sr = s + rl * 288;
     double* tw = s + 8 * 288 + rl * 256;
 #pragma unroll
@@ -286,8 +285,8 @@
 #pragma unroll
             for (int r = 0; r < 8; r++) {
                 const double kb = u2d(kbw[r]), ka = u2d(kaw[r]);
-                a0[g][r] += fmul_rem(v[r], kb, kb * qi, q);
-                a1[g][r] += fmul_rem(v[r], ka, ka * qi, q);
+                a0[g][r] += fmul_remq(v[r], kb, qi, q);
+                a1[g][r] += fmul_remq(v[r], ka, qi, q);
             }
         }
         if (big && (++nsum & 3) == 0) {
@@ -353,7 +352,7 @@
     const int row = rb * 8 + rl;
     const double q = (double)T.q[pid], qi = T.qinv[pid];
     const bool big = q >= kBigPrime;
-    const double* W = T.psif + ((long)pid << LOGN);
+    const double* W = T.psid + ((long)pid << LOGN);
     double* sr = s + rl * 288;
     double* tw = s + 8 * 288 + rl * 256;
     double* ebw = s + 8 * 288 + 8 * 256 + w * 512;
@@ -409,8 +408,8 @@
 #pragma unroll
             for (int r = 0; r < 8; r++) {
                 const double v = u2d(dp[32 * r]), kb = u2d(kp[32 * r]), ka = u2d(kp[32 * r + kcomp]);
-                a0[r] += fmul_rem(v, kb, kb * qi, q);
-                a1[r] += fmul_rem(v, ka, ka * qi, q);
+                a0[r] += fmul_remq(v, kb, qi, q);
+                a1[r] += fmul_remq(v, ka, qi, q);
             }
         }
     }
@@ -453,8 +452,8 @@
 #pragma unroll
         for (int r = 0; r < 8; r++) {
             const double kb = u2d(kbw[r]), ka = u2d(kaw[r]);
-            a0[r] += fmul_rem(v[r], kb, kb * qi, q);
-            a1[r] += fmul_rem(v[r], ka, ka * qi, q);
+            a0[r] += fmul_remq(v[r], kb, qi, q);
+            a1[r] += fmul_remq(v[r], ka, qi, q);
         }
         if (big && (++nsum & 3) == 0) {
 #pragma unroll
@@ -491,7 +490,7 @@
         }
         return;
     }
-    const double* IW = T.ipsif + ((long)pid << LOGN);
+    const double* IW = T.ipsid + ((long)pid << LOGN);
 #pragma unroll
     for (int m = 0; m < 8; m++) {
         const int e = L + 32 * m;
diff --git a/aes-fhe_amd/csrc/ntt256f.h b/aes-fhe_amd/csrc/ntt256f.h
--- a/aes-fhe_amd/csrc/ntt256f.h
+++ b/aes-fhe_amd/csrc/ntt256f.h
@@ -6,34 +6,20 @@
 namespace aesfhe {
 
 
-__device__ __forceinline__ void ct_f(double& x, double& y, double wq, double q) {
-    const double v = fmul_rem(y, tw_w(wq, q), wq, q);
+__device__ __forceinline__ void ct_f(double& x, double& y, double w, double q, double qi) {
+    const double v = fmul_remq(y, w, qi, q);
     const double t = x;
     x = t + v;
     y = t - v;
 }
 template <bool FOLD>
-__device__ __forceinline__ void gs_f(double& x, double& y, double wq, double q, double qi) {
+__device__ __forceinline__ void gs_f(double& x, double& y, double w, double q, double qi) {
     const double s = x + y, d = x - y;
     x = FOLD ? fred(s, q, qi) : s;
-    y = fmul_rem(d, tw_w(wq, q), wq, q);
-}
-__device__ __forceinline__ void ct_fw(double& x, double& y, double w, double wq, double q) {
-    const double v = fmul_rem(y, w, wq, q);
-    const double t = x;
-    x = t + v;
-    y = t - v;
-}
-template <bool FOLD>
-__device__ __forceinline__ void gs_fw(double& x, double& y, double w, double wq, double q, double qi) {
-    const double s = x + y, d = x - y;
-    x = FOLD ? fred(s, q, qi) : s;
-    y = fmul_rem(d, w, wq, q);
-}
-__device__ __forceinline__ void tw_row(const double* W, int idx, double rq, double q, double qi,
-                                       double& w, double& wq) {
-    w = fmul_rem(tw_w(W[idx], q), tw_w(rq, q), rq, q);
-    wq = w * qi;
+    y = fmul_remq(d, w, qi, q);
+}
+__device__ __forceinline__ double tw_row(const double* W, int idx, double rw, double q, double qi) {
+    return fmul_remq(W[idx], rw, qi, q);
 }
 __device__ __forceinline__ double ld_d(const u64* p) { return __longlong_as_double((long long)*p); }
 __device__ __forceinline__ void st_d(u64* p, double v) { __builtin_nontemporal_store((u64)__double_as_longlong(v), p); }
@@ -54,7 +40,7 @@
 };
 template <int R, int SPREAD = 0>
 __device__ __forceinline__ void nttf_fwd_cols_body(const Span& src, const Span& dst, const Tabs& T, int bx, int by,
-                                                   double* s, double* twq, const SpreadSrc& ss = SpreadSrc{}) {
+                                                   double* s, double* tws, const SpreadSrc& ss = SpreadSrc{}) {
     static_assert(R == 256 || R == 512, "rows of 256: N = 2^16 or 2^17");
     constexpr int H = R / 256;
     int pid;
@@ -64,10 +50,9 @@
     const int c = bx * 16 + cl;
     const double q = (double)T.q[pid], qi = T.qinv[pid];
     const bool big = q >= kBigPrime;
-    const double* tg = T.psif + ((long)pid << T.logN);
-    const double* cw = T.cw + (long)pid * kColW;
-#pragma unroll
-    for (int h = 0; h < H; h++) twq[tid + 256 * h] = tg[tid + 256 * h];
+    const double* tg = T.psid + ((long)pid << T.logN);
+#pragma unroll
+    for (int h = 0; h < H; h++) tws[tid + 256 * h] = tg[tid + 256 * h];
     double x[16 * H];
 #pragma unroll
     for (int h = 0; h < H; h++)
@@ -85,9 +70,9 @@
         }
     __syncthreads();
     if (H == 2) {
-        const double w = cw[1], wq = tg[1];
-#pragma unroll
-        for (int a = 0; a < 16; a++) ct_fw(x[a], x[16 + a], w, wq, q);
+        const double w = tg[1];
+#pragma unroll
+        for (int a = 0; a < 16; a++) ct_f(x[a], x[16 + a], w, q, qi);
     }
 #pragma unroll
     for (int h = 0; h < H; h++) {
@@ -104,7 +89,7 @@
             for (int a = 0; a < 16; a++) {
                 if (a & hh) continue;
                 const int ti = m * mul + (a >> (4 - st));
-                ct_fw(xh[a], xh[a + hh], cw[ti], tg[ti], q);
+                ct_f(xh[a], xh[a + hh], tg[ti], q, qi);
             }
         }
         if (h > 0) __syncthreads();
@@ -124,7 +109,7 @@
 #pragma unroll
             for (int bb = 0; bb < 16; bb++) {
                 if (bb & hh) continue;
-                ct_f(xh[bb], xh[bb + hh], twq[m * mul + ap * (m >> 4) + (bb >> (8 - st))], q);
+                ct_f(xh[bb], xh[bb + hh], tws[m * mul + ap * (m >> 4) + (bb >> (8 - st))], q, qi);
             }
         }
 #pragma unroll
@@ -134,14 +119,14 @@
 template <int R = 256>
 __global__ __launch_bounds__(256) void k_nttf_fwd_cols(Span src, Span dst, Tabs T) {
     __shared__ double s[256 * kPadF];
-    __shared__ double twq[R];
-    nttf_fwd_cols_body<R>(src, dst, T, blockIdx.x, blockIdx.y, s, twq);
+    __shared__ double tws[R];
+    nttf_fwd_cols_body<R>(src, dst, T, blockIdx.x, blockIdx.y, s, tws);
 }
 template <int R, int SPREAD>
 __global__ __launch_bounds__(256) void k_nttf_fwd_cols_spread(SpreadSrc ss, Span dst, Tabs T) {
     __shared__ double s[256 * kPadF];
-    __shared__ double twq[R];
-    nttf_fwd_cols_body<R, SPREAD>(dst, dst, T, blockIdx.x, blockIdx.y, s, twq, ss);
+    __shared__ double tws[R];
+    nttf_fwd_cols_body<R, SPREAD>(dst, dst, T, blockIdx.x, blockIdx.y, s, tws, ss);
 }
 
 struct RowFin {
@@ -170,13 +155,12 @@
 #pragma unroll
             for (int a = 0; a < 16; a++) x[a] = fred(x[a], q, qi);
         }
-        const double rq = R[st];
+        const double rw = R[st];
 #pragma unroll
         for (int j = 0; j < ml; j++) {
-            double w, wq;
-            tw_row(W, RR * ml + j, rq, q, qi, w, wq);
-#pragma unroll
-            for (int k = 0; k < h; k++) ct_fw(x[j * 2 * h + k], x[j * 2 * h + k + h], w, wq, q);
+            const double w = tw_row(W, RR * ml + j, rw, q, qi);
+#pragma unroll
+            for (int k = 0; k < h; k++) ct_f(x[j * 2 * h + k], x[j * 2 * h + k + h], w, q, qi);
         }
     }
 #pragma unroll
@@ -192,13 +176,12 @@
 #pragma unroll
             for (int bb = 0; bb < 16; bb++) x[bb] = fred(x[bb], q, qi);
         }
-        const double rq = R[st];
+        const double rw = R[st];
 #pragma unroll
         for (int j = 0; j < nj; j++) {
-            double w, wq;
-            tw_row(W, RR * ml + ap * nj + j, rq, q, qi, w, wq);
-#pragma unroll
-            for (int k = 0; k < h; k++) ct_fw(x[j * 2 * h + k], x[j * 2 * h + k + h], w, wq, q);
+            const double w = tw_row(W, RR * ml + ap * nj + j, rw, q, qi);
+#pragma unroll
+            for (int k = 0; k < h; k++) ct_f(x[j * 2 * h + k], x[j * 2 * h + k + h], w, q, qi);
         }
     }
 }
@@ -223,8 +206,8 @@
     const int row = bx * 16 + rl;
     const double q = (double)T.q[pid], qi = T.qinv[pid];
     const bool big = q >= kBigPrime;
-    const double* W = T.psif + ((long)pid << T.logN);
-    const double* Rf = T.rtwf + (long)pid * R * 8 + row * 8;
+    const double* W = T.psid + ((long)pid << T.logN);
+    const double* Rf = T.rtwd + (long)pid * R * 8 + row * 8;
     double x[16];
     double* sr = s + rl * 16 * kPadF;
     const int ap = b;
@@ -285,7 +268,7 @@
     const int row = blockIdx.x * 16 + rl;
     const double q = (double)T.q[pid], qi = T.qinv[pid];
     const bool big = q >= kBigPrime;
-    const double* W = T.ipsif + ((long)pid << T.logN);
+    const double* W = T.ipsid + ((long)pid << T.logN);
     const u64* gb = in + (long)blockIdx.x * 16 * 256;
     {
         const int e0 = (tid >> 6) * 1024 + (tid & 63);
@@ -297,8 +280,8 @@
             for (int k = 0; k < 16; k++) {
                 const int e = e0 + 64 * k;
                 const double y = u2d(gb2[e]);
-                double v = fmul_rem(u2d(gb[e]), y, y * qi, q);
-                if (FMA) v = fmul_rem(v, al, al * qi, q);
+                double v = fmul_remq(u2d(gb[e]), y, qi, q);
+                if (FMA) v = fmul_remq(v, al, qi, q);
                 s[row_tile_idx(e)] = u2d(fcanon(v, q, qi));
             }
         } else {
@@ -315,19 +298,18 @@
     double x[16];
 #pragma unroll
     for (int bb = 0; bb < 16; bb++) x[bb] = sr[ap * kPadF + bb];
-    const double* R = T.irtwf + (long)pid * RR * 8 + row * 8;
+    const double* R = T.irtwd + (long)pid * RR * 8 + row * 8;
     auto stages_lo = [&](auto fold) {
 #pragma unroll
         for (int st = 0; st < 4; st++) {
             const int t = 1 << st, ml = 128 / t, nj = 8 / t;
-            const double rq = R[7 - st];
+            const double rw = R[7 - st];
 #pragma unroll
             for (int j = 0; j < nj; j++) {
-                double w, wq;
-                tw_row(W, RR * ml + ap * nj + j, rq, q, qi, w, wq);
+                const double w = tw_row(W, RR * ml + ap * nj + j, rw, q, qi);
 #pragma unroll
                 for (int k = 0; k < t; k++)
-                    gs_fw<decltype(fold)::value>(x[j * 2 * t + k], x[j * 2 * t + k + t], w, wq, q, qi);
+                    gs_f<decltype(fold)::value>(x[j * 2 * t + k], x[j * 2 * t + k + t], w, q, qi);
             }
         }
     };
@@ -342,14 +324,13 @@
 #pragma unroll
         for (int st = 4; st < 8; st++) {
             const int t = 1 << st, ta = t >> 4, ml = 128 / t;
-            const double rq = R[7 - st];
+            const double rw = R[7 - st];
 #pragma unroll
             for (int j = 0; j < ml; j++) {
-                double w, wq;
-                tw_row(W, RR * ml + j, rq, q, qi, w, wq);
+                const double w = tw_row(W, RR * ml + j, rw, q, qi);
 #pragma unroll
                 for (int k = 0; k < ta; k++)
-                    gs_fw<decltype(fold)::value>(x[j * 2 * ta + k], x[j * 2 * ta + k + ta], w, wq, q, qi);
+                    gs_f<decltype(fold)::value>(x[j * 2 * ta + k], x[j * 2 * ta + k + ta], w, q, qi);
             }
         }
     };
@@ -365,17 +346,16 @@
     static_assert(R == 256 || R == 512, "rows of 256: N = 2^16 or 2^17");
     constexpr int H = R / 256;
     __shared__ double s[256 * kPadF];
-    __shared__ double twq[R];
+    __shared__ double tws[R];
     int pid;
     u64* io = span_ptr(dst, blockIdx.y, T.logN, T.Lp1, pid);
     const int tid = threadIdx.x, cl = tid & 15, b = tid >> 4;
     const int c = blockIdx.x * 16 + cl;
     const double q = (double)T.q[pid], qi = T.qinv[pid];
     const bool big = q >= kBigPrime;
-    const double* tg = T.ipsif + ((long)pid << T.logN);
-    const double* icw = T.icw + (long)pid * kColW;
-#pragma unroll
-    for (int h = 0; h < H; h++) twq[tid + 256 * h] = tg[tid + 256 * h];
+    const double* tg = T.ipsid + ((long)pid << T.logN);
+#pragma unroll
+    for (int h = 0; h < H; h++) tws[tid + 256 * h] = tg[tid + 256 * h];
     const int ap = b;
     double x[16 * H];
 #pragma unroll
@@ -395,7 +375,7 @@
 #pragma unroll
                 for (int bb = 0; bb < 16; bb++) {
                     if (bb & tr) continue;
-                    gs_f<decltype(fold)::value>(xh[bb], xh[bb + tr], twq[base + (bb >> (st + 1))], q, qi);
+                    gs_f<decltype(fold)::value>(xh[bb], xh[bb + tr], tws[base + (bb >> (st + 1))], q, qi);
                 }
             }
         };
@@ -416,7 +396,7 @@
                 for (int a = 0; a < 16; a++) {
                     if (a & ta) continue;
                     const int ti = base + (a >> (st - 3));
-                    gs_fw<decltype(fold)::value>(xh[a], xh[a + ta], icw[ti], tg[ti], q, qi);
+                    gs_f<decltype(fold)::value>(xh[a], xh[a + ta], tg[ti], q, qi);
                 }
             }
         };
@@ -424,12 +404,12 @@
         else stages_hi(std::false_type{});
     }
     if (H == 2) {
-        const double w = icw[1], wq = tg[1];
+        const double w = tg[1];
 #pragma unroll
         for (int a = 0; a < 16; a++) {
             x[a] = fred(x[a], q, qi);
             x[16 + a] = fred(x[16 + a], q, qi);
-            gs_fw<false>(x[a], x[16 + a], w, wq, q, qi);
+            gs_f<false>(x[a], x[16 + a], w, q, qi);
         }
     }
     const double nif = LF ? lf[blockIdx.y % dst.nl] : T.ninvf[pid];
```

Result: faster. 289,200 (median of 6 runs) (+2.0%).
